# ArielleRosinski/pyGAT

Measured on AMD Instinct MI355X. Metric: GAT-layer fwd+bwd edges/sec, higher is better.
Workload: dtype f32

## Files before the change

include/pygat_amd.h:

```cpp
#ifndef PYGAT_AMD_H
#define PYGAT_AMD_H

#include <stdint.h>
#include <stddef.h>

#ifdef __cplusplus
extern "C" {
#endif

#define PYGAT_ABI_VERSION 14

enum {
  PYGAT_OK = 0,
  PYGAT_EINVAL = -1,
  PYGAT_EHIP = -2,
  PYGAT_ENODEV = -3
};

enum {
  PYGAT_F_ELU = 1,
  PYGAT_F_SKIP = 2,
  PYGAT_F_MAIN_ONLY = 4,
  PYGAT_F_FIXUP_ONLY = 8
};

int pygat_abi_version(void);
const char* pygat_last_error(void);
int pygat_padded_width(int f_out);
int pygat_device_count(void);
int pygat_device_name(char* host_buf, int len);
int pygat_kernel_footprint(const char* kernel, int* num_regs, int* scratch_bytes);

enum { PYGAT_GEMM_DEFAULT = -1, PYGAT_GEMM_SPLIT_BF16 = 0, PYGAT_GEMM_FP32_MFMA = 1 };
int pygat_default_gemm_mode(void);

int pygat_dense_row_counts(const float* adj, int n, int64_t ld, int mode,
                           int32_t* counts, void* stream);
size_t pygat_scan_workspace_bytes(int64_t n);
int pygat_exclusive_scan_i32(const int32_t* in, int64_t n, int32_t* out, void* ws, void* stream);
int pygat_dense_fill_cols(const float* adj, int n, int64_t ld, int mode,
                          const int32_t* rowptr, int32_t* col, void* stream);
int pygat_csr_symmetric_perm(int n, const int32_t* rowptr, const int32_t* col,
                             int32_t* perm, int32_t* flags, void* stream);

#define PYGAT_MAX_SEGMENTS 4
typedef struct {
  int nseg;
  int32_t col_start[PYGAT_MAX_SEGMENTS + 1];
  float* ptr[PYGAT_MAX_SEGMENTS];
  int64_t ld[PYGAT_MAX_SEGMENTS];
} pygat_out_segments;

size_t pygat_gemm_workspace_bytes(int M, int N, int split_k);
int pygat_gemm_f32(int transA, int transB, int M, int N, int64_t K,
                   const float* A, int64_t lda, const float* B, int64_t ldb,
                   const pygat_out_segments* out, int accumulate,
                   int split_k, void* ws, int gemm_mode, void* stream);

typedef struct {
  int w;
  int64_t stride;
} pygat_col_blocks;
int pygat_gemm_f32_blocked(int transA, int transB, int M, int N, int64_t K,
                           const float* A, int64_t lda, const pygat_col_blocks* a_blk, const float* B, int64_t ldb,
                           const pygat_out_segments* out, const pygat_col_blocks* c_blk, int accumulate,
                           int split_k, void* ws, int gemm_mode, void* stream);

int pygat_pack_params(int H, int Fin, int Fo, const float* W, const float* a,
                      const float* w_skip, float* Wcat, int64_t ldw, float* a_pad,
                      void* stream);
#define PYGAT_MAX_HEADS_TABLE 16
int pygat_pack_params_heads(int H, int Fin, int Fo, const float* const* W, const float* const* a,
                            const float* const* w_skip, float* Wcat, int64_t ldw, float* a_pad, void* stream);
int pygat_stack_heads(int H, int64_t nW, int nA, int64_t nS, const float* const* W, const float* const* a,
                      const float* const* w_skip, float* W_out, float* a_out, float* skip_out, void* stream);
int pygat_stack_heads_padded(int H, int64_t nW, int64_t nW_out, int nA, int64_t nS, int64_t nS_out, const float* const* W,
                             const float* const* a, const float* const* w_skip, float* W_out, float* a_out, float* skip_out,
                             void* stream);
int pygat_project(int n, int Fin, int H, int Fo, const float* X, int64_t ldx, const float* Wcat, int64_t ldw, const float* a_pad,
                  float* Wh, float* Sk, float* s, int split_k, void* ws, int gemm_mode, void* stream);
int pygat_project_blocked(int n, int Fin, int H, int Fo, const float* X, int64_t ldx, const pygat_col_blocks* x_blk,
                          const float* Wcat, int64_t ldw, const float* a_pad, float* Wh, float* Sk, float* s, int split_k,
                          void* ws, int gemm_mode, void* stream);
int pygat_attn_scores(int n, int H, int Fo, float* Wh, const float* wh_mask, const float* a_pad,
                      float* s, float* t, void* stream);
int pygat_unpack_wgrad(int H, int Fin, int Fo, const float* dWcat, int64_t ld,
                       int col_offset, float* dW, void* stream);

typedef struct {
  int n;
  int64_t nnz;
  const int32_t* rowptr;
  const int32_t* edge_rc;
  int slot_edges;
  const int32_t* slot_begin;
  const int32_t* cut_rows;
  int n_cut;
  int n_cut_wide;
  int64_t slot_first;
  int64_t slot_count;
  const int32_t* slot_meta;
  const int32_t* slot_order;
  const int32_t* user_row;
} pygat_graph;

int pygat_edge_pairs(int n, const int32_t* rowptr, const int32_t* col, int32_t* edge_rc, void* stream);

int pygat_slot_bounds(int n, int64_t nnz, const int32_t* rowptr, const int32_t* edge_rc, int slot_edges,
                      int32_t* slot_begin, void* stream);
int pygat_slot_meta(int n, int64_t nnz, const int32_t* rowptr, const int32_t* edge_rc, int slot_edges,
                    const int32_t* slot_begin, int32_t* slot_meta, void* stream);

size_t pygat_partials_bytes(int64_t nnz, int slot_edges, int H, int Fp);

int pygat_head_group(int n, int H, int Fo);

int pygat_gat_forward_phases_ok(int n, int H, int Fo);
int pygat_gat_forward(const pygat_graph* g, int H, int Fo, float alpha, int flags,
                      const float* Wh, const float* s, const float* a_pad, const float* sk,
                      const float* att_mask,
                      float* out, float* hattn, float* m, float* Z, float* aneg, float* qneg,
                      void* part, void* stream);

int pygat_head_mean(int n, int H, int Fo, const float* hattn, const float* sk,
                    float* out, void* stream);

int pygat_gat_backward_prepare(int n, int H, int Fo, int flags, int mean_mode,
                               const float* G, const float* y, const float* sk,
                               const float* s, const float* m, const float* Z,
                               float* GR, const float* aneg, const float* qneg, float alpha, float* ds,
                               int h_first, int h_count, int head_group, const int32_t* user_row, void* stream);
int pygat_gat_backward_row(const pygat_graph* g, int H, int Fo, float alpha,
                           const float* Wh, const float* a_pad, const float* GR,
                           const float* att_mask, float* ds, void* part, int h_first, int h_count, int head_group,
                           void* stream);
size_t pygat_gat_backward_col_da_bytes(const pygat_graph* gT, int H, int Fo, int head_group);
int pygat_gat_backward_col(const pygat_graph* gT, const int32_t* perm_t, int H, int Fo, float alpha,
                           const float* Wh, const float* a_pad, const float* GR,
                           const float* att_mask, const float* ds,
                           float* dWh, float* dt, float* dz_t, void* part, float* da_part, int h_first, int h_count,
                           int head_group, void* stream);
int pygat_a_grad_fold(const pygat_graph* gT, int H, int Fo, const float* Wh, const float* ds, const float* dt,
                      const float* da_part, float* da, void* ws, int head_group, void* stream);
int pygat_gat_backward_rowsum(const pygat_graph* g, const int32_t* perm_f, int H, int Fo, const float* dz_t,
                              float* ds, void* part, int h_first, int h_count, void* stream);
size_t pygat_agrad_workspace_bytes(int H, int Fo);
int pygat_a_grad(int n, int H, int Fo, const float* Wh, const float* ds, const float* dt,
                 float* da, void* ws, const float* a_pad, float* dWh, const float* dwh_mask, int h_first, int h_count,
                 void* stream);

size_t pygat_wgrad_workspace_bytes(int Fin, int H, int Fo, int split_k);
int pygat_wgrad(int n, int Fin, int H, int Fo, const float* X, int64_t ldx, const float* dWh, const float* ds,
                const float* a_pad, float* dW, int split_k, void* ws, int h_first, int h_count, int gemm_mode, void* stream);

int pygat_wgrad_blocked(int n, int Fin, int H, int Fo, const float* X, int64_t ldx, const pygat_col_blocks* x_blk,
                        const float* dWh, const float* ds, const float* a_pad, float* dW, int split_k, void* ws,
                        int h_first, int h_count, int gemm_mode, void* stream);

int pygat_gat_forward_tail(int row_first, int n_rows, int H, int Fo, int flags, const float* Wh, int64_t ldwh, const float* sk,
                           float* out, const int32_t* user_row, float* m, float* Z, float* qneg, void* stream);
int pygat_gat_backward_col_tail(int row_first, int n_rows, int H, int Fo, const float* GR, float* dWh, float* dt, void* stream);
int pygat_gat_backward_tail(int row_first, int n_rows, int H, int Fo, int flags, const float* G, const float* y,
                            const int32_t* user_row, float* dWh, int64_t ld_dwh, int zero_cols, float* ds, float* dt, void* stream);

int pygat_gatv2_forward(const pygat_graph* g, int H, int Fo, float alpha, int flags,
                        const float* WW, const float* a2, const float* sk, const float* att_mask,
                        float* out, float* hattn, float* m, float* Z, void* part, void* stream);
int pygat_gatv2_backward_prepare(int n, int H, int Fo, int flags, int mean_mode,
                                 const float* G, const float* y, const float* sk,
                                 const float* m, const float* Z, const float* WW, float* GRW, const int32_t* user_row,
                                 void* stream);
size_t pygat_gatv2_workspace_bytes(int64_t nnz, int slot_edges, int H, int Fo);
int pygat_gatv2_backward(const pygat_graph* g, const pygat_graph* gT, const int32_t* perm_t, const int32_t* perm_f,
                         int H, int Fo, float alpha, const float* WW, const float* a2, const float* GRW,
                         const float* att_mask, float* dWW, float* da, void* ws, void* stream);

int pygat_dropout_mask(int64_t count, float p, const void* seed, uint32_t stream_id, float* out, void* stream);
int pygat_dropout_mask2(float p, const void* seed, int64_t count1, uint32_t stream1, float* out1, int64_t count2,
                        uint32_t stream2, float* out2, void* stream);
int pygat_dropout_expand(int n, int Fin, int H, const float* x, int64_t ldx, const float* mask, float p,
                         const void* seed, uint32_t stream_id, float* out, int64_t ldo, void* stream);
int pygat_dropout_head_sum(int n, int Fin, int H, const float* dxe, int64_t lde, const float* mask, float p,
                           const void* seed, uint32_t stream_id, float* dx, int64_t ldx, int accumulate,
                           void* stream);
int pygat_pack_blockdiag(int H, int Fin, int Fo, const float* W, const float* w_skip, float* Bp, int64_t ldb,
                         void* stream);
int pygat_unpack_blockdiag(int H, int Fin, int Fo, const float* dBp, int64_t ldb, int col_offset, float* dW,
                           void* stream);

int pygat_headmask_supported(int H, int Fo, int skip);
int pygat_dropout_bits(int n, int Fin, int H, float p, const void* seed, int stream_id, unsigned char* bits, void* stream);
size_t pygat_project_dropout_workspace_bytes(int n, int H, int Fo, int skip, int split_k);
int pygat_project_dropout(int n, int Fin, int H, int Fo, const float* X, int64_t ldx, const unsigned char* bits, float p,
                          const float* Wcat, int64_t ldw, float* Wh, float* Sk, int split_k, void* ws, void* stream);
size_t pygat_wgrad_dropout_workspace_bytes(int Fin, int H, int Fo, int skip, int split_k);
int pygat_wgrad_dropout(int n, int Fin, int H, int Fo, const float* X, int64_t ldx, const unsigned char* bits, float p,
                        const float* dWh, const float* Gp, int64_t ldgp, float* dWc, int split_k, void* ws, void* stream);
int pygat_dropout_head_sum_bits(int n, int Fin, int H, const float* dxe, int64_t lde, const unsigned char* bits, float p,
                                float* dx, int64_t ldx, int accumulate, void* stream);
int pygat_dropout_narrow(int Fin, int H, int Fo, int skip);
int pygat_dx_dropout(int n, int Fin, int H, int Fo, const float* dWh, const float* Gp, int64_t ldgp, const unsigned char* bits,
                     float p, const float* Wcat, int64_t ldw, float* dx, int64_t lddx, int accumulate, void* stream);

size_t pygat_nll_workspace_bytes(int n);
int pygat_elu_logsoftmax_nll(int n, int C, const float* out, int64_t ldo, const int32_t* label, const float* weight,
                             void* ws, float* loss, void* stream);
int pygat_elu_logsoftmax_nll_backward(int n, int C, const float* out, int64_t ldo, const int32_t* label, const float* weight,
                                      const float* gscale, float* dout, int64_t ldd, void* stream);

int pygat_project_sparse(int n, int Fin, int H, int Fo, const int32_t* rowptr, const int32_t* col, const float* val,
                         const float* Wcat, int64_t ldw, float p, const void* seed, int stream_id, const unsigned char* bits,
                         float* Wh, float* Sk, float* s, void* stream);
size_t pygat_wgrad_sparse_workspace_bytes(int nseg, int H, int Fo, int skip);
int pygat_wgrad_sparse(int n, int Fin, int H, int Fo, int nseg, const int32_t* colseg, const int32_t* seg_col,
                       const int32_t* seg_begin, const int32_t* seg_end, const int32_t* row, const float* val, float p,
                       const void* seed, int stream_id, const unsigned char* bits, const float* dWh, const float* Gp, int64_t ldg,
                       void* ws, float* dW, float* dWskip, void* stream);

size_t pygat_bce_workspace_bytes(int64_t total);
int pygat_bce_with_logits(int64_t total, const float* logits, const float* targets, void* ws, float* loss, void* stream);
int pygat_bce_with_logits_backward(int64_t total, const float* logits, const float* targets, const float* gscale, float* dlogits,
                                   void* stream);

#define PYGAT_ADAM_MAX_TENSORS 48
#define PYGAT_ADAM_STATE_BYTES 24
int pygat_adam_step(int ntensors, float* const* params, const float* const* grads, float* const* exp_avg,
                    float* const* exp_avg_sq, const int64_t* numel, double lr, double beta1, double beta2, double eps,
                    double weight_decay, void* state, void* stream);

#ifdef __cplusplus
}
#endif
#endif
```

pygat_amd/_lib.py:

```python
from __future__ import annotations

import ctypes as C
import os

import torch

_HERE = os.path.dirname(os.path.abspath(__file__))
LIB_PATH = os.path.join(_HERE, "libpygat_amd.so")
from .config import config as _config
if _config.lib_path:
    LIB_PATH = os.path.abspath(_config.lib_path)

ABI_VERSION = 14
F_ELU = 1
F_SKIP = 2
F_MAIN_ONLY = 4
F_FIXUP_ONLY = 8

SYMBOLS = [
    "pygat_abi_version", "pygat_last_error", "pygat_padded_width", "pygat_device_count",
    "pygat_device_name", "pygat_kernel_footprint", "pygat_default_gemm_mode", "pygat_dense_row_counts", "pygat_scan_workspace_bytes",
    "pygat_exclusive_scan_i32", "pygat_dense_fill_cols", "pygat_csr_symmetric_perm",
    "pygat_gemm_workspace_bytes", "pygat_gemm_f32", "pygat_gemm_f32_blocked", "pygat_project_blocked", "pygat_wgrad_blocked", "pygat_pack_params", "pygat_pack_params_heads", "pygat_stack_heads", "pygat_stack_heads_padded", "pygat_project", "pygat_attn_scores",
    "pygat_unpack_wgrad",
    "pygat_edge_pairs", "pygat_slot_bounds", "pygat_slot_meta", "pygat_partials_bytes", "pygat_head_group", "pygat_gat_forward", "pygat_gat_forward_phases_ok", "pygat_gat_forward_tail", "pygat_gat_backward_col_tail", "pygat_gat_backward_tail", "pygat_head_mean",
    "pygat_gat_backward_prepare", "pygat_gat_backward_row", "pygat_gat_backward_col", "pygat_gat_backward_rowsum",
    "pygat_gat_backward_col_da_bytes", "pygat_a_grad_fold",
    "pygat_agrad_workspace_bytes", "pygat_a_grad", "pygat_wgrad_workspace_bytes", "pygat_wgrad",
    "pygat_gatv2_forward", "pygat_gatv2_backward_prepare", "pygat_gatv2_workspace_bytes", "pygat_gatv2_backward",
    "pygat_dropout_mask", "pygat_dropout_mask2", "pygat_dropout_expand", "pygat_dropout_head_sum", "pygat_pack_blockdiag",
    "pygat_unpack_blockdiag",
    "pygat_headmask_supported", "pygat_dropout_bits", "pygat_project_dropout_workspace_bytes", "pygat_project_dropout",
    "pygat_wgrad_dropout_workspace_bytes",
    "pygat_wgrad_dropout", "pygat_dropout_head_sum_bits",
    "pygat_nll_workspace_bytes", "pygat_elu_logsoftmax_nll", "pygat_elu_logsoftmax_nll_backward",
    "pygat_project_sparse", "pygat_wgrad_sparse", "pygat_wgrad_sparse_workspace_bytes", "pygat_dropout_narrow", "pygat_dx_dropout", "pygat_adam_step", "pygat_bce_workspace_bytes", "pygat_bce_with_logits", "pygat_bce_with_logits_backward",
]


MAX_ADAM_TENSORS = 48
MAX_SEGMENTS = 4


class OutSegments(C.Structure):
    _fields_ = [("nseg", C.c_int), ("col_start", C.c_int32 * (MAX_SEGMENTS + 1)), ("ptr", C.c_void_p * MAX_SEGMENTS),
                ("ld", C.c_int64 * MAX_SEGMENTS)]


class ColBlocks(C.Structure):
    _fields_ = [("w", C.c_int), ("stride", C.c_int64)]


class Graph(C.Structure):
    _fields_ = [("n", C.c_int), ("nnz", C.c_int64), ("rowptr", C.c_void_p), ("edge_rc", C.c_void_p),
                ("slot_edges", C.c_int), ("slot_begin", C.c_void_p), ("cut_rows", C.c_void_p),
                ("n_cut", C.c_int), ("n_cut_wide", C.c_int), ("slot_first", C.c_int64), ("slot_count", C.c_int64),
                ("slot_meta", C.c_void_p), ("slot_order", C.c_void_p), ("user_row", C.c_void_p)]


def _load():
    if not os.path.exists(LIB_PATH):
        raise ImportError(
            f"pygat_amd: {LIB_PATH} not found. Build it with `python -c 'import __graft_entry__ as g; "
            f"g.build()'` or `make -C pygat_amd/csrc`. There is no CPU/PyTorch fallback for the hot path.")
    lib = C.CDLL(LIB_PATH)
    missing = [s for s in SYMBOLS if not hasattr(lib, s)]
    if missing:
        raise ImportError(f"pygat_amd: {LIB_PATH} lacks symbols {missing}")
    p, i, i64, f, sz = C.c_void_p, C.c_int, C.c_int64, C.c_float, C.c_size_t
    lib.pygat_abi_version.restype = i
    lib.pygat_last_error.restype = C.c_char_p
    lib.pygat_padded_width.argtypes = [i]
    lib.pygat_device_name.argtypes = [C.c_char_p, i]
    lib.pygat_kernel_footprint.argtypes = [C.c_char_p, C.POINTER(C.c_int), C.POINTER(C.c_int)]
    lib.pygat_default_gemm_mode.argtypes = []
    lib.pygat_dense_row_counts.argtypes = [p, i, i64, i, p, p]
    lib.pygat_scan_workspace_bytes.argtypes = [i64]
    lib.pygat_scan_workspace_bytes.restype = sz
    lib.pygat_exclusive_scan_i32.argtypes = [p, i64, p, p, p]
    lib.pygat_dense_fill_cols.argtypes = [p, i, i64, i, p, p, p]
    lib.pygat_csr_symmetric_perm.argtypes = [i, p, p, p, p, p]
    lib.pygat_gemm_workspace_bytes.argtypes = [i, i, i]
    lib.pygat_gemm_workspace_bytes.restype = sz
    lib.pygat_gemm_f32.argtypes = [i, i, i, i, i64, p, i64, p, i64, C.POINTER(OutSegments), i, i, p, i, p]
    CB = C.POINTER(ColBlocks)
    lib.pygat_gemm_f32_blocked.argtypes = [i, i, i, i, i64, p, i64, CB, p, i64, C.POINTER(OutSegments), CB, i, i, p, i, p]
    lib.pygat_project_blocked.argtypes = [i, i, i, i, p, i64, CB, p, i64, p, p, p, p, i, p, i, p]
    lib.pygat_wgrad_blocked.argtypes = [i, i, i, i, p, i64, CB, p, p, p, p, i, p, i, i, i, p]
    lib.pygat_pack_params.argtypes = [i, i, i, p, p, p, p, i64, p, p]
    lib.pygat_pack_params_heads.argtypes = [i, i, i, p, p, p, p, i64, p, p]
    lib.pygat_stack_heads.argtypes = [i, i64, i, i64, p, p, p, p, p, p, p]
    lib.pygat_stack_heads_padded.argtypes = [i, i64, i64, i, i64, i64, p, p, p, p, p, p, p]
    lib.pygat_unpack_wgrad.argtypes = [i, i, i, p, i64, i, p, p]
    lib.pygat_attn_scores.argtypes = [i, i, i, p, p, p, p, p, p]
    lib.pygat_project.argtypes = [i, i, i, i, p, i64, p, i64, p, p, p, p, i, p, i, p]
    lib.pygat_edge_pairs.argtypes = [i, p, p, p, p]
    lib.pygat_slot_bounds.argtypes = [i, i64, p, p, i, p, p]
    lib.pygat_slot_meta.argtypes = [i, i64, p, p, i, p, p, p]
    lib.pygat_partials_bytes.argtypes = [i64, i, i, i]
    lib.pygat_partials_bytes.restype = sz
    lib.pygat_head_group.argtypes = [i, i, i]
    lib.pygat_head_group.restype = i
    lib.pygat_gat_forward.argtypes = [C.POINTER(Graph), i, i, f, i, p, p, p, p, p, p, p, p, p, p, p, p, p]
    lib.pygat_gat_forward_phases_ok.argtypes = [i, i, i]
    lib.pygat_gat_forward_tail.argtypes = [i, i, i, i, i, p, i64, p, p, p, p, p, p, p]
    lib.pygat_gat_backward_col_tail.argtypes = [i, i, i, i, p, p, p, p]
    lib.pygat_gat_backward_tail.argtypes = [i, i, i, i, i, p, p, p, p, i64, i, p, p, p]
    lib.pygat_head_mean.argtypes = [i, i, i, p, p, p, p]
    lib.pygat_gat_backward_prepare.argtypes = [i, i, i, i, i, p, p, p, p, p, p, p, p, p, f, p, i, i, i, p, p]
    lib.pygat_gat_backward_row.argtypes = [C.POINTER(Graph), i, i, f, p, p, p, p, p, p, i, i, i, p]
    lib.pygat_gat_backward_col.argtypes = [C.POINTER(Graph), p, i, i, f, p, p, p, p, p, p, p, p, p, p, i, i, i, p]
    lib.pygat_gat_backward_col_da_bytes.argtypes = [C.POINTER(Graph), i, i, i]
    lib.pygat_gat_backward_col_da_bytes.restype = sz
    lib.pygat_a_grad_fold.argtypes = [C.POINTER(Graph), i, i, p, p, p, p, p, p, i, p]
    lib.pygat_gat_backward_rowsum.argtypes = [C.POINTER(Graph), p, i, i, p, p, p, i, i, p]
    lib.pygat_agrad_workspace_bytes.argtypes = [i, i]
    lib.pygat_agrad_workspace_bytes.restype = sz
    lib.pygat_a_grad.argtypes = [i, i, i, p, p, p, p, p, p, p, p, i, i, p]
    lib.pygat_gatv2_forward.argtypes = [C.POINTER(Graph), i, i, f, i, p, p, p, p, p, p, p, p, p, p]
    lib.pygat_gatv2_backward_prepare.argtypes = [i, i, i, i, i, p, p, p, p, p, p, p, p, p]
    lib.pygat_gatv2_workspace_bytes.argtypes = [i64, i, i, i]
    lib.pygat_gatv2_workspace_bytes.restype = sz
    lib.pygat_gatv2_backward.argtypes = [C.POINTER(Graph), C.POINTER(Graph), p, p, i, i, f, p, p, p, p, p, p, p, p]
    u32 = C.c_uint32
    lib.pygat_wgrad_workspace_bytes.argtypes = [i, i, i, i]
    lib.pygat_wgrad_workspace_bytes.restype = sz
    lib.pygat_wgrad.argtypes = [i, i, i, i, p, i64, p, p, p, p, i, p, i, i, i, p]
    lib.pygat_dropout_mask.argtypes = [i64, f, p, u32, p, p]
    lib.pygat_dropout_mask2.argtypes = [f, p, i64, u32, p, i64, u32, p, p]
    lib.pygat_dropout_expand.argtypes = [i, i, i, p, i64, p, f, p, u32, p, i64, p]
    lib.pygat_dropout_head_sum.argtypes = [i, i, i, p, i64, p, f, p, u32, p, i64, i, p]
    lib.pygat_pack_blockdiag.argtypes = [i, i, i, p, p, p, i64, p]
    lib.pygat_unpack_blockdiag.argtypes = [i, i, i, p, i64, i, p, p]
    lib.pygat_headmask_supported.argtypes = [i, i, i]
    lib.pygat_dropout_bits.argtypes = [i, i, i, f, p, i, p, p]
    lib.pygat_project_dropout_workspace_bytes.argtypes = [i, i, i, i, i]
    lib.pygat_project_dropout_workspace_bytes.restype = sz
    lib.pygat_project_dropout.argtypes = [i, i, i, i, p, i64, p, f, p, i64, p, p, i, p, p]
    lib.pygat_wgrad_dropout_workspace_bytes.argtypes = [i, i, i, i, i]
    lib.pygat_wgrad_dropout_workspace_bytes.restype = sz
    lib.pygat_wgrad_dropout.argtypes = [i, i, i, i, p, i64, p, f, p, p, i64, p, i, p, p]
    lib.pygat_dropout_head_sum_bits.argtypes = [i, i, i, p, i64, p, f, p, i64, i, p]
    lib.pygat_project_sparse.argtypes = [i, i, i, i, p, p, p, p, i64, f, p, i, p, p, p, p, p]
    lib.pygat_wgrad_sparse.argtypes = [i, i, i, i, i, p, p, p, p, p, p, f, p, i, p, p, p, i64, p, p, p, p]
    lib.pygat_wgrad_sparse_workspace_bytes.argtypes = [i, i, i, i]
    lib.pygat_dropout_narrow.argtypes = [i, i, i, i]
    lib.pygat_bce_workspace_bytes.argtypes = [i64]
    lib.pygat_bce_workspace_bytes.restype = sz
    lib.pygat_bce_with_logits.argtypes = [i64, p, p, p, p, p]
    lib.pygat_bce_with_logits_backward.argtypes = [i64, p, p, p, p, p]
    lib.pygat_adam_step.argtypes = [i, p, p, p, p, p, C.c_double, C.c_double, C.c_double, C.c_double, C.c_double, p, p]
    lib.pygat_dx_dropout.argtypes = [i, i, i, i, p, p, i64, p, f, p, i64, p, i64, i, p]
    lib.pygat_wgrad_sparse_workspace_bytes.restype = sz
    lib.pygat_nll_workspace_bytes.argtypes = [i]
    lib.pygat_nll_workspace_bytes.restype = sz
    lib.pygat_elu_logsoftmax_nll.argtypes = [i, i, p, i64, p, p, p, p, p]
    lib.pygat_elu_logsoftmax_nll_backward.argtypes = [i, i, p, i64, p, p, p, p, i64, p]
    for s in SYMBOLS:
        fn = getattr(lib, s)
        if fn.restype is C.c_int or s in ("pygat_abi_version", "pygat_padded_width", "pygat_device_count", "pygat_default_gemm_mode"):
            fn.restype = i
    if lib.pygat_abi_version() != ABI_VERSION:
        raise ImportError(f"pygat_amd: ABI version {lib.pygat_abi_version()} != {ABI_VERSION}")
    return lib


lib = _load()


def check(rc: int, what: str = "") -> None:
    if rc == 0:
        return
    msg = lib.pygat_last_error().decode(errors="replace")
    if rc == -1:
        raise ValueError(f"pygat_amd {what}: {msg}")
    raise RuntimeError(f"pygat_amd {what}: {msg} (code {rc})")


def padded_width(f_out: int) -> int:
    fp = lib.pygat_padded_width(int(f_out))
    if fp == 0:
        raise ValueError(f"pygat_amd: head width {f_out} unsupported (1..256)")
    return fp
```

pygat_amd/config.py:

```python
from __future__ import annotations

import os
from dataclasses import dataclass, fields
from typing import Optional


def _flag(name: str, default: bool) -> bool:
    v = os.environ.get(name)
    return default if v is None else v not in ("0", "", "false", "False")


def _opt_flag(name: str) -> Optional[bool]:
    v = os.environ.get(name)
    return None if v is None else v == "1"


def _opt_int(name: str) -> Optional[int]:
    v = os.environ.get(name)
    return int(v) if v else None


@dataclass(frozen=True)
class Config:
    lib_path: Optional[str]
    dist_chunks: int
    dropout_wide: bool
    sparse_max_density: float
    sparse_x: bool
    slot_edges: Optional[int]
    slot_meta: bool
    two_gather_backward: Optional[bool]
    backward: Optional[str]
    da_in_k4: bool
    k1_split_min_k: int
    overlap_backward: bool
    pad_k: bool
    renumber: bool
    tail: bool

    @staticmethod
    def from_env() -> "Config":
        return Config(
            lib_path=os.environ.get("PYGAT_AMD_LIB") or None,
            dist_chunks=int(os.environ.get("PYGAT_DIST_CHUNKS", 4)),
            dropout_wide=_flag("PYGAT_DROPOUT_WIDE", False),
            sparse_max_density=float(os.environ.get("PYGAT_SPARSE_MAX_DENSITY", 0.15)),
            sparse_x=_flag("PYGAT_SPARSE_X", True),
            slot_edges=_opt_int("PYGAT_SLOT_EDGES"),
            slot_meta=not _flag("PYGAT_NO_SLOT_META", False),
            two_gather_backward=_opt_flag("PYGAT_TWO_GATHER_BACKWARD"),
            backward=os.environ.get("PYGAT_BACKWARD") or None,
            da_in_k4=_flag("PYGAT_DA_IN_K4", True),
            k1_split_min_k=int(os.environ.get("PYGAT_K1_SPLIT_MIN_K", 128)),
            overlap_backward=_flag("PYGAT_OVERLAP_BACKWARD", False),
            pad_k=_flag("PYGAT_PAD_K", True),
            renumber=_flag("PYGAT_RENUMBER", True),
            tail=_flag("PYGAT_TAIL", True),
        )

    def describe(self) -> dict:
        return {f.name: getattr(self, f.name) for f in fields(self)}


config = Config.from_env()
```

pygat_amd/csrc/core.hip:

```cpp
#include "common.h"
#include <string.h>

namespace pygat {
static thread_local char g_err[512] = "";

void set_error(const char* fmt, ...) {
  va_list ap;
  va_start(ap, fmt);
  vsnprintf(g_err, sizeof(g_err), fmt, ap);
  va_end(ap);
}

static const int g_default_split = [] { const char* e = getenv("PYGAT_GEMM_F32"); return (e && atoi(e) != 0) ? 0 : 1; }();
bool gemm_split(int mode) { return mode == PYGAT_GEMM_DEFAULT ? g_default_split != 0 : mode == PYGAT_GEMM_SPLIT_BF16; }
}

extern "C" int pygat_default_gemm_mode(void) { return pygat::g_default_split ? PYGAT_GEMM_SPLIT_BF16 : PYGAT_GEMM_FP32_MFMA; }

extern "C" int pygat_abi_version(void) { return PYGAT_ABI_VERSION; }
extern "C" const char* pygat_last_error(void) { return pygat::g_err; }
extern "C" int pygat_padded_width(int f_out) { return pygat::padded_width(f_out); }

namespace pygat {
int footprint_k2_headline(int* regs, int* scratch);
int footprint_k4_headline_da(int* regs, int* scratch);
int footprint_gemm_x3(int which, int* regs, int* scratch);
}

extern "C" int pygat_kernel_footprint(const char* kernel, int* num_regs, int* scratch_bytes) {
  PYGAT_REQUIRE(kernel && num_regs && scratch_bytes, "kernel_footprint: null argument");
  if (!strcmp(kernel, "k2_headline")) return pygat::footprint_k2_headline(num_regs, scratch_bytes);
  if (!strcmp(kernel, "k4_headline_da")) return pygat::footprint_k4_headline_da(num_regs, scratch_bytes);
  if (!strcmp(kernel, "tn_x3w")) return pygat::footprint_gemm_x3(0, num_regs, scratch_bytes);
  if (!strcmp(kernel, "x3gw")) return pygat::footprint_gemm_x3(1, num_regs, scratch_bytes);
  pygat::set_error("kernel_footprint: unknown kernel '%s' (k2_headline, k4_headline_da, tn_x3w, x3gw)", kernel);
  return PYGAT_EINVAL;
}

extern "C" int pygat_device_count(void) {
  int n = 0;
  if (hipGetDeviceCount(&n) != hipSuccess) {
    (void)hipGetLastError();
    return 0;
  }
  return n;
}

extern "C" int pygat_device_name(char* host_buf, int len) {
  if (!host_buf || len <= 0) return PYGAT_EINVAL;
  int dev = 0;
  hipDeviceProp_t p;
  if (hipGetDevice(&dev) != hipSuccess || hipGetDeviceProperties(&p, dev) != hipSuccess) {
    (void)hipGetLastError();
    pygat::set_error("no HIP device");
    return PYGAT_ENODEV;
  }
  snprintf(host_buf, (size_t)len, "%s (%s)", p.name, p.gcnArchName);
  return PYGAT_OK;
}
```

pygat_amd/csrc/gemm_fast.h:

```cpp
#pragma once
#include "common.h"

namespace pygat {

typedef float f32x16 __attribute__((ext_vector_type(16)));

struct SmallKArgs {
  int M, N, K;
  const float* A;
  int64_t lda;
  const float* B;
  int64_t ldb;
  pygat_out_segments out;
  int accumulate;
  int tiles_m;
  int transB;
  const float* sr_a;
  int sr_fp;
  const float* svec;
  int64_t sv_ld;
  int sv_n;
  float* s_out;
  int64_t s_ld;
  int vec_out, s_vec;
  int lds_rows;
};

struct TnArgs {
  int M, N;
  int64_t K;
  const float* A;
  int64_t lda;
  const float* B;
  int64_t ldb;
  int64_t k_per_split;
  float* ws;
  int N1;
  const float* B2;
  int64_t ldb2;
};

#ifdef __HIPCC__
__device__ __forceinline__ float* out_segment(const pygat_out_segments& out, int col, int64_t& ld) {
  ld = out.ld[0];
  float* p = out.ptr[0];
  int c0 = 0;
#pragma unroll
  for (int q = 1; q < PYGAT_MAX_SEGMENTS; ++q)
    if (q < out.nseg && col >= out.col_start[q]) { ld = out.ld[q]; p = out.ptr[q]; c0 = out.col_start[q]; }
  return p + (col - c0);
}
#endif

bool gemm_split(int mode);

int try_gemm_smallk_x3(const SmallKArgs& g, int NT, dim3 grid, hipStream_t st);
int try_project_x3(int n, int Fin, int H, int Fp, const float* X, int64_t ldx, const float* Wcat, int64_t ldw, float* Wh,
                   float* s, const float* a_pad, bool split, hipStream_t st);
int try_gemm_tn_x3(const TnArgs& g, int splits, hipStream_t st);
int try_gemm_x3g(int transA, int transB, int M, int N, int64_t K, const float* A, int64_t lda, const float* B, int64_t ldb,
                 const pygat_out_segments* out, int accumulate, int splits, int64_t k_per_split, float* ws, hipStream_t st,
                 ColBlocks ab, ColBlocks cb, int* splits_used);

}
```

pygat_amd/csrc/k1_gemm.hip:

```cpp
#include "common.h"
#include "narrow.h"
#include <type_traits>

namespace pygat {

typedef float f32x16 __attribute__((ext_vector_type(16)));

constexpr int BM = 128;
constexpr int BK = 16;
constexpr int PAD = 4;

struct GemmArgs {
  int M, N;
  int64_t K;
  const float* A;
  int64_t lda;
  const float* B;
  int64_t ldb;
  pygat_out_segments out;
  int accumulate;
  int64_t k_per_split;
  float* ws;
  int a_vec, b_vec;
  ColBlocks ab, cb;
// ... 216 lines not shown
        __syncthreads();
        if (kt + 1 < nkt) {
          gload2(kof(kt + 3));
          mma_tile(1);
          if (kt + 2 < nkt) sstore(0);
          __syncthreads();
        }
        if (((kt >> 1) % (FLUSH_TILES / 2)) == FLUSH_TILES / 2 - 1) flush();
      }
    } else {
      if (nkt > 0) {
        gload(kbeg);
        sstore(0);
      }
      __syncthreads();
      for (int64_t kt = 0; kt < nkt; ++kt) {
        const int buf = (int)(kt & 1);
        if (kt + 1 < nkt) gload(kbeg + (kt + 1) * BK);
        mma_tile(buf);
        if (kt + 1 < nkt) sstore(buf ^ 1);
        __syncthreads();
        if ((kt % FLUSH_TILES) == FLUSH_TILES - 1) flush();
      }
    }
  };
  if (interior) kloop(std::true_type{});
  else kloop(std::false_type{});
#pragma unroll
  for (int i = 0; i < NT; ++i)
#pragma unroll
    for (int r = 0; r < 16; ++r) acc[i][r] += acc2[i][r];

#pragma unroll
  for (int nt = 0; nt < NT; ++nt) {
    const int col = n0 + 32 * nt + fr;
    if (col >= g.N) continue;
    float* base;
    int64_t ld;
    if (g.ws) {
      base = g.ws + ((int64_t)blockIdx.z * g.M) * g.N + col;
      ld = g.N;
    } else if (g.cb.lw < 62) {
      base = g.out.ptr[0] + blk_off(col, g.cb);
      ld = g.out.ld[0];
    } else {
      int s = 0;
#pragma unroll
      for (int q = 1; q < PYGAT_MAX_SEGMENTS; ++q)
        if (q < g.out.nseg && col >= g.out.col_start[q]) s = q;
      base = g.out.ptr[s] + (col - g.out.col_start[s]);
      ld = g.out.ld[s];
    }
#pragma unroll
    for (int r = 0; r < 16; ++r) {
      const int row = m0 + 32 * w + (r & 3) + 8 * (r >> 2) + 4 * fk;
      if (row < g.M) {
        float* p = base + (int64_t)row * ld;
        if (!g.ws && g.accumulate) *p += acc[nt][r];
        else *p = acc[nt][r];
      }
    }
  }
}

__global__ __launch_bounds__(512) void gemm_splitk_reduce_kernel(int M, int N, int splits,
                                                                 const float* __restrict__ ws,
                                                                 pygat_out_segments out, int accumulate) {
  const int64_t tot = (int64_t)M * N;
  const int lane = threadIdx.x & 63, q = threadIdx.x >> 6;
  const int64_t i = (int64_t)blockIdx.x * 64 + lane;
  float v = 0.f;
  if (i < tot) {
    int z = q;
    for (; z + 24 < splits; z += 32) {
      const float x0 = ws[(int64_t)z * tot + i], x1 = ws[(int64_t)(z + 8) * tot + i];
      const float x2 = ws[(int64_t)(z + 16) * tot + i], x3 = ws[(int64_t)(z + 24) * tot + i];
      v += x0; v += x1; v += x2; v += x3;
    }
    for (; z < splits; z += 8) v += ws[(int64_t)z * tot + i];
  }
  __shared__ float sm[8][64];
  sm[q][lane] = v;
  __syncthreads();
  if (q == 0 && i < tot) {
    float acc = 0.f;
#pragma unroll
    for (int z = 0; z < 8; ++z) acc += sm[z][lane];
    const int row = (int)(i / N), col = (int)(i % N);
    int s = 0;
    for (int k = 1; k < out.nseg; ++k)
      if (col >= out.col_start[k]) s = k;
    float* p = out.ptr[s] + (int64_t)row * out.ld[s] + (col - out.col_start[s]);
    if (accumulate) *p += acc; else *p = acc;
  }
}

struct HeadMaskArgs {
  int M;
  int64_t K;
  const float* A;
  int64_t lda;
  const unsigned char* bits;
  const float* B1;
  int64_t ldb1;
  const float* B2;
  int64_t ldb2;
  float* C1;
  int64_t ldc1;
  float* C2;
  int64_t ldc2;
  int64_t c_split_stride;
  int H, Fp;
  float scale;
  int64_t k_per_split;
};

typedef float f32x4_u __attribute__((ext_vector_type(4), aligned(4)));
typedef uint32_t u32_u __attribute__((aligned(1)));

template <bool TA, int HB, int NTH>
__global__ __launch_bounds__(256) __attribute__((amdgpu_waves_per_eu(2))) void gemm_headmask_kernel(HeadMaskArgs g) {
  constexpr int NTOT = HB * NTH, BN = 32 * NTOT;
  constexpr int LDAS = BM + PAD, LDBS = BN + PAD;
  constexpr int NVA = 2;
  constexpr int NU = (BK * HB * 8 * NTH + 255) / 256;
  extern __shared__ __attribute__((aligned(16))) float hm_sm[];
  float* As = hm_sm;
  float* Bs = As + 2 * BK * LDAS;
  unsigned char* Ms = reinterpret_cast<unsigned char*>(Bs + 2 * BK * LDBS);
  const int m0 = blockIdx.x * BM, hb0 = blockIdx.y * HB;
  const int64_t kbeg = (int64_t)blockIdx.z * g.k_per_split;
  const int64_t kend = (kbeg + g.k_per_split < g.K) ? kbeg + g.k_per_split : g.K;
  const int lane = threadIdx.x & 63, w = threadIdx.x >> 6;
  const int cols_h = g.B2 ? 2 * g.Fp : g.Fp;
  const int q_h = cols_h >> 2;
  const int units = BK * HB * q_h;

  f32x16 acc[NTOT];
#pragma unroll
  for (int i = 0; i < NTOT; ++i)
#pragma unroll
    for (int r = 0; r < 16; ++r) acc[i][r] = 0.f;

  float4 ra[NVA];
  uint32_t rm[NVA];
  float4 rb[NU];
  auto gload = [&](int64_t k0) {
#pragma unroll
    for (int i = 0; i < NVA; ++i) {
      const int idx = threadIdx.x + 256 * i;
      float4 v = make_float4(0.f, 0.f, 0.f, 0.f);
      uint32_t mv = 0;
      int64_t off;
      int nval;
      if constexpr (TA) {
        const int64_t k = k0 + idx / (BM / 4);
        const int c = m0 + (idx % (BM / 4)) * 4;
        off = k * g.lda + c;
        nval = (k < kend) ? (g.M - c) : 0;
      } else {
        const int row = m0 + (idx >> 2);
        const int64_t k = k0 + (idx & 3) * 4;
        off = (int64_t)row * g.lda + k;
        nval = (row < g.M) ? (int)(kend - k) : 0;
      }
      if (nval >= 4) {
        const f32x4_u t = *reinterpret_cast<const f32x4_u*>(g.A + off);
        v = make_float4(t.x, t.y, t.z, t.w);
        mv = *reinterpret_cast<const u32_u*>(g.bits + off);
      } else if (nval > 0) {
        float t[4] = {0.f, 0.f, 0.f, 0.f};
        for (int q = 0; q < nval; ++q) { t[q] = g.A[off + q]; mv |= (uint32_t)g.bits[off + q] << (8 * q); }
        v = make_float4(t[0], t[1], t[2], t[3]);
      }
      ra[i] = v; rm[i] = mv;
    }
#pragma unroll
    for (int i = 0; i < NU; ++i) {
      const int u = threadIdx.x + 256 * i;
      float4 v = make_float4(0.f, 0.f, 0.f, 0.f);
      if (u < units) {
        const int kk = u / (HB * q_h), r2 = u - kk * (HB * q_h), hl = r2 / q_h, c = (r2 - hl * q_h) * 4;
        const int64_t k = k0 + kk;
        const int h = hb0 + hl;
        if (k < kend && h < g.H)
          v = c < g.Fp ? ld4(g.B1 + k * g.ldb1 + (int64_t)h * g.Fp + c) : ld4(g.B2 + k * g.ldb2 + (int64_t)h * g.Fp + (c - g.Fp));
      }
      rb[i] = v;
    }
  };
  auto sstore = [&](int buf) {
    float* as = As + buf * BK * LDAS;
    unsigned char* ms = Ms + buf * BK * LDAS;
    if constexpr (TA) store_kstrided<BM, NVA, LDAS>(as, ra);
    else store_kcontig<BM, NVA, LDAS>(as, ra);
#pragma unroll
    for (int i = 0; i < NVA; ++i) {
      const int idx = threadIdx.x + 256 * i;
      if constexpr (TA) {
        *reinterpret_cast<uint32_t*>(ms + (idx / (BM / 4)) * LDAS + (idx % (BM / 4)) * 4) = rm[i];
      } else {
        const int row = idx >> 2, kq = (idx & 3) * 4;
        ms[(kq + 0) * LDAS + row] = (unsigned char)rm[i]; ms[(kq + 1) * LDAS + row] = (unsigned char)(rm[i] >> 8);
        ms[(kq + 2) * LDAS + row] = (unsigned char)(rm[i] >> 16); ms[(kq + 3) * LDAS + row] = (unsigned char)(rm[i] >> 24);
      }
    }
    float* bs = Bs + buf * BK * LDBS;
#pragma unroll
    for (int i = 0; i < NU; ++i) {
      const int u = threadIdx.x + 256 * i;
      if (u < units) {
        const int kk = u / (HB * q_h), r2 = u - kk * (HB * q_h), hl = r2 / q_h, c = (r2 - hl * q_h) * 4;
        st4(bs + kk * LDBS + hl * 32 * NTH + c, rb[i]);
      }
    }
  };

  const int64_t nkt = (kend > kbeg) ? (kend - kbeg + BK - 1) / BK : 0;
  if (nkt > 0) { gload(kbeg); sstore(0); }
  __syncthreads();
  const int fr = lane & 31, fk = lane >> 5;
  for (int64_t kt = 0; kt < nkt; ++kt) {
    const int buf = (int)(kt & 1);
    if (kt + 1 < nkt) gload(kbeg + (kt + 1) * BK);
    const float* as = As + buf * BK * LDAS + fk * LDAS + 32 * w + fr;
    const unsigned char* ms = Ms + buf * BK * LDAS + fk * LDAS + 32 * w + fr;
    const float* bs = Bs + buf * BK * LDBS + fk * LDBS + fr;
#pragma unroll
    for (int kk = 0; kk < BK; kk += 2) {
      const float xs = as[kk * LDAS];
      const uint32_t mb = (uint32_t)ms[kk * LDAS] >> hb0;
#pragma unroll
      for (int hl = 0; hl < HB; ++hl) {
        const float a = ((mb >> hl) & 1u) ? xs : 0.f;
#pragma unroll
        for (int nt = 0; nt < NTH; ++nt)
          acc[hl * NTH + nt] = __builtin_amdgcn_mfma_f32_32x32x2f32(a, bs[kk * LDBS + 32 * (hl * NTH + nt)], acc[hl * NTH + nt], 0, 0, 0);
      }
    }
    if (kt + 1 < nkt) sstore(buf ^ 1);
    __syncthreads();
  }

  const int64_t zoff = (int64_t)blockIdx.z * g.c_split_stride;
#pragma unroll
  for (int hl = 0; hl < HB; ++hl) {
    const int h = hb0 + hl;
    if (h >= g.H) continue;
#pragma unroll
    for (int nt = 0; nt < NTH; ++nt) {
      const int c = 32 * nt + fr;
      if (c >= cols_h) continue;
      float* base = c < g.Fp ? g.C1 + zoff + (int64_t)h * g.Fp + c : g.C2 + zoff + (int64_t)h * g.Fp + (c - g.Fp);
      const int64_t ld = c < g.Fp ? g.ldc1 : g.ldc2;
#pragma unroll
      for (int r = 0; r < 16; ++r) {
        const int row = m0 + 32 * w + (r & 3) + 8 * (r >> 2) + 4 * fk;
        if (row < g.M) base[(int64_t)row * ld] = acc[hl * NTH + nt][r] * g.scale;
      }
    }
  }
}

template <bool TA>
static int launch_headmask(const HeadMaskArgs& g, int splits, hipStream_t st) {
  const int cols_h = g.B2 ? 2 * g.Fp : g.Fp;
  const int nth = cols_h <= 32 ? 1 : cols_h <= 64 ? 2 : cols_h <= 128 ? 4 : 8;
  const int hb = 8 / nth;
  if (cols_h > 256 || g.H > 8) return 0;
  dim3 grid((unsigned)cdiv(g.M, BM), (unsigned)cdiv(g.H, hb), (unsigned)splits);
  const size_t lds = (size_t)(2 * BK * (BM + PAD) + 2 * BK * (32 * 8 + PAD)) * sizeof(float) + 2 * BK * (BM + PAD);
  switch (nth) {
    case 1: hipLaunchKernelGGL((gemm_headmask_kernel<TA, 8, 1>), grid, dim3(256), lds, st, g); break;
    case 2: hipLaunchKernelGGL((gemm_headmask_kernel<TA, 4, 2>), grid, dim3(256), lds, st, g); break;
    case 4: hipLaunchKernelGGL((gemm_headmask_kernel<TA, 2, 4>), grid, dim3(256), lds, st, g); break;
    default: hipLaunchKernelGGL((gemm_headmask_kernel<TA, 1, 8>), grid, dim3(256), lds, st, g); break;
  }
  return 1;
}

template <bool TA, bool TB>
static int launch_gemm(const GemmArgs& g, int splits, hipStream_t st) {
  const int nt_needed = (int)cdiv(g.N, 32);
  int NT = nt_needed <= 1 ? 1 : nt_needed <= 2 ? 2 : nt_needed <= 3 ? 3 : nt_needed <= 4 ? 4 : nt_needed <= 5 ? 5 : 4;
  dim3 grid((unsigned)cdiv(g.M, BM), (unsigned)cdiv(g.N, 32 * NT), (unsigned)splits);
  auto lds = [](int nt, int bk) { return (size_t)2 * bk * ((BM + PAD) + (32 * nt + PAD)) * sizeof(float); };
  switch (NT) {
    case 1: hipLaunchKernelGGL((gemm_f32_kernel<TA, TB, 1, 16>), grid, dim3(256), lds(1, 16), st, g); break;
    case 2: hipLaunchKernelGGL((gemm_f32_kernel<TA, TB, 2, 16>), grid, dim3(256), lds(2, 16), st, g); break;
    case 3: hipLaunchKernelGGL((gemm_f32_kernel<TA, TB, 3, 16>), grid, dim3(256), lds(3, 16), st, g); break;
    case 4: hipLaunchKernelGGL((gemm_f32_kernel<TA, TB, 4, 16>), grid, dim3(256), lds(4, 16), st, g); break;
    default: hipLaunchKernelGGL((gemm_f32_kernel<TA, TB, 5, 16>), grid, dim3(256), lds(5, 16), st, g); break;
  }
  return 0;
}

int try_gemm_smallk(int transB, int M, int N, int64_t K, const float* A, int64_t lda, const float* B, int64_t ldb,
                    const pygat_out_segments* out, int accumulate, bool split, hipStream_t st, const float* svec = nullptr,
                    int64_t sv_ld = 0, int sv_n = 0, float* s_out = nullptr, int64_t s_ld = 0);
int try_gemm_tn_stream(int M, int N, int64_t K, const float* A, int64_t lda, const float* B, int64_t ldb,
                       int max_splits, float* ws, bool split, hipStream_t st, int N1, const float* B2, int64_t ldb2);
int try_project_x3(int n, int Fin, int H, int Fp, const float* X, int64_t ldx, const float* Wcat, int64_t ldw, float* Wh,
                   float* s, const float* a_pad, bool split, hipStream_t st);
int try_gemm_x3g(int transA, int transB, int M, int N, int64_t K, const float* A, int64_t lda, const float* B, int64_t ldb,
                 const pygat_out_segments* out, int accumulate, int splits, int64_t k_per_split, float* ws, hipStream_t st,
                 ColBlocks ab, ColBlocks cb, int* splits_used);
bool gemm_split(int mode);

}

using namespace pygat;

extern "C" size_t pygat_gemm_workspace_bytes(int M, int N, int split_k) {
  if (split_k <= 1) return 0;
  return (size_t)split_k * (size_t)M * (size_t)N * sizeof(float);
}

extern "C" int pygat_gemm_f32(int transA, int transB, int M, int N, int64_t K, const float* A, int64_t lda,
                              const float* B, int64_t ldb, const pygat_out_segments* out, int accumulate,
                              int split_k, void* ws, int gemm_mode, void* stream) {
  return pygat_gemm_f32_blocked(transA, transB, M, N, K, A, lda, nullptr, B, ldb, out, nullptr, accumulate, split_k, ws, gemm_mode,
                                stream);
}

extern "C" int pygat_gemm_f32_blocked(int transA, int transB, int M, int N, int64_t K, const float* A, int64_t lda,
                                      const pygat_col_blocks* a_blk, const float* B, int64_t ldb, const pygat_out_segments* out,
                                      const pygat_col_blocks* c_blk, int accumulate, int split_k, void* ws, int gemm_mode,
                                      void* stream) {
  PYGAT_REQUIRE(A && B && out, "gemm: null pointer");
  PYGAT_REQUIRE(gemm_mode >= PYGAT_GEMM_DEFAULT && gemm_mode <= PYGAT_GEMM_FP32_MFMA, "gemm: unknown product mode %d", gemm_mode);
  const bool split = gemm_split(gemm_mode);
  PYGAT_REQUIRE(M > 0 && N > 0 && K > 0, "gemm: bad sizes M=%d N=%d K=%lld", M, N, (long long)K);
  PYGAT_REQUIRE(out->nseg >= 1 && out->nseg <= PYGAT_MAX_SEGMENTS && out->col_start[0] == 0 && out->col_start[out->nseg] == N,
                "gemm: output segments must cover [0,N) (nseg=%d)", out->nseg);
  const bool a_blocked = col_blocks_on(a_blk), c_blocked = col_blocks_on(c_blk);
  for (int s = 0; s < out->nseg; ++s)
    PYGAT_REQUIRE(out->ptr[s] && out->col_start[s + 1] > out->col_start[s] &&
                      (c_blocked || out->ld[s] >= out->col_start[s + 1] - out->col_start[s]),
                  "gemm: bad output segment %d", s);
  PYGAT_REQUIRE((a_blocked ? lda >= a_blk->w : lda >= (transA ? M : K)) && ldb >= (transB ? K : N), "gemm: leading dimension too small");
  PYGAT_REQUIRE(col_blocks_ok(a_blk, transA ? M : K, lda) && (!a_blocked || aligned16(A)),
                "gemm: bad column blocks of A (w a power of two >= 16 dividing the blocked extent; 16-byte aligned base, rows, blocks)");
  PYGAT_REQUIRE(!c_blocked || (col_blocks_ok(c_blk, N, out->ld[0]) && out->nseg == 1 && aligned16(out->ptr[0])),
                "gemm: bad column blocks of C (one segment; w a power of two >= 16 dividing N)");
  if (split_k < 1) split_k = 1;
  PYGAT_REQUIRE(split_k == 1 || ws, "gemm: split_k > 1 needs a workspace");
  PYGAT_REQUIRE(!c_blocked || split_k == 1, "gemm: a column-blocked C takes no split-K");
  const ColBlocks ab = col_blocks_of(a_blk), cb = col_blocks_of(c_blk);
  hipStream_t st = (hipStream_t)stream;
  if (a_blocked || c_blocked) {
  } else if (!transA && split_k == 1) {
    int r = try_gemm_smallk(transB, M, N, K, A, lda, B, ldb, out, accumulate, split, st);
    if (r < 0) return r;
    if (r == 1) return PYGAT_OK;
  }
  if (!a_blocked && transA && !transB && split_k > 1) {
    int r = try_gemm_tn_stream(M, N, K, A, lda, B, ldb, split_k, (float*)ws, split, st, N, nullptr, 0);
    if (r < 0) return r;
    if (r >= 1) {
      int64_t tot = (int64_t)M * N;
      hipLaunchKernelGGL(gemm_splitk_reduce_kernel, dim3((unsigned)cdiv(tot, 64)), dim3(512), 0, st, M, N, r,
                         (const float*)ws, *out, accumulate);
      PYGAT_CHECK_LAUNCH("gemm_splitk_reduce");
      return PYGAT_OK;
    }
  }
  if (split) {
    const int64_t kps16 = cdiv(cdiv(K, split_k), 16) * 16;
    int sp = (int)cdiv(K, kps16);
    const int r = try_gemm_x3g(transA, transB, M, N, K, A, lda, B, ldb, out, accumulate, sp, kps16, (float*)ws, st, ab, cb, &sp);
    if (r < 0) return r;
    if (r == 1) {
      if (sp > 1) {
        hipLaunchKernelGGL(gemm_splitk_reduce_kernel, dim3((unsigned)cdiv((int64_t)M * N, 64)), dim3(512), 0, st, M, N, sp,
                           (const float*)ws, *out, accumulate);
        PYGAT_CHECK_LAUNCH("gemm_splitk_reduce");
      }
      return PYGAT_OK;
    }
  }
  GemmArgs g;
  g.M = M; g.N = N; g.K = K; g.A = A; g.lda = lda; g.B = B; g.ldb = ldb; g.out = *out;
  g.accumulate = accumulate;
  g.ab = ab; g.cb = cb;
  int64_t kps = cdiv(cdiv(K, split_k), BK) * BK;
  int splits = (int)cdiv(K, kps);
  g.k_per_split = kps;
  g.ws = (splits > 1) ? (float*)ws : nullptr;
  g.a_vec = aligned16(A) && (lda % 4 == 0);
  g.b_vec = aligned16(B) && (ldb % 4 == 0);
  if (!transA && !transB) launch_gemm<false, false>(g, splits, st);
  else if (transA && !transB) launch_gemm<true, false>(g, splits, st);
  else if (!transA && transB) launch_gemm<false, true>(g, splits, st);
  else { pygat::set_error("gemm: transA && transB is not built"); return PYGAT_EINVAL; }
  PYGAT_CHECK_LAUNCH("gemm_f32");
  if (splits > 1) {
    int64_t tot = (int64_t)M * N;
    hipLaunchKernelGGL(gemm_splitk_reduce_kernel, dim3((unsigned)cdiv(tot, 64)), dim3(512), 0, st, M, N, splits,
                       (const float*)ws, *out, accumulate);
    PYGAT_CHECK_LAUNCH("gemm_splitk_reduce");
  }
  return PYGAT_OK;
}

extern "C" int pygat_project(int n, int Fin, int H, int Fo, const float* X, int64_t ldx, const float* Wcat, int64_t ldw,
                             const float* a_pad, float* Wh, float* Sk, float* s, int split_k, void* ws, int gemm_mode,
                             void* stream) {
  return pygat_project_blocked(n, Fin, H, Fo, X, ldx, nullptr, Wcat, ldw, a_pad, Wh, Sk, s, split_k, ws, gemm_mode, stream);
}

extern "C" int pygat_project_blocked(int n, int Fin, int H, int Fo, const float* X, int64_t ldx, const pygat_col_blocks* x_blk,
                                     const float* Wcat, int64_t ldw, const float* a_pad, float* Wh, float* Sk, float* s,
                                     int split_k, void* ws, int gemm_mode, void* stream) {
  const bool blocked = col_blocks_on(x_blk);
  const int Fp = padded_width(Fo);
  PYGAT_REQUIRE(n > 0 && Fin > 0 && H > 0 && Fp > 0 && X && Wcat && Wh && s, "project: bad arguments");
  PYGAT_REQUIRE(gemm_mode >= PYGAT_GEMM_DEFAULT && gemm_mode <= PYGAT_GEMM_FP32_MFMA, "project: unknown product mode %d", gemm_mode);
  const bool split = gemm_split(gemm_mode);
  const int R = H * Fp, nw = R * (Sk ? 2 : 1), ncols = nw + H;
  PYGAT_REQUIRE(ldw >= nw + 2 * H && (blocked ? ldx >= x_blk->w : ldx >= Fin), "project: leading dimension too small");
  pygat_out_segments seg;
  int k = 0;
  if (!blocked && a_pad && split_k <= 1) {
    const int r = try_project_x3(n, Fin, H, Fp, X, ldx, Wcat, ldw, Wh, s, a_pad, split, (hipStream_t)stream);
    if (r < 0) return r;
    if (r == 1) {
      if (!Sk) return PYGAT_OK;
      seg.nseg = 1; seg.col_start[0] = 0; seg.col_start[1] = R; seg.ptr[0] = Sk; seg.ld[0] = R;
      return pygat_gemm_f32(0, 0, n, R, Fin, X, ldx, Wcat + R, ldw, &seg, 0, 1, nullptr, gemm_mode, stream);
    }
  }
  seg.col_start[0] = 0; seg.ptr[k] = Wh; seg.ld[k] = R; ++k;
  if (Sk) { seg.col_start[k] = R; seg.ptr[k] = Sk; seg.ld[k] = R; ++k; }
  if (!blocked && H <= 8 && split_k <= 1) {
    seg.col_start[k] = nw; seg.nseg = k;
    const int r = try_gemm_smallk(0, n, nw, Fin, X, ldx, Wcat, ldw, &seg, 0, split, (hipStream_t)stream, Wcat + nw, ldw, H, s, H);
    if (r < 0) return r;
    if (r == 1) return PYGAT_OK;
  }
  seg.col_start[k] = nw; seg.ptr[k] = s; seg.ld[k] = H; ++k;
  seg.col_start[k] = ncols;
  seg.nseg = k;
  return pygat_gemm_f32_blocked(0, 0, n, ncols, Fin, X, ldx, x_blk, Wcat, ldw, &seg, nullptr, 0, split_k, ws, gemm_mode, stream);
}

namespace pygat {
__global__ __launch_bounds__(256) void unpack_wgrad_rank1_kernel(int H, int Fin, int Fo, int Fp, const float* __restrict__ dWc,
                                                                 int64_t ld, int with_ds, const float* __restrict__ a_pad,
                                                                 float* __restrict__ dW) {
  const int64_t idx = (int64_t)blockIdx.x * 256 + threadIdx.x;
  if (idx >= (int64_t)H * Fin * Fo) return;
  const int f = (int)(idx % Fo);
  const int k = (int)((idx / Fo) % Fin);
  const int h = (int)(idx / ((int64_t)Fo * Fin));
  float v = dWc[(int64_t)k * ld + h * Fp + f];
  if (with_ds) v = fmaf(dWc[(int64_t)k * ld + H * Fp + h], a_pad[(int64_t)h * 2 * Fp + f], v);
  dW[idx] = v;
}
}

extern "C" size_t pygat_wgrad_workspace_bytes(int Fin, int H, int Fo, int split_k) {
  const int Fp = padded_width(Fo);
  if (Fin <= 0 || H <= 0 || Fp <= 0) return 0;
  if (split_k < 1) split_k = 1;
  const size_t ncols = (size_t)H * Fp + (size_t)((H + 3) / 4) * 4;
  return (size_t)(split_k + 1) * (size_t)Fin * ncols * sizeof(float);
}

extern "C" int pygat_wgrad(int n, int Fin, int H, int Fo, const float* X, int64_t ldx, const float* dWh, const float* ds,
                           const float* a_pad, float* dW, int split_k, void* ws, int h_first, int h_count, int gemm_mode,
                           void* stream) {
  return pygat_wgrad_blocked(n, Fin, H, Fo, X, ldx, nullptr, dWh, ds, a_pad, dW, split_k, ws, h_first, h_count, gemm_mode, stream);
}

extern "C" int pygat_wgrad_blocked(int n, int Fin, int H, int Fo, const float* X, int64_t ldx, const pygat_col_blocks* x_blk,
                                   const float* dWh, const float* ds, const float* a_pad, float* dW, int split_k, void* ws,
                                   int h_first, int h_count, int gemm_mode, void* stream) {
  const bool blocked = col_blocks_on(x_blk);
  const int Fp = padded_width(Fo);
  PYGAT_REQUIRE(gemm_mode >= PYGAT_GEMM_DEFAULT && gemm_mode <= PYGAT_GEMM_FP32_MFMA, "wgrad: unknown product mode %d", gemm_mode);
  const bool split = gemm_split(gemm_mode);
  PYGAT_REQUIRE(n > 0 && Fin > 0 && H > 0 && Fp > 0 && X && dWh && dW && ws && (blocked ? ldx >= x_blk->w : ldx >= Fin),
                "wgrad: bad arguments");
  PYGAT_REQUIRE(!ds || a_pad, "wgrad: ds needs a_pad");
  if (h_count == 0 && h_first == 0) h_count = H;
  PYGAT_REQUIRE(h_first >= 0 && h_count > 0 && h_first + h_count <= H, "wgrad: bad head range [%d, +%d) of %d", h_first, h_count, H);
  const int64_t ldd = (int64_t)H * Fp, lds = H;
  dWh += (int64_t)h_first * Fp;
  if (ds) ds += h_first;
  if (a_pad) a_pad += (int64_t)h_first * 2 * Fp;
  dW += (int64_t)h_first * Fin * Fo;
  H = h_count;
  if (split_k < 1) split_k = 1;
  hipStream_t st = (hipStream_t)stream;
  const int R = H * Fp;
  const int ldc = R + ((H + 3) / 4) * 4;
  float* dWc = (float*)ws;
  float* slabs = dWc + (size_t)Fin * ldc;
  pygat_out_segments seg;
  seg.nseg = 1; seg.col_start[0] = 0; seg.ptr[0] = dWc; seg.ld[0] = ldc;
  bool done = false;
  if (!blocked && ds && split_k > 1 && split && R > 64 && Fin > 64) {
    seg.col_start[1] = R;
    int r = try_gemm_tn_stream(Fin, R, n, X, ldx, dWh, ldd, split_k, slabs, split, st, R, nullptr, 0);
    if (r < 0) return r;
    if (r >= 1) {
      hipLaunchKernelGGL(gemm_splitk_reduce_kernel, dim3((unsigned)cdiv((int64_t)Fin * R, 64)), dim3(512), 0, st, Fin, R, r,
                         (const float*)slabs, seg, 0);
      PYGAT_CHECK_LAUNCH("wgrad(reduce)");
      pygat_out_segments seg2;
      seg2.nseg = 1; seg2.col_start[0] = 0; seg2.col_start[1] = H; seg2.ptr[0] = dWc + R; seg2.ld[0] = ldc;
      int64_t sk2 = (int64_t)split_k * (R + H) / H;
      if (sk2 > 256) sk2 = 256;
      const int r2 = try_gemm_tn_stream(Fin, H, n, X, ldx, ds, lds, (int)sk2, slabs, split, st, H, nullptr, 0);
      if (r2 < 0) return r2;
      if (r2 >= 1) {
        hipLaunchKernelGGL(gemm_splitk_reduce_kernel, dim3((unsigned)cdiv((int64_t)Fin * H, 64)), dim3(512), 0, st, Fin, H, r2,
                           (const float*)slabs, seg2, 0);
        PYGAT_CHECK_LAUNCH("wgrad(reduce ds)");
      } else {
        const int rc = pygat_gemm_f32(1, 0, Fin, H, n, X, ldx, ds, lds, &seg2, 0, split_k, slabs, gemm_mode, stream);
        if (rc) return rc;
      }
      done = true;
    }
  }
  if (!blocked && !done && ds && split_k > 1) {
    seg.col_start[1] = R + H;
    int r = try_gemm_tn_stream(Fin, R + H, n, X, ldx, dWh, ldd, split_k, slabs, split, st, R, ds, lds);
    if (r < 0) return r;
    if (r >= 1) {
      const int64_t tot = (int64_t)Fin * (R + H);
      hipLaunchKernelGGL(gemm_splitk_reduce_kernel, dim3((unsigned)cdiv(tot, 64)), dim3(512), 0, st, Fin, R + H, r,
                         (const float*)slabs, seg, 0);
      PYGAT_CHECK_LAUNCH("wgrad(reduce)");
      done = true;
    }
  }
  if (!done) {
    seg.col_start[1] = R;
    int rc = pygat_gemm_f32_blocked(1, 0, Fin, R, n, X, ldx, x_blk, dWh, ldd, &seg, nullptr, 0, split_k, slabs, gemm_mode, stream);
    if (rc) return rc;
    if (ds) {
      seg.col_start[1] = H; seg.ptr[0] = dWc + R;
      rc = pygat_gemm_f32_blocked(1, 0, Fin, H, n, X, ldx, x_blk, ds, lds, &seg, nullptr, 0, split_k, slabs, gemm_mode, stream);
      if (rc) return rc;
    }
  }
  hipLaunchKernelGGL(unpack_wgrad_rank1_kernel, dim3((unsigned)cdiv((int64_t)H * Fin * Fo, 256)), dim3(256), 0, st, H, Fin,
                     Fo, Fp, (const float*)dWc, (int64_t)ldc, ds ? 1 : 0, a_pad, dW);
  PYGAT_CHECK_LAUNCH("wgrad(unpack)");
  return PYGAT_OK;
}


extern "C" int pygat_headmask_supported(int H, int Fo, int skip) {
  const int Fp = padded_width(Fo);
  return (H >= 1 && H <= 8 && Fp > 0 && Fp * (skip ? 2 : 1) <= 256) ? 1 : 0;
}

extern "C" size_t pygat_project_dropout_workspace_bytes(int n, int H, int Fo, int skip, int split_k) {
  const int Fp = padded_width(Fo);
  if (n <= 0 || H <= 0 || Fp <= 0 || split_k <= 1) return 0;
  return (size_t)split_k * (size_t)n * (size_t)(H * Fp * (skip ? 2 : 1)) * sizeof(float);
}

extern "C" int pygat_project_dropout(int n, int Fin, int H, int Fo, const float* X, int64_t ldx, const unsigned char* bits,
                                     float p, const float* Wcat, int64_t ldw, float* Wh, float* Sk, int split_k, void* ws,
                                     void* stream) {
  const int Fp = padded_width(Fo);
  PYGAT_REQUIRE(n > 0 && Fin > 0 && X && bits && Wcat && Wh && ldx == Fin, "project_dropout: bad arguments (X must be dense: ldx == Fin)");
  PYGAT_REQUIRE(pygat_headmask_supported(H, Fo, Sk != nullptr), "project_dropout: unsupported H=%d F'=%d", H, Fo);
  PYGAT_REQUIRE(p >= 0.f && p <= 1.f, "project_dropout: p=%g outside [0,1]", (double)p);
  if (narrow_takes(Fin, H, Fo, Sk != nullptr))
    return narrow_project(n, Fin, H, Fo, X, ldx, bits, p, Wcat, ldw, Wh, Sk, (hipStream_t)stream);
  if (split_k < 1) split_k = 1;
  PYGAT_REQUIRE(split_k == 1 || ws, "project_dropout: split_k > 1 needs a workspace");
  const int R = H * Fp, ntot = R * (Sk ? 2 : 1);
  hipStream_t st = (hipStream_t)stream;
  const int64_t kps = cdiv(cdiv(Fin, split_k), BK) * BK;
  const int splits = (int)cdiv(Fin, kps);
  HeadMaskArgs g;
  g.M = n; g.K = Fin; g.A = X; g.lda = ldx; g.bits = bits;
  g.B1 = Wcat; g.ldb1 = ldw; g.B2 = Sk ? Wcat + R : nullptr; g.ldb2 = ldw;
  if (splits > 1) {
    g.C1 = (float*)ws; g.ldc1 = ntot; g.C2 = (float*)ws + R; g.ldc2 = ntot; g.c_split_stride = (int64_t)n * ntot;
  } else {
    g.C1 = Wh; g.ldc1 = R; g.C2 = Sk; g.ldc2 = R; g.c_split_stride = 0;
  }
  g.H = H; g.Fp = Fp; g.scale = p < 1.f ? 1.f / (1.f - p) : 0.f; g.k_per_split = kps;
  launch_headmask<false>(g, splits, st);
  PYGAT_CHECK_LAUNCH("project_dropout");
  if (splits > 1) {
    pygat_out_segments seg;
    seg.nseg = Sk ? 2 : 1; seg.col_start[0] = 0; seg.ptr[0] = Wh; seg.ld[0] = R; seg.col_start[1] = R;
    if (Sk) { seg.ptr[1] = Sk; seg.ld[1] = R; seg.col_start[2] = 2 * R; }
    hipLaunchKernelGGL(gemm_splitk_reduce_kernel, dim3((unsigned)cdiv((int64_t)n * ntot, 64)), dim3(512), 0, st, n, ntot,
                       splits, (const float*)ws, seg, 0);
    PYGAT_CHECK_LAUNCH("project_dropout(reduce)");
  }
  return PYGAT_OK;
}

extern "C" size_t pygat_wgrad_dropout_workspace_bytes(int Fin, int H, int Fo, int skip, int split_k) {
  const int Fp = padded_width(Fo);
  if (Fin <= 0 || H <= 0 || Fp <= 0) return 0;
  if (split_k < 1) split_k = 1;
  return (size_t)split_k * (size_t)Fin * (size_t)(H * Fp * (skip ? 2 : 1)) * sizeof(float);
}

extern "C" int pygat_wgrad_dropout(int n, int Fin, int H, int Fo, const float* X, int64_t ldx, const unsigned char* bits,
                                   float p, const float* dWh, const float* Gp, int64_t ldgp, float* dWc, int split_k,
                                   void* ws, void* stream) {
  const int Fp = padded_width(Fo);
  PYGAT_REQUIRE(n > 0 && Fin > 0 && X && bits && dWh && dWc && ldx == Fin, "wgrad_dropout: bad arguments");
  PYGAT_REQUIRE(pygat_headmask_supported(H, Fo, Gp != nullptr), "wgrad_dropout: unsupported H=%d F'=%d", H, Fo);
  if (split_k < 1) split_k = 1;
  PYGAT_REQUIRE(split_k == 1 || ws, "wgrad_dropout: split_k > 1 needs a workspace");
  if (narrow_takes(Fin, H, Fo, Gp != nullptr)) {
    PYGAT_REQUIRE(ws, "wgrad_dropout: the narrow kernels need the workspace (pygat_wgrad_dropout_workspace_bytes)");
    return narrow_wgrad(n, Fin, H, Fo, X, ldx, bits, p, dWh, Gp, ldgp, dWc, split_k, ws, (hipStream_t)stream);
  }
  const int R = H * Fp, ntot = R * (Gp ? 2 : 1);
  hipStream_t st = (hipStream_t)stream;
  int64_t kps = cdiv(cdiv(n, split_k), BK) * BK;
  const int splits = (int)cdiv(n, kps);
  float* out = splits > 1 ? (float*)ws : dWc;
  HeadMaskArgs g;
  g.M = Fin; g.K = n; g.A = X; g.lda = ldx; g.bits = bits;
  g.B1 = dWh; g.ldb1 = R; g.B2 = Gp; g.ldb2 = ldgp;
  g.C1 = out; g.ldc1 = ntot; g.C2 = out + R; g.ldc2 = ntot; g.c_split_stride = (int64_t)Fin * ntot;
  g.H = H; g.Fp = Fp; g.scale = p < 1.f ? 1.f / (1.f - p) : 0.f; g.k_per_split = kps;
  launch_headmask<true>(g, splits, st);
  PYGAT_CHECK_LAUNCH("wgrad_dropout");
  if (splits > 1) {
    pygat_out_segments seg;
    seg.nseg = 1; seg.col_start[0] = 0; seg.col_start[1] = ntot; seg.ptr[0] = dWc; seg.ld[0] = ntot;
    hipLaunchKernelGGL(gemm_splitk_reduce_kernel, dim3((unsigned)cdiv((int64_t)Fin * ntot, 64)), dim3(512), 0, st, Fin, ntot,
                       splits, (const float*)ws, seg, 0);
    PYGAT_CHECK_LAUNCH("wgrad_dropout(reduce)");
  }
  return PYGAT_OK;
}
```

pygat_amd/csrc/k1_gemm_x3.hip:

```cpp
#include "gemm_fast.h"
#include <stdlib.h>
#include <type_traits>

namespace pygat {

typedef __bf16 bf16x8 __attribute__((ext_vector_type(8)));

struct U4 { uint32_t v[4]; };
struct Frag3 { U4 h, m, l; };

__device__ __forceinline__ void split_pair(float x0, float x1, uint32_t& h, uint32_t& m, uint32_t& l) {
  const uint32_t u0 = __float_as_uint(x0), u1 = __float_as_uint(x1);
  h = __builtin_amdgcn_perm(u1, u0, 0x07060302u);
  const float r0 = x0 - __uint_as_float(u0 & 0xffff0000u), r1 = x1 - __uint_as_float(u1 & 0xffff0000u);
  const uint32_t v0 = __float_as_uint(r0), v1 = __float_as_uint(r1);
  m = __builtin_amdgcn_perm(v1, v0, 0x07060302u);
  const float q0 = r0 - __uint_as_float(v0 & 0xffff0000u), q1 = r1 - __uint_as_float(v1 & 0xffff0000u);
  l = __builtin_amdgcn_perm(__float_as_uint(q1), __float_as_uint(q0), 0x07060302u);
}
__device__ __forceinline__ Frag3 split8(float x0, float x1, float x2, float x3, float x4, float x5, float x6, float x7) {
  Frag3 f;
  split_pair(x0, x1, f.h.v[0], f.m.v[0], f.l.v[0]);
  split_pair(x2, x3, f.h.v[1], f.m.v[1], f.l.v[1]);
  split_pair(x4, x5, f.h.v[2], f.m.v[2], f.l.v[2]);
  split_pair(x6, x7, f.h.v[3], f.m.v[3], f.l.v[3]);
  return f;
}
__device__ __forceinline__ Frag3 split8v(const float4& a, const float4& b) { return split8(a.x, a.y, a.z, a.w, b.x, b.y, b.z, b.w); }
__device__ __forceinline__ void split_one(float x, uint16_t& h, uint16_t& m, uint16_t& l) {
  const uint32_t u = __float_as_uint(x);
  h = (uint16_t)(u >> 16);
  const float r = x - __uint_as_float(u & 0xffff0000u);
  const uint32_t v = __float_as_uint(r);
  m = (uint16_t)(v >> 16);
  const float q = r - __uint_as_float(v & 0xffff0000u);
  l = (uint16_t)(__float_as_uint(q) >> 16);
}

template <class TA_, class TB_>
__device__ __forceinline__ f32x16 mfma_bf16(const TA_& a, const TB_& b, f32x16 c) {
  return __builtin_amdgcn_mfma_f32_32x32x16_bf16(__builtin_bit_cast(bf16x8, a), __builtin_bit_cast(bf16x8, b), c, 0, 0, 0);
}
__device__ __forceinline__ void pair_of(const float4& a, const float4& b, int j, float& x0, float& x1) {
  if (j == 0) { x0 = a.x; x1 = a.y; } else if (j == 1) { x0 = a.z; x1 = a.w; } else if (j == 2) { x0 = b.x; x1 = b.y; } else { x0 = b.z; x1 = b.w; }
}
#ifndef PYGAT_DIAG_K1
#define PYGAT_DIAG_K1 0
#endif
#ifndef PYGAT_K1_LDS_ROWS
#define PYGAT_K1_LDS_ROWS 1
#endif
template <class TB_>
__device__ __forceinline__ f32x16 mma9(const Frag3& a, const TB_& bh, const TB_& bm, const TB_& bl, f32x16 c) {
#if (PYGAT_DIAG_K1 & 8)
  return mfma_bf16(a.h, bh, c);
#endif
  c = mfma_bf16(a.l, bl, c);
  c = mfma_bf16(a.l, bm, c);
  c = mfma_bf16(a.m, bl, c);
  c = mfma_bf16(a.l, bh, c);
  c = mfma_bf16(a.h, bl, c);
  c = mfma_bf16(a.m, bm, c);
  c = mfma_bf16(a.m, bh, c);
  c = mfma_bf16(a.h, bm, c);
  c = mfma_bf16(a.h, bh, c);
  return c;
}

template <class TB_>
__device__ __forceinline__ f32x16 mma9t(const Frag3& x, const TB_& wh, const TB_& wm, const TB_& wl, f32x16 c) {
#if (PYGAT_DIAG_K1 & 8)
  return mfma_bf16(wh, x.h, c);
#endif
  c = mfma_bf16(wl, x.l, c);
  c = mfma_bf16(wm, x.l, c);
  c = mfma_bf16(wl, x.m, c);
  c = mfma_bf16(wh, x.l, c);
  c = mfma_bf16(wl, x.h, c);
  c = mfma_bf16(wm, x.m, c);
  c = mfma_bf16(wh, x.m, c);
  c = mfma_bf16(wm, x.h, c);
  c = mfma_bf16(wh, x.h, c);
  return c;
}
__device__ __forceinline__ float half_wave_sum(float x) {
  const uint32_t u = __float_as_uint(x);
  const auto r = __builtin_amdgcn_permlane32_swap(u, u, false, false);
  return __uint_as_float(r[0]) + __uint_as_float(r[1]);
}

#if (PYGAT_DIAG_K1 & 16)
__device__ unsigned long long k1_stamps[2048 * 8 * 8];
#endif
template <bool TB, int NT, int SM, int SPC>
__global__ __launch_bounds__(512) void gemm_smallk_x3_kernel(SmallKArgs g) {
  constexpr bool SV = (SM == 1);
  constexpr int SRF = (SM >= 4) ? SM : 0;
  constexpr int BN = 32 * NT;
  extern __shared__ __attribute__((aligned(16))) unsigned char smem_x3[];
  const int KP = g.K + 8;
  uint16_t* Bimg = reinterpret_cast<uint16_t*>(smem_x3);
  const int IMG = BN * KP;
  float* Us = reinterpret_cast<float*>(Bimg + 3 * IMG);
  float* Asr = Us + (SV ? g.K * 8 : 0);
  float* Stg = Asr + (SRF > 0 ? BN : 0) + 4;
  const int n0 = blockIdx.y * BN;
  unsigned long long st_entry = 0; (void)st_entry;
  if ((PYGAT_DIAG_K1 & 16)) st_entry = __builtin_amdgcn_s_memrealtime();
  for (int item = threadIdx.x; item < (g.K >> 3) * BN; item += 512) {
    const int n = item % BN, k8 = item / BN;
    const bool ok = n0 + n < g.N;
    float v[8];
    if constexpr (!TB) {
      const float* bp = g.B + (int64_t)(8 * k8) * g.ldb + (ok ? n0 + n : 0);
#pragma unroll
      for (int j = 0; j < 8; ++j) v[j] = bp[(int64_t)j * g.ldb];
    } else {
      const float* bp = g.B + (int64_t)(ok ? n0 + n : 0) * g.ldb + 8 * k8;
#pragma unroll
      for (int j = 0; j < 8; ++j) v[j] = bp[j];
    }
    uint32_t ph[4], pm[4], pl[4];
#pragma unroll
    for (int j = 0; j < 4; ++j) {
      uint16_t h0, m0, l0, h1, m1, l1;
      split_one(ok ? v[2 * j] : 0.f, h0, m0, l0);
      split_one(ok ? v[2 * j + 1] : 0.f, h1, m1, l1);
      ph[j] = (uint32_t)h0 | ((uint32_t)h1 << 16); pm[j] = (uint32_t)m0 | ((uint32_t)m1 << 16); pl[j] = (uint32_t)l0 | ((uint32_t)l1 << 16);
    }
    uint16_t* d = Bimg + n * KP + 8 * k8;
    *reinterpret_cast<uint4*>(d) = make_uint4(ph[0], ph[1], ph[2], ph[3]);
    *reinterpret_cast<uint4*>(d + IMG) = make_uint4(pm[0], pm[1], pm[2], pm[3]);
    *reinterpret_cast<uint4*>(d + 2 * IMG) = make_uint4(pl[0], pl[1], pl[2], pl[3]);
  }
  if constexpr (SV) {
    for (int idx = threadIdx.x; idx < g.K * 8; idx += 512) {
      const int k = idx >> 3, h = idx & 7;
      Us[idx] = (h < g.sv_n) ? g.svec[(int64_t)k * g.sv_ld + h] : 0.f;
    }
  }
  if constexpr (SRF > 0) {
    for (int n = threadIdx.x; n < BN; n += 512) {
      const int col = n0 + n;
      Asr[n] = (col < g.N) ? g.sr_a[(col / SRF) * 2 * SRF + (col % SRF)] : 0.f;
    }
  }
  if (threadIdx.x < 4) reinterpret_cast<int*>(Asr + (SRF > 0 ? BN : 0))[threadIdx.x] = 0;
  __syncthreads();

  const int lane = threadIdx.x & 63, w = threadIdx.x >> 6;
  const int fr = lane & 31, fh = lane >> 5;
  const int nchunks = g.K / 32;
  if ((int)blockIdx.x >= g.tiles_m) return;
  const int my_tiles = (g.tiles_m - (int)blockIdx.x + (int)gridDim.x - 1) / (int)gridDim.x;
  const int total = my_tiles * nchunks;

  auto chunk_ptr = [&](int c) -> const float* {
    if (c > total - 1) c = total - 1;
    const int t = c / nchunks, kc = c - t * nchunks;
    int64_t row = ((int64_t)blockIdx.x + (int64_t)t * gridDim.x) * 256 + 32 * w + fr;
    if (row > g.M - 1) row = g.M - 1;
    return g.A + row * g.lda + kc * 32 + 8 * fh;
  };

  f32x16 acc[NT];
#pragma unroll
  for (int i = 0; i < NT; ++i)
#pragma unroll
    for (int r = 0; r < 16; ++r) acc[i][r] = 0.f;
  float sacc[8];
#pragma unroll
  for (int i = 0; i < 8; ++i) sacc[i] = 0.f;
  const bool sv_on = SV && blockIdx.y == 0;

  auto store_tile = [&](int64_t row0, auto fast_tag) {
    constexpr bool FAST = decltype(fast_tag)::value;
    const int64_t row = row0 + fr;
    const bool row_ok = FAST || row < g.M;
    const bool full = FAST || row0 + 32 <= g.M;
    if constexpr (SV) {
      if (sv_on) {
#pragma unroll
        for (int i = 0; i < 8; ++i) sacc[i] += __shfl_xor(sacc[i], 32);
        if (fh == 0 && row_ok) {
          float* so = g.s_out + row * g.s_ld;
          if (FAST && g.sv_n == 8) {
#pragma unroll
            for (int i = 0; i < 8; ++i) so[i] = sacc[i];
          } else {
#pragma unroll
            for (int i = 0; i < 8; ++i)
              if (i < g.sv_n) so[i] = sacc[i];
          }
        }
      }
#pragma unroll
      for (int i = 0; i < 8; ++i) sacc[i] = 0.f;
    }
    constexpr int SRD = SRF > 0 ? SRF : 32;
    constexpr int HPT = 32 / SRD, GPH = SRF > 0 ? SRF / 8 : 1;
    float hs[4] = {0.f, 0.f, 0.f, 0.f};
    float keep[4] = {0.f, 0.f, 0.f, 0.f};
    (void)keep;
    float* so = (SRF > 0) ? g.s_out + row * g.s_ld + n0 / SRD : nullptr;
#pragma unroll
    for (int nt = 0; nt < NT; ++nt) {
      if constexpr (SRF > 0 && !(PYGAT_DIAG_K1 & 2)) {
#pragma unroll
        for (int hh = 0; hh < HPT; ++hh) {
          float p = 0.f;
#pragma unroll
          for (int gg = 0; gg < GPH; ++gg) {
            const int gq = hh * GPH + gg;
            const float4 av = ld4(Asr + 32 * nt + 8 * gq + 4 * fh);
            p = fmaf(acc[nt][4 * gq], av.x, p); p = fmaf(acc[nt][4 * gq + 1], av.y, p);
            p = fmaf(acc[nt][4 * gq + 2], av.z, p); p = fmaf(acc[nt][4 * gq + 3], av.w, p);
          }
          const int hi = nt * HPT + hh;
          hs[hi & 3] = half_wave_sum(p);
          if constexpr (FAST) {
            if ((hi & 3) == 3) {
              const int grp = hi >> 2;
              if ((grp & 1) == 0) {
#pragma unroll
                for (int q = 0; q < 4; ++q) keep[q] = hs[q];
                if (hi == NT * HPT - 1) st4(so + 4 * grp, make_float4(keep[0], keep[1], keep[2], keep[3]));
              } else {
#pragma unroll
                for (int q = 0; q < 4; ++q) keep[q] = fh ? hs[q] : keep[q];
                st4(so + 4 * (grp - 1) + 4 * fh, make_float4(keep[0], keep[1], keep[2], keep[3]));
              }
            }
          } else if ((hi & 3) == 3) {
            if (g.s_vec) {
              if (row_ok && fh == ((hi >> 2) & 1)) st4(so + (hi - 3), make_float4(hs[0], hs[1], hs[2], hs[3]));
            } else if (row_ok && fh == 0) {
              so[hi - 3] = hs[0]; so[hi - 2] = hs[1]; so[hi - 1] = hs[2]; so[hi] = hs[3];
            }
          } else if (hi == NT * HPT - 1) {
            if (row_ok && fh == 0) {
#pragma unroll
              for (int q = 0; q <= (hi & 3); ++q) so[hi - (hi & 3) + q] = hs[q];
            }
          }
        }
      }
      const int colt = n0 + 32 * nt;
      if constexpr (FAST) {
        if (!(PYGAT_DIAG_K1 & 1)) {
          int64_t ld;
          float* base = out_segment(g.out, colt, ld);
          asm volatile("" : "+v"(ld));
          float* patch = Stg + w * (32 * 36);
#pragma unroll
          for (int gq = 0; gq < 4; ++gq)
            st4(patch + fr * 36 + 8 * gq + 4 * fh, make_float4(acc[nt][4 * gq], acc[nt][4 * gq + 1], acc[nt][4 * gq + 2], acc[nt][4 * gq + 3]));
          float* bq = base + (row0 + (lane >> 3)) * ld + 4 * (lane & 7);
#pragma unroll
          for (int q = 0; q < 4; ++q)
            st4(bq + (int64_t)8 * q * ld, ld4(patch + ((lane >> 3) + 8 * q) * 36 + 4 * (lane & 7)));
        }
      } else {
      const bool vec = full && !g.accumulate && g.vec_out && colt + 32 <= g.N;
      if ((PYGAT_DIAG_K1 & 1) ? (g.M == -12345) : vec) {
        int64_t ld;
        float* base = out_segment(g.out, colt, ld) + row * ld + 4 * fh;
#pragma unroll
        for (int gq = 0; gq < 4; ++gq)
          st4(base + 8 * gq, make_float4(acc[nt][4 * gq], acc[nt][4 * gq + 1], acc[nt][4 * gq + 2], acc[nt][4 * gq + 3]));
      } else if (!(PYGAT_DIAG_K1 & 1)) {
#pragma unroll
        for (int gq = 0; gq < 4; ++gq) {
          const int col4 = colt + 8 * gq + 4 * fh;
          int64_t ld;
          float* p = out_segment(g.out, col4, ld) + row * ld;
#pragma unroll
          for (int j = 0; j < 4; ++j)
            if (row_ok && col4 + j < g.N) {
              if (g.accumulate) p[j] += acc[nt][4 * gq + j]; else p[j] = acc[nt][4 * gq + j];
            }
        }
      }
      }
#pragma unroll
      for (int r = 0; r < 16; ++r) acc[nt][r] = 0.f;
    }
  };

#define PYGAT_X3_LOAD(R, P)                                                                   \
  {                                                                                           \
    const float* p__ = (P);                                                                   \
    R##0 = ld4(p__); R##1 = ld4(p__ + 4); R##2 = ld4(p__ + 16); R##3 = ld4(p__ + 20);         \
  }
#define PYGAT_X3_SACC(X, KK)                                                                  \
  {                                                                                           \
    const float4 ua = ld4(us + (KK) * 8), ub = ld4(us + (KK) * 8 + 4);                        \
    sacc[0] = fmaf((X), ua.x, sacc[0]); sacc[1] = fmaf((X), ua.y, sacc[1]);                   \
    sacc[2] = fmaf((X), ua.z, sacc[2]); sacc[3] = fmaf((X), ua.w, sacc[3]);                   \
    sacc[4] = fmaf((X), ub.x, sacc[4]); sacc[5] = fmaf((X), ub.y, sacc[5]);                   \
    sacc[6] = fmaf((X), ub.z, sacc[6]); sacc[7] = fmaf((X), ub.w, sacc[7]);                   \
  }
#define PYGAT_X3_SACC8(V0, V1, KK)                                                            \
  PYGAT_X3_SACC((V0).x, (KK) + 0) PYGAT_X3_SACC((V0).y, (KK) + 1) PYGAT_X3_SACC((V0).z, (KK) + 2) PYGAT_X3_SACC((V0).w, (KK) + 3) \
  PYGAT_X3_SACC((V1).x, (KK) + 4) PYGAT_X3_SACC((V1).y, (KK) + 5) PYGAT_X3_SACC((V1).z, (KK) + 6) PYGAT_X3_SACC((V1).w, (KK) + 7)
#define PYGAT_X3_BREAD(DST, S, NTI)                                                           \
  {                                                                                           \
    const uint16_t* q__ = bb + (NTI) * 32 * KP + (S) * 16;                                    \
    DST[0] = *reinterpret_cast<const uint4*>(q__);                                            \
    DST[1] = *reinterpret_cast<const uint4*>(q__ + IMG);                                      \
    DST[2] = *reinterpret_cast<const uint4*>(q__ + 2 * IMG);                                  \
  }
#define PYGAT_X3_BODY(R, KOFF, NSTEP)                                                         \
  {                                                                                           \
    const uint16_t* bb = Bimg + fr * KP + (KOFF) + 8 * fh;                                    \
    if constexpr (SV) if (sv_on) {                                                            \
      const float* us = Us + ((KOFF) + 8 * fh) * 8;                                           \
      PYGAT_X3_SACC8(R##0, R##1, 0)                                                           \
      if constexpr ((NSTEP) == 2) { PYGAT_X3_SACC8(R##2, R##3, 16) }                          \
    }                                                                                         \
    Frag3 af[2];                                                                              \
    af[0] = split8v((R##0), (R##1));                                                          \
    if constexpr ((NSTEP) == 2) af[1] = split8v((R##2), (R##3));                              \
    uint4 bf[2][3];                                                                           \
    PYGAT_X3_BREAD(bf[0], 0, 0)                                                               \
    _Pragma("unroll") for (int i__ = 0; i__ < (NSTEP) * NT; ++i__) {                          \
      const int s__ = i__ / NT, nt__ = i__ % NT;                                              \
      if (i__ + 1 < (NSTEP) * NT) PYGAT_X3_BREAD(bf[(i__ + 1) & 1], (i__ + 1) / NT, (i__ + 1) % NT) \
      __builtin_amdgcn_sched_barrier(0);                                                      \
      acc[nt__] = mma9t(af[s__], bf[i__ & 1][0], bf[i__ & 1][1], bf[i__ & 1][2], acc[nt__]);  \
      __builtin_amdgcn_sched_barrier(0);                                                      \
    }                                                                                         \
  }
#define PYGAT_X3_STEP(R, CIDX)                                                                \
  {                                                                                           \
    const int c__ = (CIDX);                                                                   \
    const int t__ = c__ / nchunks, kc__ = c__ - t__ * nchunks;                                \
    PYGAT_X3_BODY(R, kc__ * 32, 2)                                                            \
    if (kc__ == nchunks - 1) store_tile(((int64_t)blockIdx.x + (int64_t)t__ * gridDim.x) * 256 + 32 * w, std::false_type{}); \
  }

  float4 ra0, ra1, ra2, ra3, rb0, rb1, rb2, rb3, rc0, rc1, rc2, rc3, rd0, rd1, rd2, rd3;
  if constexpr (SPC == 0) {
    PYGAT_X3_LOAD(ra, chunk_ptr(0))
    __builtin_amdgcn_sched_barrier(0);
    PYGAT_X3_LOAD(rb, chunk_ptr(1))
    __builtin_amdgcn_sched_barrier(0);
    PYGAT_X3_LOAD(rc, chunk_ptr(2))
    __builtin_amdgcn_sched_barrier(0);
    for (int c = 0; c < total; c += 4) {
      PYGAT_X3_LOAD(rd, chunk_ptr(c + 3))
      PYGAT_X3_STEP(ra, c)
      PYGAT_X3_LOAD(ra, chunk_ptr(c + 4))
      if (c + 1 < total) PYGAT_X3_STEP(rb, c + 1)
      PYGAT_X3_LOAD(rb, chunk_ptr(c + 5))
      if (c + 2 < total) PYGAT_X3_STEP(rc, c + 2)
      PYGAT_X3_LOAD(rc, chunk_ptr(c + 6))
      if (c + 3 < total) PYGAT_X3_STEP(rd, c + 3)
    }
  } else {
    constexpr int CW = 16 * SPC;
    const int total_q = 8 * my_tiles;
    auto q_row0 = [&](int q) -> int64_t {
      return ((int64_t)blockIdx.x + (int64_t)(q >> 3) * gridDim.x) * 256 + 32 * (q & 7);
    };
    auto tile_ptr = [&](int q, int chunk) -> const float* {
      if (q > total_q - 1) q = total_q - 1;
      int64_t row = q_row0(q) + fr;
      if (row > g.M - 1) row = g.M - 1;
      if (PYGAT_DIAG_K1 & 4) row &= 255;
      return g.A + row * g.lda + chunk * CW + 8 * fh;
    };
    int* q_next = reinterpret_cast<int*>(Asr + (SRF > 0 ? BN : 0));
    const uint32_t q_addr = (uint32_t)(uintptr_t)(__attribute__((address_space(3))) int*)q_next;
    auto grab = [&]() -> int {
      int r;
      asm volatile("ds_add_rtn_u32 %0, %1, %2\n\ts_waitcnt lgkmcnt(0)" : "=v"(r) : "v"(q_addr), "v"(lane == 0 ? 1 : 0) : "memory");
      return r;
    };
#define PYGAT_X3_LOADC(R, P)                                                                  \
  {                                                                                           \
    const float* p__ = (P);                                                                   \
    R##0 = ld4(p__); R##1 = ld4(p__ + 4);                                                     \
    if constexpr (SPC == 2) { R##2 = ld4(p__ + 16); R##3 = ld4(p__ + 20); }                   \
  }
    constexpr int PPG = (4 + NT - 1) / NT;
    constexpr int VPM = ((11 + (SV ? 16 : 0)) * PPG + 8) / 9;
#define PYGAT_X3_PSTEP(SIDX, AC, AN, SRC0, SRC1, CUR0, CUR1, KOFF, KNEXT)                     \
  _Pragma("unroll") for (int i__ = 0; i__ < NT; ++i__) {                                      \
    constexpr int par__ = 0;                                                                  \
    (void)par__;                                                                              \
    const int cur__ = ((SIDX) * NT + i__) & 1;                                                \
    {                                                                                         \
      const int nk__ = (i__ + 1 < NT) ? (KOFF) : (KNEXT), nn__ = (i__ + 1 < NT) ? i__ + 1 : 0; \
      const uint16_t* q__ = Bimg + fr * KP + nk__ + 8 * fh + nn__ * 32 * KP;                  \
      bfP[cur__ ^ 1][0] = *reinterpret_cast<const uint4*>(q__);                               \
      bfP[cur__ ^ 1][1] = *reinterpret_cast<const uint4*>(q__ + IMG);                         \
      bfP[cur__ ^ 1][2] = *reinterpret_cast<const uint4*>(q__ + 2 * IMG);                     \
    }                                                                                         \
    _Pragma("unroll") for (int j__ = i__ * PPG; j__ < (i__ + 1) * PPG && j__ < 4; ++j__) {    \
      float x0__, x1__;                                                                       \
      pair_of((SRC0), (SRC1), j__, x0__, x1__);                                               \
      split_pair(x0__, x1__, AN.h.v[j__], AN.m.v[j__], AN.l.v[j__]);                          \
      if constexpr (SV) if (sv_on) {                                                          \
        pair_of((CUR0), (CUR1), j__, x0__, x1__);                                             \
        const float* us = Us + ((KOFF) + 8 * fh + 2 * j__) * 8;                               \
        PYGAT_X3_SACC(x0__, 0) PYGAT_X3_SACC(x1__, 1)                                         \
      }                                                                                       \
    }                                                                                         \
    acc[i__] = mma9t(AC, bfP[cur__][0], bfP[cur__][1], bfP[cur__][2], acc[i__]);              \
    _Pragma("unroll") for (int m__ = 0; m__ < 9; ++m__) {                                     \
      __builtin_amdgcn_sched_group_barrier(0x008, 1, 0);                                      \
      __builtin_amdgcn_sched_group_barrier(0x002, VPM, 0);                                    \
      if (m__ < (SV ? 7 : 3)) __builtin_amdgcn_sched_group_barrier(0x100, 1, 0);              \
    }                                                                                         \
    __builtin_amdgcn_sched_barrier(0);                                                        \
  }
#if (PYGAT_DIAG_K1 & 16)
#define PYGAT_X3_STAMP(V) { __builtin_amdgcn_sched_barrier(0); V = __builtin_amdgcn_s_memtime(); __builtin_amdgcn_sched_barrier(0); }
#else
#define PYGAT_X3_STAMP(V)
#endif
    unsigned long long st_a = 0, st_b = 0, st_c = 0, st_mfma = 0, st_epi = 0, st_first = 0, st_real = 0, st_n = 0;
    (void)st_n; (void)st_a; (void)st_b; (void)st_c; (void)st_mfma; (void)st_epi; (void)st_first; (void)st_real;
    if ((PYGAT_DIAG_K1 & 16)) st_real = __builtin_amdgcn_s_memrealtime();
#define PYGAT_X3_TILE(FAST)                                                                   \
  {                                                                                           \
    PYGAT_X3_STAMP(st_a)                                                                      \
    PYGAT_X3_LOADC(rd, tile_ptr(qc, 3))                                                       \
    const int qn = __builtin_amdgcn_readfirstlane(qn_v);                                      \
    if constexpr (SPC == 2) {                                                                 \
      PYGAT_X3_PSTEP(0, afA, afB, ra2, ra3, ra0, ra1, 0, 16)                                  \
      PYGAT_X3_PSTEP(1, afB, afA, rb0, rb1, ra2, ra3, 16, 32)                                 \
      PYGAT_X3_LOADC(ra, tile_ptr(qn, 0))                                                     \
      PYGAT_X3_PSTEP(2, afA, afB, rb2, rb3, rb0, rb1, 32, 48)                                 \
      PYGAT_X3_PSTEP(3, afB, afA, rc0, rc1, rb2, rb3, 48, 64)                                 \
      PYGAT_X3_LOADC(rb, tile_ptr(qn, 1))                                                     \
      PYGAT_X3_PSTEP(4, afA, afB, rc2, rc3, rc0, rc1, 64, 80)                                 \
      PYGAT_X3_PSTEP(5, afB, afA, rd0, rd1, rc2, rc3, 80, 96)                                 \
      PYGAT_X3_LOADC(rc, tile_ptr(qn, 2))                                                     \
      PYGAT_X3_PSTEP(6, afA, afB, rd2, rd3, rd0, rd1, 96, 112)                                \
      PYGAT_X3_PSTEP(7, afB, afA, ra0, ra1, rd2, rd3, 112, 0)                                 \
    } else {                                                                                  \
      PYGAT_X3_PSTEP(0, afA, afB, rb0, rb1, ra0, ra1, 0, 16)                                  \
      PYGAT_X3_LOADC(ra, tile_ptr(qn, 0))                                                     \
      PYGAT_X3_PSTEP(1, afB, afA, rc0, rc1, rb0, rb1, 16, 32)                                 \
      PYGAT_X3_LOADC(rb, tile_ptr(qn, 1))                                                     \
      PYGAT_X3_PSTEP(2, afA, afB, rd0, rd1, rc0, rc1, 32, 48)                                 \
      PYGAT_X3_LOADC(rc, tile_ptr(qn, 2))                                                     \
      PYGAT_X3_PSTEP(3, afB, afA, ra0, ra1, rd0, rd1, 48, 0)                                  \
    }                                                                                         \
    PYGAT_X3_STAMP(st_b)                                                                      \
    store_tile(q_row0(qc), FAST);                                                             \
    qc = qn;                                                                                  \
    qn_v = grab();                                                                            \
    PYGAT_X3_STAMP(st_c)                                                                      \
    if ((PYGAT_DIAG_K1 & 16)) { if (!st_first) st_first = st_a; st_mfma += st_b - st_a; st_epi += st_c - st_b; ++st_n; }   \
  }
    int qc = __builtin_amdgcn_readfirstlane(grab());
    int qn_v = grab();
    PYGAT_X3_LOADC(ra, tile_ptr(qc, 0))
    __builtin_amdgcn_sched_barrier(0);
    PYGAT_X3_LOADC(rb, tile_ptr(qc, 1))
    __builtin_amdgcn_sched_barrier(0);
    PYGAT_X3_LOADC(rc, tile_ptr(qc, 2))
    __builtin_amdgcn_sched_barrier(0);
    Frag3 afA = split8v(ra0, ra1), afB;
    uint4 bfP[2][3];
    {
      const uint16_t* q__ = Bimg + fr * KP + 8 * fh;
      bfP[0][0] = *reinterpret_cast<const uint4*>(q__);
      bfP[0][1] = *reinterpret_cast<const uint4*>(q__ + IMG);
      bfP[0][2] = *reinterpret_cast<const uint4*>(q__ + 2 * IMG);
    }
    const int64_t last_base = ((int64_t)blockIdx.x + (int64_t)(my_tiles - 1) * gridDim.x) * 256;
    int full_last = (int)((g.M - last_base) / 32);
    full_last = full_last < 0 ? 0 : (full_last > 8 ? 8 : full_last);
    constexpr bool FASTABLE = SRF == 0 || ((NT * 32 / (SRF > 0 ? SRF : 32)) % 4) == 0;
    const int fast_q = (!FASTABLE || (g.N % 32) != 0 || !g.vec_out || !g.lds_rows || (SRF > 0 && !g.s_vec)) ? 0 : 8 * (my_tiles - 1) + full_last;
    if (qc < fast_q) {
      PYGAT_X3_TILE(std::true_type{})
      while (qc < fast_q) PYGAT_X3_TILE(std::true_type{})
    }
    while (qc < total_q) PYGAT_X3_TILE(std::false_type{})
#if (PYGAT_DIAG_K1 & 16)
    if (lane == 0 && blockIdx.x < 2048) {
      unsigned long long* o = k1_stamps + ((int64_t)blockIdx.x * 8 + w) * 8;
      o[0] = st_c - st_first; o[1] = st_mfma; o[2] = st_epi; o[3] = st_n;
      o[4] = st_entry; o[5] = st_real; o[6] = __builtin_amdgcn_s_memrealtime(); o[7] = 0;
    }
#endif
#undef PYGAT_X3_STAMP
#undef PYGAT_X3_LOADC
#undef PYGAT_X3_TILE
#undef PYGAT_X3_PSTEP
  }
#undef PYGAT_X3_LOAD
#undef PYGAT_X3_SACC
#undef PYGAT_X3_SACC8
#undef PYGAT_X3_BREAD
#undef PYGAT_X3_STEP
#undef PYGAT_X3_BODY
}

template <bool TB, int SM, int SPC>
static hipError_t launch_smallk_x3(const SmallKArgs& g, int NT, dim3 grid, size_t lds, hipStream_t st) {
  int dev = -1;
  (void)hipGetDevice(&dev);
#define PYGAT_X3_LAUNCH(n)                                                                                \
  case n: {                                                                                               \
    static bool attr_set[64] = {};    \
    if (dev < 0 || dev >= 64 || !attr_set[dev]) {                                                         \
      (void)hipFuncSetAttribute(reinterpret_cast<const void*>(&gemm_smallk_x3_kernel<TB, n, SM, SPC>),    \
                                hipFuncAttributeMaxDynamicSharedMemorySize, 160 * 1024);                  \
      if (dev >= 0 && dev < 64) attr_set[dev] = true;                                                     \
    }                                                                                                     \
    hipLaunchKernelGGL((gemm_smallk_x3_kernel<TB, n, SM, SPC>), grid, dim3(512), lds, st, g);             \
  } break;
  switch (NT) {
    PYGAT_X3_LAUNCH(1)
    PYGAT_X3_LAUNCH(2)
    PYGAT_X3_LAUNCH(3)
    PYGAT_X3_LAUNCH(4)
    default:
    PYGAT_X3_LAUNCH(5)
  }
#undef PYGAT_X3_LAUNCH
  return hipGetLastError();
}

template <int SPC>
static hipError_t launch_smallk_x3_sv(const SmallKArgs& g, int NT, dim3 grid, size_t lds, hipStream_t st) {
  int dev = -1;
  (void)hipGetDevice(&dev);
#define PYGAT_X3_LAUNCH(n)                                                                                \
  {                                                                                                       \
    static bool attr_set[64] = {};                                                                        \
    if (dev < 0 || dev >= 64 || !attr_set[dev]) {                                                         \
      (void)hipFuncSetAttribute(reinterpret_cast<const void*>(&gemm_smallk_x3_kernel<false, n, 1, SPC>),  \
                                hipFuncAttributeMaxDynamicSharedMemorySize, 160 * 1024);                  \
      if (dev >= 0 && dev < 64) attr_set[dev] = true;                                                     \
    }                                                                                                     \
    hipLaunchKernelGGL((gemm_smallk_x3_kernel<false, n, 1, SPC>), grid, dim3(512), lds, st, g);           \
  }
  if (NT == 1) PYGAT_X3_LAUNCH(1) else PYGAT_X3_LAUNCH(2)
#undef PYGAT_X3_LAUNCH
  return hipGetLastError();
}

int try_gemm_smallk_x3(const SmallKArgs& g_in, int NT, dim3 grid, hipStream_t st) {
  SmallKArgs g = g_in;
  const size_t lds = (size_t)3 * (32 * NT) * (g.K + 8) * sizeof(uint16_t) + (g.svec ? (size_t)g.K * 8 * sizeof(float) : 0) +
                     (g.sr_a ? (size_t)32 * NT * sizeof(float) : 0) + 16;
  const size_t lds_patches = (size_t)8 * 32 * 36 * sizeof(float);
  g.vec_out = 1;
  for (int q = 0; q < g.out.nseg; ++q) {
    if ((g.out.col_start[q] % 4) != 0) return 0;
    if ((g.out.col_start[q] % 32) != 0 || (g.out.ld[q] % 4) != 0 || !aligned16(g.out.ptr[q])) g.vec_out = 0;
  }
  g.lds_rows = (PYGAT_K1_LDS_ROWS && g.vec_out && lds + lds_patches <= 150 * 1024) ? 1 : 0;
  g.s_vec = (g.s_out && aligned16(g.s_out) && (g.s_ld % 4) == 0 && g.sr_fp > 0 && ((32 * NT / g.sr_fp) % 4) == 0) ? 1 : 0;
  if (lds > 150 * 1024 || (g.svec && NT == 5)) return 0;
  const size_t ldsz = lds + (g.lds_rows ? lds_patches : 0);
  constexpr bool generic = false;
  const int spc = (generic || g.accumulate || g.svec || (NT == 5 && g.K == 128)) ? 0 : (g.K == 128 ? 2 : (g.K == 64 ? 1 : 0));
  hipError_t e;
  if (g.sr_a) {
    if (spc == 0 || g.transB || g.svec || (g.sr_fp != 8 && g.sr_fp != 16) || (g.N % (32 * NT)) != 0) return 0;
    if (spc == 2) e = g.sr_fp == 16 ? launch_smallk_x3<false, 16, 2>(g, NT, grid, ldsz, st) : launch_smallk_x3<false, 8, 2>(g, NT, grid, ldsz, st);
    else e = g.sr_fp == 16 ? launch_smallk_x3<false, 16, 1>(g, NT, grid, ldsz, st) : launch_smallk_x3<false, 8, 1>(g, NT, grid, ldsz, st);
  } else if (g.svec) {
    const int spc_sv = (NT <= 2 && !g.accumulate) ? (g.K == 128 ? 2 : (g.K == 64 ? 1 : 0)) : 0;
    e = spc_sv == 2 ? launch_smallk_x3_sv<2>(g, NT, grid, ldsz, st)
                    : (spc_sv == 1 ? launch_smallk_x3_sv<1>(g, NT, grid, ldsz, st) : launch_smallk_x3<false, 1, 0>(g, NT, grid, ldsz, st));
  } else if (g.transB) {
    e = spc == 2 ? launch_smallk_x3<true, 0, 2>(g, NT, grid, ldsz, st)
                 : (spc == 1 ? launch_smallk_x3<true, 0, 1>(g, NT, grid, ldsz, st) : launch_smallk_x3<true, 0, 0>(g, NT, grid, ldsz, st));
  } else {
    e = spc == 2 ? launch_smallk_x3<false, 0, 2>(g, NT, grid, ldsz, st)
                 : (spc == 1 ? launch_smallk_x3<false, 0, 1>(g, NT, grid, ldsz, st) : launch_smallk_x3<false, 0, 0>(g, NT, grid, ldsz, st));
  }
  if (e != hipSuccess) {
    set_error("gemm_smallk_x3: %s", hipGetErrorString(e));
    return PYGAT_EHIP;
  }
  return 1;
}

int try_project_x3(int n, int Fin, int H, int Fp, const float* X, int64_t ldx, const float* Wcat, int64_t ldw, float* Wh,
                   float* s, const float* a_pad, bool split, hipStream_t st) {
  const int R = H * Fp;
  if (!split || !a_pad || (Fp != 8 && Fp != 16) || (R % 32) != 0 || (Fin != 64 && Fin != 128) || n < 8192) return 0;
  if (!aligned16(X) || (ldx % 4) != 0) return 0;
  const int nt_r = R / 32;
  if (nt_r > 4 && (nt_r % 4) != 0) return 0;
  const int NT = nt_r <= 4 ? nt_r : 4;
  SmallKArgs g;
  g.M = n; g.N = R; g.K = Fin; g.A = X; g.lda = ldx; g.B = Wcat; g.ldb = ldw; g.accumulate = 0;
  g.out.nseg = 1; g.out.col_start[0] = 0; g.out.col_start[1] = R; g.out.ptr[0] = Wh; g.out.ld[0] = R;
  g.svec = nullptr; g.sv_ld = 0; g.sv_n = 0; g.s_out = s; g.s_ld = H;
  g.tiles_m = (int)cdiv(n, 256); g.transB = 0; g.sr_a = a_pad; g.sr_fp = Fp;
  const int tiles_n = R / (32 * NT);
  int gx = 256 / tiles_n;
  if (gx < 1) gx = 1;
  if (gx > g.tiles_m) gx = g.tiles_m;
  return try_gemm_smallk_x3(g, NT, dim3((unsigned)gx, (unsigned)tiles_n, 1), st);
}


constexpr int TNX_RS = 10;
constexpr int TNX_IMG = 128 * TNX_RS;
constexpr int TNX_STAGE = 6 * TNX_IMG;
__device__ __forceinline__ uint4 ld_frag(const uint32_t* p) {
  const uint2 a = *reinterpret_cast<const uint2*>(p), b = *reinterpret_cast<const uint2*>(p + 2);
  return make_uint4(a.x, a.y, b.x, b.y);
}

__global__ __launch_bounds__(256) void gemm_tn_x3_kernel(TnArgs g) {
  extern __shared__ __attribute__((aligned(16))) uint32_t lds_tn[];
  const int tid = threadIdx.x, lane = tid & 63, w = tid >> 6;
  const int fr = lane & 31, fh = lane >> 5;
  const int m0 = blockIdx.y * 128, n0 = blockIdx.z * 128;
  const int64_t kbeg = (int64_t)blockIdx.x * g.k_per_split;
  const int64_t kend = (kbeg + g.k_per_split < g.K) ? kbeg + g.k_per_split : g.K;
  const int nsteps = (int)((kend - kbeg + 15) / 16);
  const int kp = tid & 7, c4 = tid >> 3;
  const float* la = g.A + ((m0 + 4 * c4 + 3 < g.M) ? m0 + 4 * c4 : 0);
  const float* lb = g.B + ((n0 + 4 * c4 + 3 < g.N) ? n0 + 4 * c4 : 0);
#define PYGAT_TNL_LOAD(R, STEP)                                                               \
  {                                                                                           \
    const int64_t k__ = kbeg + 16 * (int64_t)(STEP) + 2 * kp;    \
    int64_t k0__ = k__ < kend ? k__ : kend - 1, k1__ = k__ + 1 < kend ? k__ + 1 : kend - 1;   \
    if (PYGAT_DIAG_K1 & 4) { k0__ &= 255; k1__ &= 255; }    \
    R##a0 = ld4(la + k0__ * g.lda); R##a1 = ld4(la + k1__ * g.lda);                           \
    R##b0 = ld4(lb + k0__ * g.ldb); R##b1 = ld4(lb + k1__ * g.ldb);                           \
    R##z0 = k__ < kend ? 1.f : 0.f; R##z1 = k__ + 1 < kend ? 1.f : 0.f;                       \
  }
#define PYGAT_TNL_PUT(IMGBASE, X0, X1, COL)                                                   \
  {                                                                                           \
    uint32_t h__, m__, l__;                                                                   \
    split_pair((X0), (X1), h__, m__, l__);                                                    \
    uint32_t* q__ = (IMGBASE) + (4 * c4 + (COL)) * TNX_RS + kp;                               \
    q__[0] = h__; q__[TNX_IMG] = m__; q__[2 * TNX_IMG] = l__;                                 \
  }
#define PYGAT_TNL_PUTA(R, STAGE, C, CMP)                                                       \
  PYGAT_TNL_PUT(lds_tn + (STAGE) * TNX_STAGE, R##a0.CMP * R##z0, R##a1.CMP * R##z1, C)
#define PYGAT_TNL_PUTB(R, STAGE, C, CMP)                                                       \
  PYGAT_TNL_PUT(lds_tn + (STAGE) * TNX_STAGE + 3 * TNX_IMG, R##b0.CMP, R##b1.CMP, C)
#define PYGAT_TNL_SPLIT(R, STAGE)                                                             \
  PYGAT_TNL_PUTA(R, STAGE, 0, x) PYGAT_TNL_PUTA(R, STAGE, 1, y) PYGAT_TNL_PUTA(R, STAGE, 2, z) PYGAT_TNL_PUTA(R, STAGE, 3, w) \
  PYGAT_TNL_PUTB(R, STAGE, 0, x) PYGAT_TNL_PUTB(R, STAGE, 1, y) PYGAT_TNL_PUTB(R, STAGE, 2, z) PYGAT_TNL_PUTB(R, STAGE, 3, w)
  f32x16 acc[2][2];
#pragma unroll
  for (int i = 0; i < 2; ++i)
#pragma unroll
    for (int j = 0; j < 2; ++j)
#pragma unroll
      for (int r = 0; r < 16; ++r) acc[i][j][r] = 0.f;
  const uint32_t* fa = lds_tn + (64 * (w >> 1) + fr) * TNX_RS + 4 * fh;
  const uint32_t* fb = lds_tn + 3 * TNX_IMG + (64 * (w & 1) + fr) * TNX_RS + 4 * fh;
#define PYGAT_TNL_READ(STAGE)                                                                 \
  uint4 fq[4][3];                                                                             \
  {                                                                                           \
    const uint32_t* a__ = fa + (STAGE) * TNX_STAGE;                                           \
    const uint32_t* b__ = fb + (STAGE) * TNX_STAGE;                                           \
    _Pragma("unroll") for (int p = 0; p < 3; ++p) {                                           \
      fq[0][p] = ld_frag(a__ + p * TNX_IMG);                                                  \
      fq[1][p] = ld_frag(a__ + p * TNX_IMG + 32 * TNX_RS);                                    \
      fq[2][p] = ld_frag(b__ + p * TNX_IMG);                                                  \
      fq[3][p] = ld_frag(b__ + p * TNX_IMG + 32 * TNX_RS);                                    \
    }                                                                                         \
  }
#define PYGAT_TNL_QUARTER(TM, TN, PUT0, PUT1)                                                 \
  {                                                                                           \
    PUT0 PUT1                                                                                 \
    Frag3 af__;                                                                               \
    af__.h = __builtin_bit_cast(U4, fq[TM][0]); af__.m = __builtin_bit_cast(U4, fq[TM][1]);   \
    af__.l = __builtin_bit_cast(U4, fq[TM][2]);                                               \
    acc[TM][TN] = mma9(af__, fq[2 + TN][0], fq[2 + TN][1], fq[2 + TN][2], acc[TM][TN]);       \
    _Pragma("unroll") for (int m__ = 0; m__ < 9; ++m__) {                                     \
      __builtin_amdgcn_sched_group_barrier(0x008, 1, 0);                                      \
      __builtin_amdgcn_sched_group_barrier(0x002, 3, 0);                                      \
      if (m__ < 6) __builtin_amdgcn_sched_group_barrier(0x200, 1, 0);                         \
    }                                                                                         \
    __builtin_amdgcn_sched_barrier(0);                                                        \
  }
#define PYGAT_TNL_STEP(RSPLIT, RLOAD, I)                                                      \
  {                                                                                           \
    PYGAT_TNL_LOAD(RLOAD, (I) + 3)                                                            \
    PYGAT_TNL_READ((I) & 1)                                                                   \
    __builtin_amdgcn_sched_barrier(0);                                                        \
    const int sn__ = ((I) + 1) & 1;    \
    PYGAT_TNL_QUARTER(0, 0, PYGAT_TNL_PUTA(RSPLIT, sn__, 0, x), PYGAT_TNL_PUTA(RSPLIT, sn__, 1, y)) \
    PYGAT_TNL_QUARTER(0, 1, PYGAT_TNL_PUTA(RSPLIT, sn__, 2, z), PYGAT_TNL_PUTA(RSPLIT, sn__, 3, w)) \
    PYGAT_TNL_QUARTER(1, 0, PYGAT_TNL_PUTB(RSPLIT, sn__, 0, x), PYGAT_TNL_PUTB(RSPLIT, sn__, 1, y)) \
    PYGAT_TNL_QUARTER(1, 1, PYGAT_TNL_PUTB(RSPLIT, sn__, 2, z), PYGAT_TNL_PUTB(RSPLIT, sn__, 3, w)) \
    __syncthreads();                                                                          \
  }
  float4 r0a0, r0a1, r0b0, r0b1, r1a0, r1a1, r1b0, r1b1, r2a0, r2a1, r2b0, r2b1;
  float r0z0, r0z1, r1z0, r1z1, r2z0, r2z1;
  PYGAT_TNL_LOAD(r0, 0)
  __builtin_amdgcn_sched_barrier(0);
  PYGAT_TNL_LOAD(r1, 1)
  __builtin_amdgcn_sched_barrier(0);
  PYGAT_TNL_LOAD(r2, 2)
  __builtin_amdgcn_sched_barrier(0);
  PYGAT_TNL_SPLIT(r0, 0)
  __syncthreads();
  for (int i = 0; i < nsteps; i += 3) {
    PYGAT_TNL_STEP(r1, r0, i)
    PYGAT_TNL_STEP(r2, r1, i + 1)
    PYGAT_TNL_STEP(r0, r2, i + 2)
  }
#undef PYGAT_TNL_LOAD
#undef PYGAT_TNL_PUT
#undef PYGAT_TNL_SPLIT
#undef PYGAT_TNL_QUARTER
#undef PYGAT_TNL_PUTA
#undef PYGAT_TNL_PUTB
#undef PYGAT_TNL_READ
#undef PYGAT_TNL_STEP
  float* base = g.ws + (int64_t)blockIdx.x * g.M * g.N;
  const int wm0 = m0 + 64 * (w >> 1), wn0 = n0 + 64 * (w & 1);
#pragma unroll
  for (int tm = 0; tm < 2; ++tm)
#pragma unroll
    for (int tn = 0; tn < 2; ++tn) {
      const int col = wn0 + 32 * tn + fr;
      if (col >= g.N) continue;
#pragma unroll
      for (int r = 0; r < 16; ++r) {
        const int row = wm0 + 32 * tm + (r & 3) + 8 * (r >> 2) + 4 * fh;
        if (row < g.M) base[(int64_t)row * g.N + col] = acc[tm][tn][r];
      }
    }
}

#ifndef PYGAT_TN_WIDE
#define PYGAT_TN_WIDE 1
#endif
typedef float f32x4 __attribute__((ext_vector_type(4)));
constexpr int TNW_RS = 16;
constexpr int TNW_IMG = 128 * TNW_RS;
constexpr int TNW_STAGE = 6 * TNW_IMG;
template <class TA_, class TB_>
__device__ __forceinline__ f32x4 mfma16_bf16(const TA_& a, const TB_& b, f32x4 c) {
  return __builtin_amdgcn_mfma_f32_16x16x32_bf16(__builtin_bit_cast(bf16x8, a), __builtin_bit_cast(bf16x8, b), c, 0, 0, 0);
}

__global__ __launch_bounds__(512) void gemm_tn_x3w_kernel(TnArgs g) {
  extern __shared__ __attribute__((aligned(16))) uint32_t lds_tw[];
  const int tid = threadIdx.x, lane = tid & 63, w = tid >> 6;
  const int fi = lane & 15, fq = lane >> 4;
  const int m0 = blockIdx.y * 128, n0 = blockIdx.z * 128;
  const int64_t kbeg = (int64_t)blockIdx.x * g.k_per_split;
  const int64_t kend = (kbeg + g.k_per_split < g.K) ? kbeg + g.k_per_split : g.K;
  const int nsteps = (int)((kend - kbeg + 31) / 32);
  const int kp = tid & 7, c4 = (tid >> 3) & 31, pr = kp + 8 * (tid >> 8);
  const float* la = g.A + ((m0 + 4 * c4 + 3 < g.M) ? m0 + 4 * c4 : 0);
  const float* lb = g.B + ((n0 + 4 * c4 + 3 < g.N) ? n0 + 4 * c4 : 0);
  uint32_t* const wbase = lds_tw + (4 * c4) * TNW_RS + (pr & 3);
  const int wq = pr >> 2, wrot = 2 * (c4 & 1);
#define PYGAT_TWL_LOAD(R, STEP)                                                               \
  {                                                                                           \
    const int64_t k__ = kbeg + 32 * (int64_t)(STEP) + 2 * pr;    \
    const int64_t k0__ = k__ < kend ? k__ : kend - 1, k1__ = k__ + 1 < kend ? k__ + 1 : kend - 1;   \
    R##a0 = ld4(la + k0__ * g.lda); R##a1 = ld4(la + k1__ * g.lda);                           \
    R##b0 = ld4(lb + k0__ * g.ldb); R##b1 = ld4(lb + k1__ * g.ldb);                           \
    R##z0 = k__ < kend ? 1.f : 0.f; R##z1 = k__ + 1 < kend ? 1.f : 0.f;                       \
  }
#define PYGAT_TWL_PUT(IMGBASE, X0, X1, COL)                                                   \
  {                                                                                           \
    uint32_t h__, m__, l__;                                                                   \
    split_pair((X0), (X1), h__, m__, l__);                                                    \
    uint32_t* q__ = (IMGBASE) + (wbase - lds_tw) + (COL) * TNW_RS + 4 * ((wq + wrot + ((COL) >> 1)) & 3);   \
    q__[0] = h__; q__[TNW_IMG] = m__; q__[2 * TNW_IMG] = l__;                                 \
  }
#define PYGAT_TWL_PUTA(R, STAGE, C, CMP)                                                       \
  PYGAT_TWL_PUT(lds_tw + (STAGE) * TNW_STAGE, R##a0.CMP * R##z0, R##a1.CMP * R##z1, C)
#define PYGAT_TWL_PUTB(R, STAGE, C, CMP)                                                       \
  PYGAT_TWL_PUT(lds_tw + (STAGE) * TNW_STAGE + 3 * TNW_IMG, R##b0.CMP, R##b1.CMP, C)
#define PYGAT_TWL_SPLIT(R, STAGE)                                                             \
  PYGAT_TWL_PUTA(R, STAGE, 0, x) PYGAT_TWL_PUTA(R, STAGE, 1, y) PYGAT_TWL_PUTA(R, STAGE, 2, z) PYGAT_TWL_PUTA(R, STAGE, 3, w) \
  PYGAT_TWL_PUTB(R, STAGE, 0, x) PYGAT_TWL_PUTB(R, STAGE, 1, y) PYGAT_TWL_PUTB(R, STAGE, 2, z) PYGAT_TWL_PUTB(R, STAGE, 3, w)
  f32x4 acc[2][4];
#pragma unroll
  for (int i = 0; i < 2; ++i)
#pragma unroll
    for (int j = 0; j < 4; ++j)
#pragma unroll
      for (int r = 0; r < 4; ++r) acc[i][j][r] = 0.f;
  const int fso = 4 * ((fq + (fi >> 1)) & 3);
  const uint32_t* fa = lds_tw + (32 * (w >> 1) + fi) * TNW_RS + fso;
  const uint32_t* fb = lds_tw + 3 * TNW_IMG + (64 * (w & 1) + fi) * TNW_RS + fso;
#define PYGAT_TWL_READ(STAGE)                                                                 \
  uint4 fqa[2][3], fqb[4][3];                                                                 \
  {                                                                                           \
    const uint32_t* a__ = fa + (STAGE) * TNW_STAGE;                                           \
    const uint32_t* b__ = fb + (STAGE) * TNW_STAGE;                                           \
    _Pragma("unroll") for (int p = 0; p < 3; ++p) {                                           \
      fqa[0][p] = *reinterpret_cast<const uint4*>(a__ + p * TNW_IMG);                         \
      fqa[1][p] = *reinterpret_cast<const uint4*>(a__ + p * TNW_IMG + 16 * TNW_RS);           \
      _Pragma("unroll") for (int t = 0; t < 4; ++t)                                           \
        fqb[t][p] = *reinterpret_cast<const uint4*>(b__ + p * TNW_IMG + 16 * t * TNW_RS);     \
    }                                                                                         \
  }
#define PYGAT_TWL_GROUP(TM, TN, PUT0)                                                         \
  {                                                                                           \
    PUT0                                                                                      \
    f32x4 c__ = acc[TM][TN];                                                                  \
    c__ = mfma16_bf16(fqa[TM][2], fqb[TN][2], c__); c__ = mfma16_bf16(fqa[TM][2], fqb[TN][1], c__);   \
    c__ = mfma16_bf16(fqa[TM][1], fqb[TN][2], c__); c__ = mfma16_bf16(fqa[TM][2], fqb[TN][0], c__);   \
    c__ = mfma16_bf16(fqa[TM][0], fqb[TN][2], c__); c__ = mfma16_bf16(fqa[TM][1], fqb[TN][1], c__);   \
    c__ = mfma16_bf16(fqa[TM][1], fqb[TN][0], c__); c__ = mfma16_bf16(fqa[TM][0], fqb[TN][1], c__);   \
    c__ = mfma16_bf16(fqa[TM][0], fqb[TN][0], c__);                                           \
    acc[TM][TN] = c__;                                                                        \
    _Pragma("unroll") for (int m__ = 0; m__ < 9; ++m__) {                                     \
      __builtin_amdgcn_sched_group_barrier(0x008, 1, 0);                                      \
      __builtin_amdgcn_sched_group_barrier(0x002, 2, 0);                                      \
      if (m__ >= 3 && m__ < 6) __builtin_amdgcn_sched_group_barrier(0x200, 1, 0);             \
    }                                                                                         \
    __builtin_amdgcn_sched_barrier(0);                                                        \
  }
#define PYGAT_TWL_STEP(RSPLIT, RLOAD, I)                                                      \
  {                                                                                           \
    PYGAT_TWL_LOAD(RLOAD, (I) + 3)                                                            \
    PYGAT_TWL_READ((I) & 1)                                                                   \
    __builtin_amdgcn_sched_barrier(0);                                                        \
    const int sn__ = ((I) + 1) & 1;    \
    PYGAT_TWL_GROUP(0, 0, PYGAT_TWL_PUTA(RSPLIT, sn__, 0, x)) PYGAT_TWL_GROUP(0, 1, PYGAT_TWL_PUTA(RSPLIT, sn__, 1, y)) \
    PYGAT_TWL_GROUP(0, 2, PYGAT_TWL_PUTA(RSPLIT, sn__, 2, z)) PYGAT_TWL_GROUP(0, 3, PYGAT_TWL_PUTA(RSPLIT, sn__, 3, w)) \
    PYGAT_TWL_GROUP(1, 0, PYGAT_TWL_PUTB(RSPLIT, sn__, 0, x)) PYGAT_TWL_GROUP(1, 1, PYGAT_TWL_PUTB(RSPLIT, sn__, 1, y)) \
    PYGAT_TWL_GROUP(1, 2, PYGAT_TWL_PUTB(RSPLIT, sn__, 2, z)) PYGAT_TWL_GROUP(1, 3, PYGAT_TWL_PUTB(RSPLIT, sn__, 3, w)) \
    __syncthreads();                                                                          \
  }
  float4 r0a0, r0a1, r0b0, r0b1, r1a0, r1a1, r1b0, r1b1, r2a0, r2a1, r2b0, r2b1;
  float r0z0, r0z1, r1z0, r1z1, r2z0, r2z1;
  PYGAT_TWL_LOAD(r0, 0)
  __builtin_amdgcn_sched_barrier(0);
  PYGAT_TWL_LOAD(r1, 1)
  __builtin_amdgcn_sched_barrier(0);
  PYGAT_TWL_LOAD(r2, 2)
  __builtin_amdgcn_sched_barrier(0);
  PYGAT_TWL_SPLIT(r0, 0)
  __syncthreads();
  for (int i = 0; i < nsteps; i += 3) {
    PYGAT_TWL_STEP(r1, r0, i)
    PYGAT_TWL_STEP(r2, r1, i + 1)
    PYGAT_TWL_STEP(r0, r2, i + 2)
  }
#undef PYGAT_TWL_LOAD
#undef PYGAT_TWL_PUT
#undef PYGAT_TWL_SPLIT
#undef PYGAT_TWL_GROUP
#undef PYGAT_TWL_PUTA
#undef PYGAT_TWL_PUTB
#undef PYGAT_TWL_READ
#undef PYGAT_TWL_STEP
  float* base = g.ws + (int64_t)blockIdx.x * g.M * g.N;
  const int wm0 = m0 + 32 * (w >> 1), wn0 = n0 + 64 * (w & 1);
#pragma unroll
  for (int tm = 0; tm < 2; ++tm)
#pragma unroll
    for (int tn = 0; tn < 4; ++tn) {
      const int col = wn0 + 16 * tn + fi;
      if (col >= g.N) continue;
#pragma unroll
      for (int r = 0; r < 4; ++r) {
        const int row = wm0 + 16 * tm + 4 * fq + r;
        if (row < g.M) base[(int64_t)row * g.N + col] = acc[tm][tn][r];
      }
    }
}

int try_gemm_tn_x3(const TnArgs& g, int splits, hipStream_t st) {
  if (g.B2 || g.M <= 64 || g.N <= 64 || (g.k_per_split % 16) != 0) return 0;
  if (!aligned16(g.A) || !aligned16(g.B) || (g.lda % 4) != 0 || (g.ldb % 4) != 0 || (g.M % 4) != 0 || (g.N % 4) != 0) return 0;
  int dev = -1;
  (void)hipGetDevice(&dev);
#if PYGAT_TN_WIDE
  {
    const int tiles = (int)(cdiv(g.M, 128) * cdiv(g.N, 128));
    int sw = splits;
    if (sw * tiles > 256) sw = 256 / tiles > 0 ? 256 / tiles : 1;
    TnArgs gw = g;
    gw.k_per_split = cdiv(cdiv(g.K, sw), 96) * 96;
    sw = (int)cdiv(g.K, gw.k_per_split);
    constexpr size_t ldsw = 2 * TNW_STAGE * sizeof(uint32_t);
    static bool attr_w[64] = {};
    if (dev < 0 || dev >= 64 || !attr_w[dev]) {
      (void)hipFuncSetAttribute(reinterpret_cast<const void*>(&gemm_tn_x3w_kernel), hipFuncAttributeMaxDynamicSharedMemorySize, (int)ldsw);
      if (dev >= 0 && dev < 64) attr_w[dev] = true;
    }
    hipLaunchKernelGGL(gemm_tn_x3w_kernel, dim3((unsigned)sw, (unsigned)cdiv(g.M, 128), (unsigned)cdiv(g.N, 128)), dim3(512), ldsw, st, gw);
    hipError_t ew = hipGetLastError();
    if (ew != hipSuccess) {
      set_error("gemm_tn_x3w: %s", hipGetErrorString(ew));
      return PYGAT_EHIP;
    }
    return sw;
  }
#endif
  dim3 grid((unsigned)splits, (unsigned)cdiv(g.M, 128), (unsigned)cdiv(g.N, 128));
  constexpr size_t lds = 2 * TNX_STAGE * sizeof(uint32_t);
  static bool attr_set[64] = {};
  if (dev < 0 || dev >= 64 || !attr_set[dev]) {
    (void)hipFuncSetAttribute(reinterpret_cast<const void*>(&gemm_tn_x3_kernel), hipFuncAttributeMaxDynamicSharedMemorySize, (int)lds);
    if (dev >= 0 && dev < 64) attr_set[dev] = true;
  }
// ... 163 lines not shown
#pragma unroll
        for (int b = 0; b < 2; ++b)
#pragma unroll
          for (int r = 0; r < 16; ++r) { acc2[a][b][r] += acc[a][b][r]; acc[a][b][r] = 0.f; }
    }
  }
  const int wm0 = m0 + 64 * (w >> 1), wn0 = n0 + 64 * (w & 1);
#pragma unroll
  for (int tm = 0; tm < 2; ++tm)
#pragma unroll
    for (int tn = 0; tn < 2; ++tn) {
      const int col = wn0 + 32 * tn + fr;
      if (col >= g.N) continue;
      float* base;
      int64_t ld;
      if (g.ws) { base = g.ws + (int64_t)blockIdx.x * g.M * g.N + col; ld = g.N; }
      else if (g.cb.lw < 62) { base = g.out.ptr[0] + blk_off(col, g.cb); ld = g.out.ld[0]; }
      else base = out_segment(g.out, col, ld);
      const bool add = !g.ws && g.accumulate;
#pragma unroll
      for (int r = 0; r < 16; ++r) {
        const int row = wm0 + 32 * tm + (r & 3) + 8 * (r >> 2) + 4 * fh;
        if (row < g.M) {
          float* p = base + (int64_t)row * ld;
          const float v = acc[tm][tn][r] + acc2[tm][tn][r];
          *p = add ? *p + v : v;
        }
      }
    }
}

#ifndef PYGAT_X3G_WIDE
#define PYGAT_X3G_WIDE 1
#endif
struct X3gwSlot {
  float4 a0, a1, b0, b1;
};

template <bool KCA, bool KCB>
__global__ __launch_bounds__(512) void gemm_x3gw_kernel(X3gArgs g) {
  extern __shared__ __attribute__((aligned(16))) uint32_t lds_xw[];
  const int tid = threadIdx.x, lane = tid & 63, w = tid >> 6;
  const int fi = lane & 15, fq = lane >> 4;
  const int m0 = blockIdx.y * 128, n0 = blockIdx.z * 128;
  const int64_t kbeg = (int64_t)blockIdx.x * g.k_per_split;
  const int64_t kend = (kbeg + g.k_per_split < g.K) ? kbeg + g.k_per_split : g.K;
  const int nsteps = (int)((kend - kbeg + 31) / 32);
  const int kp = tid & 7, c4 = (tid >> 3) & 31, pr = kp + 8 * (tid >> 8);
  const int lq = (tid >> 4) & 3, lrow = (tid & 15) + 16 * (tid >> 6);
  const float* la;
  const float* lb;
  if constexpr (KCA) la = g.A + (int64_t)((m0 + lrow < g.M) ? m0 + lrow : g.M - 1) * g.lda;
  else la = g.A + blk_off((m0 + 4 * c4 < g.M) ? m0 + 4 * c4 : 0, g.ab);
  if constexpr (KCB) lb = g.B + (int64_t)((n0 + lrow < g.N) ? n0 + lrow : g.N - 1) * g.ldb;
  else lb = g.B + ((n0 + 4 * c4 < g.N) ? n0 + 4 * c4 : 0);

  auto load = [&](X3gwSlot& r, int step) {
    const int st = step < nsteps ? step : nsteps - 1;
    const int64_t ks = kbeg + 32 * (int64_t)st;
    {
      const int64_t k = ks + 2 * pr;
      const int64_t k0 = k < kend ? k : kend - 1, k1 = k + 1 < kend ? k + 1 : kend - 1;
      if constexpr (!KCA) { r.a0 = ld4(la + k0 * g.lda); r.a1 = ld4(la + k1 * g.lda); }
      if constexpr (!KCB) { r.b0 = ld4(lb + k0 * g.ldb); r.b1 = ld4(lb + k1 * g.ldb); }
    }
    {
      const int64_t k = ks + 8 * lq;
      const int64_t k0 = k < kend ? k : kend - 4, k1 = k + 4 < kend ? k + 4 : kend - 4;
      if constexpr (KCA) { r.a0 = ld4(la + blk_off(k0, g.ab)); r.a1 = ld4(la + blk_off(k1, g.ab)); }
      if constexpr (KCB) { r.b0 = ld4(lb + k0); r.b1 = ld4(lb + k1); }
    }
  };
  auto put_strided = [&](uint32_t* img, const float4& x0, const float4& x1, float z0, float z1, auto q_tag) {
    constexpr int Q = decltype(q_tag)::value;
    const float p0 = Q == 0 ? x0.x : Q == 1 ? x0.y : Q == 2 ? x0.z : x0.w;
    const float p1 = Q == 0 ? x1.x : Q == 1 ? x1.y : Q == 2 ? x1.z : x1.w;
    uint32_t h, m, l;
    split_pair(p0 * z0, p1 * z1, h, m, l);
    uint32_t* d = img + (4 * c4 + Q) * TNW_RS + 4 * (((pr >> 2) + 2 * (c4 & 1) + (Q >> 1)) & 3) + (pr & 3);
    d[0] = h; d[TNW_IMG] = m; d[2 * TNW_IMG] = l;
  };
  auto put_contig = [&](uint32_t* img, const float4& x0, const float4& x1, float z0, float z1, uint32_t (&ph)[4], uint32_t (&pm)[4],
                        uint32_t (&pl)[4], auto q_tag) {
    constexpr int Q = decltype(q_tag)::value;
    const float p0 = Q == 0 ? x0.x * z0 : Q == 1 ? x0.z * z0 : Q == 2 ? x1.x * z1 : x1.z * z1;
    const float p1 = Q == 0 ? x0.y * z0 : Q == 1 ? x0.w * z0 : Q == 2 ? x1.y * z1 : x1.w * z1;
    split_pair(p0, p1, ph[Q], pm[Q], pl[Q]);
    if constexpr (Q == 3) {
      uint32_t* d = img + lrow * TNW_RS + 4 * ((lq + (lrow >> 1)) & 3);
      *reinterpret_cast<uint4*>(d) = make_uint4(ph[0], ph[1], ph[2], ph[3]);
      *reinterpret_cast<uint4*>(d + TNW_IMG) = make_uint4(pm[0], pm[1], pm[2], pm[3]);
      *reinterpret_cast<uint4*>(d + 2 * TNW_IMG) = make_uint4(pl[0], pl[1], pl[2], pl[3]);
    }
  };
  uint32_t pah[4], pam[4], pal[4], pbh[4], pbm[4], pbl[4];
  auto put_a = [&](const X3gwSlot& r, int stage, int step_of_r, auto q_tag) {
    uint32_t* img = lds_xw + stage * TNW_STAGE;
    const int64_t ks = kbeg + 32 * (int64_t)step_of_r;
    if constexpr (KCA) {
      const int64_t k = ks + 8 * lq;
      put_contig(img, r.a0, r.a1, k < kend ? 1.f : 0.f, k + 4 < kend ? 1.f : 0.f, pah, pam, pal, q_tag);
    } else {
      const int64_t k = ks + 2 * pr;
      put_strided(img, r.a0, r.a1, k < kend ? 1.f : 0.f, k + 1 < kend ? 1.f : 0.f, q_tag);
    }
  };
  auto put_b = [&](const X3gwSlot& r, int stage, auto q_tag) {
    uint32_t* img = lds_xw + stage * TNW_STAGE + 3 * TNW_IMG;
    if constexpr (KCB) put_contig(img, r.b0, r.b1, 1.f, 1.f, pbh, pbm, pbl, q_tag);
    else put_strided(img, r.b0, r.b1, 1.f, 1.f, q_tag);
  };

  f32x4 acc[2][4], acc2[2][4];
#pragma unroll
  for (int i = 0; i < 2; ++i)
#pragma unroll
    for (int j = 0; j < 4; ++j)
#pragma unroll
      for (int r = 0; r < 4; ++r) { acc[i][j][r] = 0.f; acc2[i][j][r] = 0.f; }
  const int fso = 4 * ((fq + (fi >> 1)) & 3);
  const uint32_t* fa = lds_xw + (32 * (w >> 1) + fi) * TNW_RS + fso;
  const uint32_t* fb = lds_xw + 3 * TNW_IMG + (64 * (w & 1) + fi) * TNW_RS + fso;

  using Q0 = std::integral_constant<int, 0>;
  using Q1 = std::integral_constant<int, 1>;
  using Q2 = std::integral_constant<int, 2>;
  using Q3 = std::integral_constant<int, 3>;
  auto step = [&](const X3gwSlot& rs, X3gwSlot& rl, int i) {
    load(rl, i + 2);
    uint4 fqa[2][3], fqb[4][3];
    {
      const uint32_t* a_ = fa + (i & 1) * TNW_STAGE;
      const uint32_t* b_ = fb + (i & 1) * TNW_STAGE;
#pragma unroll
      for (int p = 0; p < 3; ++p) {
        fqa[0][p] = *reinterpret_cast<const uint4*>(a_ + p * TNW_IMG);
        fqa[1][p] = *reinterpret_cast<const uint4*>(a_ + p * TNW_IMG + 16 * TNW_RS);
#pragma unroll
        for (int t = 0; t < 4; ++t) fqb[t][p] = *reinterpret_cast<const uint4*>(b_ + p * TNW_IMG + 16 * t * TNW_RS);
      }
    }
    __builtin_amdgcn_sched_barrier(0);
    const int sn = (i + 1) & 1;
    auto group = [&](auto tm_tag, auto tn_tag) {
      constexpr int TM = decltype(tm_tag)::value, TN = decltype(tn_tag)::value;
      f32x4 c = acc[TM][TN];
      c = mfma16_bf16(fqa[TM][2], fqb[TN][2], c); c = mfma16_bf16(fqa[TM][2], fqb[TN][1], c);
      c = mfma16_bf16(fqa[TM][1], fqb[TN][2], c); c = mfma16_bf16(fqa[TM][2], fqb[TN][0], c);
      c = mfma16_bf16(fqa[TM][0], fqb[TN][2], c); c = mfma16_bf16(fqa[TM][1], fqb[TN][1], c);
      c = mfma16_bf16(fqa[TM][1], fqb[TN][0], c); c = mfma16_bf16(fqa[TM][0], fqb[TN][1], c);
      c = mfma16_bf16(fqa[TM][0], fqb[TN][0], c);
      acc[TM][TN] = c;
#pragma unroll
      for (int m = 0; m < 9; ++m) {
        __builtin_amdgcn_sched_group_barrier(0x008, 1, 0);
        __builtin_amdgcn_sched_group_barrier(0x002, 2, 0);
        if (m >= 3 && m < 6) __builtin_amdgcn_sched_group_barrier(0x200, 1, 0);
      }
      __builtin_amdgcn_sched_barrier(0);
    };
    put_a(rs, sn, i + 1, Q0{}); group(Q0{}, Q0{});
    put_a(rs, sn, i + 1, Q1{}); group(Q0{}, Q1{});
    put_a(rs, sn, i + 1, Q2{}); group(Q0{}, Q2{});
    put_a(rs, sn, i + 1, Q3{}); group(Q0{}, Q3{});
    put_b(rs, sn, Q0{}); group(Q1{}, Q0{});
    put_b(rs, sn, Q1{}); group(Q1{}, Q1{});
    put_b(rs, sn, Q2{}); group(Q1{}, Q2{});
    put_b(rs, sn, Q3{}); group(Q1{}, Q3{});
    __syncthreads();
  };

  X3gwSlot r0, r1;
  load(r0, 0);
  __builtin_amdgcn_sched_barrier(0);
  load(r1, 1);
  __builtin_amdgcn_sched_barrier(0);
  put_a(r0, 0, 0, Q0{}); put_a(r0, 0, 0, Q1{}); put_a(r0, 0, 0, Q2{}); put_a(r0, 0, 0, Q3{});
  put_b(r0, 0, Q0{}); put_b(r0, 0, Q1{}); put_b(r0, 0, Q2{}); put_b(r0, 0, Q3{});
  __syncthreads();
  for (int i = 0; i < nsteps; i += 2) {
    step(r1, r0, i);
    if (i + 1 < nsteps) step(r0, r1, i + 1);
    if (((i >> 1) & 1) == 1) {
#pragma unroll
      for (int a = 0; a < 2; ++a)
#pragma unroll
        for (int b = 0; b < 4; ++b)
#pragma unroll
          for (int r = 0; r < 4; ++r) { acc2[a][b][r] += acc[a][b][r]; acc[a][b][r] = 0.f; }
    }
  }
  const int wm0 = m0 + 32 * (w >> 1), wn0 = n0 + 64 * (w & 1);
#pragma unroll
  for (int tm = 0; tm < 2; ++tm)
#pragma unroll
    for (int tn = 0; tn < 4; ++tn) {
      const int col = wn0 + 16 * tn + fi;
      if (col >= g.N) continue;
      float* base;
      int64_t ld;
      if (g.ws) { base = g.ws + (int64_t)blockIdx.x * g.M * g.N + col; ld = g.N; }
      else if (g.cb.lw < 62) { base = g.out.ptr[0] + blk_off(col, g.cb); ld = g.out.ld[0]; }
      else base = out_segment(g.out, col, ld);
      const bool add = !g.ws && g.accumulate;
#pragma unroll
      for (int r = 0; r < 4; ++r) {
        const int row = wm0 + 16 * tm + 4 * fq + r;
        if (row < g.M) {
          float* p = base + (int64_t)row * ld;
          const float v = acc[tm][tn][r] + acc2[tm][tn][r];
          *p = add ? *p + v : v;
        }
      }
    }
}

int try_gemm_x3g(int transA, int transB, int M, int N, int64_t K, const float* A, int64_t lda, const float* B, int64_t ldb,
                 const pygat_out_segments* out, int accumulate, int splits, int64_t k_per_split, float* ws, hipStream_t st,
                 ColBlocks ab, ColBlocks cb, int* splits_used) {
  if (splits_used) *splits_used = splits;
  if (M < 64 || N <= 64 || K < 32) return 0;
  if (!aligned16(A) || !aligned16(B) || (lda % 4) != 0 || (ldb % 4) != 0) return 0;
  const bool kca = !transA, kcb = transB != 0;
  if ((kca || kcb) && ((K % 4) != 0 || (k_per_split % 4) != 0)) return 0;
  if ((!kca && (M % 4) != 0 && lda < (M + 3) / 4 * 4) || (!kcb && (N % 4) != 0 && ldb < (N + 3) / 4 * 4)) return 0;
  if (splits > 1 && (!ws || (k_per_split % 16) != 0)) return 0;
  X3gArgs g;
  g.M = M; g.N = N; g.K = K; g.A = A; g.lda = lda; g.B = B; g.ldb = ldb;
  g.k_per_split = splits > 1 ? k_per_split : K;
  g.ws = splits > 1 ? ws : nullptr;
  g.out = *out; g.accumulate = accumulate;
  g.ab = ab; g.cb = cb;
  if (cb.lw < 62 && splits > 1) return 0;
#if PYGAT_X3G_WIDE
  {
    const int tiles = (int)(cdiv(M, 128) * cdiv(N, 128));
    int sw = splits;
    if (sw > 1) {
      if (sw * tiles > 256) sw = 256 / tiles > 1 ? 256 / tiles : 1;
      if (sw > 1) {
        g.k_per_split = cdiv(cdiv(K, sw), 32) * 32;
        sw = (int)cdiv(K, g.k_per_split);
      }
      if (sw <= 1) { sw = 1; g.k_per_split = K; g.ws = nullptr; }
    }
    if (splits_used) *splits_used = sw;
    constexpr size_t ldsw = 2 * TNW_STAGE * sizeof(uint32_t);
    dim3 gridw((unsigned)sw, (unsigned)cdiv(M, 128), (unsigned)cdiv(N, 128));
#define PYGAT_X3GW_LAUNCH(KA, KB)                                                                                         \
  do {                                                                                                                    \
    int dev = -1;                                                                                                         \
    (void)hipGetDevice(&dev);                                                                                             \
    static bool attr_set[64] = {};                                                                                        \
    if (dev < 0 || dev >= 64 || !attr_set[dev]) {                                                                         \
      (void)hipFuncSetAttribute(reinterpret_cast<const void*>(&gemm_x3gw_kernel<KA, KB>),                                 \
                                hipFuncAttributeMaxDynamicSharedMemorySize, (int)ldsw);                                   \
      if (dev >= 0 && dev < 64) attr_set[dev] = true;                                                                     \
    }                                                                                                                     \
    hipLaunchKernelGGL((gemm_x3gw_kernel<KA, KB>), gridw, dim3(512), ldsw, st, g);                                        \
  } while (0)
    if (kca && kcb) PYGAT_X3GW_LAUNCH(true, true);
    else if (kca) PYGAT_X3GW_LAUNCH(true, false);
    else if (kcb) PYGAT_X3GW_LAUNCH(false, true);
    else PYGAT_X3GW_LAUNCH(false, false);
#undef PYGAT_X3GW_LAUNCH
    hipError_t ew = hipGetLastError();
    if (ew != hipSuccess) {
      set_error("gemm_x3gw: %s", hipGetErrorString(ew));
      return PYGAT_EHIP;
    }
    return 1;
  }
#endif
  dim3 grid((unsigned)splits, (unsigned)cdiv(M, 128), (unsigned)cdiv(N, 128));
  constexpr size_t lds = 2 * TNX_STAGE * sizeof(uint32_t);
#define PYGAT_X3G_LAUNCH(KA, KB)                                                                                          \
  do {                                                                                                                    \
    int dev = -1;                                                                                                         \
    (void)hipGetDevice(&dev);                                                                                             \
    static bool attr_set[64] = {};                                                                                        \
    if (dev < 0 || dev >= 64 || !attr_set[dev]) {                                                                         \
      (void)hipFuncSetAttribute(reinterpret_cast<const void*>(&gemm_x3g_kernel<KA, KB>),                                  \
                                hipFuncAttributeMaxDynamicSharedMemorySize, (int)lds);                                    \
      if (dev >= 0 && dev < 64) attr_set[dev] = true;                                                                     \
    }                                                                                                                     \
    hipLaunchKernelGGL((gemm_x3g_kernel<KA, KB>), grid, dim3(256), lds, st, g);                                           \
  } while (0)
  if (kca && kcb) PYGAT_X3G_LAUNCH(true, true);
  else if (kca) PYGAT_X3G_LAUNCH(true, false);
  else if (kcb) PYGAT_X3G_LAUNCH(false, true);
  else PYGAT_X3G_LAUNCH(false, false);
#undef PYGAT_X3G_LAUNCH
  hipError_t e = hipGetLastError();
  if (e != hipSuccess) {
    set_error("gemm_x3g: %s", hipGetErrorString(e));
    return PYGAT_EHIP;
  }
  return 1;
}

int footprint_gemm_x3(int which, int* regs, int* scratch) {
  hipFuncAttributes at;
  const void* fn = which == 0 ? reinterpret_cast<const void*>(&gemm_tn_x3w_kernel)
                              : reinterpret_cast<const void*>(&gemm_x3gw_kernel<true, false>);
  const hipError_t e = hipFuncGetAttributes(&at, fn);
  if (e != hipSuccess) {
    (void)hipGetLastError();
    set_error("kernel_footprint: %s", hipGetErrorString(e));
    return PYGAT_EHIP;
  }
  *regs = at.numRegs; *scratch = (int)at.localSizeBytes;
  return PYGAT_OK;
}

}

#if (PYGAT_DIAG_K1 & 16)
extern "C" __attribute__((visibility("default"))) int pygat_diag_k1_stamps(unsigned long long* host, int words) {
  const int all = 2048 * 8 * 8;
  if (!host || words < all) return -1;
  if (hipDeviceSynchronize() != hipSuccess) return -2;
  return hipMemcpyFromSymbol(host, HIP_SYMBOL(pygat::k1_stamps), sizeof(unsigned long long) * all) == hipSuccess ? all : -3;
}
#endif
```

pygat_amd/ops.py:

```python
from __future__ import annotations

import ctypes as C
import threading
from typing import Optional, Sequence

import torch

from . import _lib
from ._lib import lib, check, padded_width
from .config import config as _config
from .graph import CSRGraph, slot_edges_for


def _stream() -> int:
    return torch.cuda.current_stream().cuda_stream


class KernelTimer:

    def __init__(self):
        self.spans = []

    def times_ms(self):
        out = {}
        for name, a, b in self.spans:
            out.setdefault(name, []).append(a.elapsed_time(b))
        return out


TIMER: Optional[KernelTimer] = None

TWO_GATHER_BACKWARD: Optional[bool] = _config.two_gather_backward

BACKWARD_FLAVOUR: Optional[str] = _config.backward


def two_gather_backward(row_floats: int) -> bool:
    return TWO_GATHER_BACKWARD if TWO_GATHER_BACKWARD is not None else row_floats < 64


def backward_flavour(row_floats: int) -> str:
    if BACKWARD_FLAVOUR:
        if BACKWARD_FLAVOUR not in ("rowlocal", "rowsum", "two-gather"):
            raise ValueError(f"PYGAT_BACKWARD={BACKWARD_FLAVOUR!r}: expected rowlocal, rowsum or two-gather")
        return BACKWARD_FLAVOUR
    if TWO_GATHER_BACKWARD is not None:
        return "two-gather" if TWO_GATHER_BACKWARD else "rowsum"
    return "rowlocal" if row_floats <= 256 else "rowsum"


BWD_WINDOW_FLOATS: Optional[int] = None

DA_IN_K4 = _config.da_in_k4
DA_MIN_BYTES = 32 << 20


RENUMBER = _config.renumber
RENUMBER_MIN_BYTES = 160 << 20
RENUMBER_MIN_BYTES_TAIL = 48 << 20
TAIL = _config.tail
TAIL_MIN_SHARE = 0.05


def head_group(N: int, H: int, Fo: int) -> int:
    if BWD_WINDOW_FLOATS is None:
        return lib.pygat_head_group(N, H, Fo)
    Fp = padded_width(Fo)
    return H if H * Fp <= BWD_WINDOW_FLOATS else max(1, min(H, BWD_WINDOW_FLOATS // Fp))


class _span:
    def __init__(self, name):
        self.name = name

    def __enter__(self):
        if TIMER is not None:
            self.a = torch.cuda.Event(enable_timing=True)
            self.a.record()

    def __exit__(self, *exc):
        if TIMER is not None:
            b = torch.cuda.Event(enable_timing=True)
            b.record()
            TIMER.spans.append((self.name, self.a, b))
        return False


def _ptr(t):
    return None if t is None else t.data_ptr()


_side = {}


def _side_stream(dev) -> "torch.cuda.Stream":
    key = torch.device(dev).index
    if key not in _side:
        _side[key] = torch.cuda.Stream(device=dev)
    return _side[key]


_K1_SLAB = _config.k1_split_min_k
OVERLAP_BACKWARD = _config.overlap_backward


def _segments(cols_ptr_ld) -> _lib.OutSegments:
    seg = _lib.OutSegments()
    seg.nseg = len(cols_ptr_ld)
    c = 0
    for k, (ncol, t, ld) in enumerate(cols_ptr_ld):
        seg.col_start[k] = c
        seg.ptr[k] = t.data_ptr()
        seg.ld[k] = ld
        c += ncol
    seg.col_start[len(cols_ptr_ld)] = c
    return seg


def _x3g_takes(transA: bool, transB: bool, M: int, N: int, K: int) -> bool:
    kca, kcb = not transA, transB
    return M >= 64 and N > 64 and K >= 32 and ((K % 4) == 0 or not (kca or kcb))


def _split_k(M: int, N: int, K: int, streamed_k: bool = False, mode: Optional[str] = None, transB: bool = False) -> int:
    nt = -(-N // 32)
    if streamed_k and K >= 4096 and M * N <= 512 * 512 and (mode or get_gemm_mode()) == "split-bf16" and M > 64 and N > 64 \
            and M % 4 == 0 and N % 4 == 0:
        tiles = -(-M // 128) * -(-N // 128)
        return max(1, min(512 // tiles, K // 256)) if tiles < 512 else 1
    if streamed_k and K >= 4096 and M * N <= 512 * 512:
        tiles = -(-M // 128) * -(-N // (32 * min(nt, 5 if nt == 5 else 4)))
        return max(1, min(256 // tiles, K // 256)) if tiles < 256 else 1
    if (mode or get_gemm_mode()) == "split-bf16" and _x3g_takes(streamed_k, transB, M, N, K) and not (not streamed_k and K <= 256 and M >= 8192):
        tiles = -(-M // 128) * -(-N // 128)
        return 1 if tiles >= 96 else max(1, min(K // 256, 512 // tiles))
    bn = 32 * (nt if nt <= 5 else 4)
    tiles = -(-M // 128) * -(-N // bn)
    by_traffic = int(0.125 * K * (M + N) / (M * N))
    want = (512 if streamed_k else 256) // tiles
    return max(1, min(256, 1024 // tiles, K // 256, max(by_traffic, want))) if tiles < 1024 else 1


GEMM_MODES = {"split-bf16": 0, "fp32-mfma": 1}
_mode_tls = threading.local()


def _mode_code(mode: Optional[str] = None) -> int:
    mode = mode or getattr(_mode_tls, "mode", None)
    return -1 if mode is None else GEMM_MODES[mode]


def set_gemm_mode(mode: Optional[str]) -> None:
    if mode is not None and mode not in GEMM_MODES:
        raise ValueError(f"gemm mode {mode!r}: expected one of {sorted(GEMM_MODES)}")
    _mode_tls.mode = mode


def get_gemm_mode() -> str:
    code = _mode_code()
    if code < 0:
        code = lib.pygat_default_gemm_mode()
    return next(k for k, v in GEMM_MODES.items() if v == code)


class gemm_mode:

    def __init__(self, mode: Optional[str]):
        self.mode = mode

    def __enter__(self):
        self.prev = getattr(_mode_tls, "mode", None)
        set_gemm_mode(self.mode)

    def __exit__(self, *exc):
        _mode_tls.mode = self.prev
        return False


def gemm(transA: bool, transB: bool, M: int, N: int, K: int, A: torch.Tensor, lda: int, B: torch.Tensor,
         ldb: int, segments, accumulate: bool = False, split_k: Optional[int] = None, mode: Optional[str] = None,
         a_blocks=None, c_blocks=None) -> None:
    if c_blocks is not None:
        split_k = 1
    if split_k is None:
        split_k = _split_k(M, N, K, streamed_k=transA and not transB, mode=mode, transB=transB)
    ws = None
    if split_k > 1:
        ws = torch.empty(lib.pygat_gemm_workspace_bytes(M, N, split_k) // 4, dtype=torch.float32, device=A.device)
    seg = _segments(segments)
    if a_blocks is None and c_blocks is None:
        check(lib.pygat_gemm_f32(int(transA), int(transB), M, N, K, A.data_ptr(), lda, B.data_ptr(), ldb,
                                 C.byref(seg), int(accumulate), split_k, _ptr(ws), _mode_code(mode), _stream()), "gemm_f32")
    else:
        check(lib.pygat_gemm_f32_blocked(int(transA), int(transB), M, N, K, A.data_ptr(), lda,
                                         None if a_blocks is None else C.byref(a_blocks), B.data_ptr(), ldb, C.byref(seg),
                                         None if c_blocks is None else C.byref(c_blocks), int(accumulate), split_k, _ptr(ws),
                                         _mode_code(mode), _stream()), "gemm_f32_blocked")


class _Level:

    def __init__(self, x, H, Fo, skip):
        self.blocks = None if x.dim() == 2 else _lib.ColBlocks(int(x.shape[2]), int(x.shape[1]) * int(x.shape[2]))
        self.N, self.Fin = (x.shape[0], x.shape[1]) if x.dim() == 2 else (x.shape[1], x.shape[0] * x.shape[2])
        self.ldx = self.Fin if x.dim() == 2 else int(x.shape[2])
        self.H, self.Fo, self.skip = H, Fo, skip
        self.Fp = padded_width(Fo)
        self.R = H * self.Fp
        self.hg = head_group(self.N, H, Fo)
        self.ldw = -(-(self.R * (2 if skip else 1) + 2 * H) // 4) * 4
        self.ts = 0

    def xb(self):
        return None if self.blocks is None else C.byref(self.blocks)

    def gp_windows(self):
        for h0 in range(0, self.H, self.hg):
            hc = min(self.hg, self.H - h0)
            yield h0 * self.Fp, hc * self.Fp, h0 * (self.Fp + 4)

    def gp_col(self, h):
        h0 = (h // self.hg) * self.hg
        return h0 * (self.Fp + 4) + (h - h0) * self.Fp


def _in_features(x) -> int:
    return x.shape[1] if x.dim() == 2 else x.shape[0] * x.shape[2]


def blocked_input_ok(x3: torch.Tensor) -> bool:
    w = int(x3.shape[2])
    return x3.dim() == 3 and x3.is_cuda and x3.dtype == torch.float32 and w >= 16 and (w & (w - 1)) == 0


class GATLevelFn(torch.autograd.Function):

    @staticmethod
    def forward(ctx, x, W, a, Wskip, graph: CSRGraph, alpha: float, concat: bool, bwd_heads=None, pipeline=None):
        if not x.is_cuda:
            raise RuntimeError("pygat_amd: inputs must be on the GPU; the hot path has no CPU fallback")
        ctx.in_dtypes = (x.dtype, W.dtype, a.dtype, None if Wskip is None else Wskip.dtype)
        x = x.contiguous().float()
        W = W.contiguous().float(); a = a.contiguous().float()
        H, Fin, Fo = W.shape
        if _in_features(x) != Fin or a.shape != (H, 2 * Fo):
            raise ValueError(f"shape mismatch: x {tuple(x.shape)}, W {tuple(W.shape)}, a {tuple(a.shape)}")
        skip = Wskip is not None
        if skip:
            Wskip = Wskip.contiguous().float()

        def pack(Wcat, ldw, a_pad, st):
            check(lib.pygat_pack_params(H, Fin, Fo, W.data_ptr(), a.data_ptr(), _ptr(Wskip), Wcat.data_ptr(), ldw,
                                        a_pad.data_ptr(), st), "pack_params")
        return _level_forward(ctx, tuple(ctx.needs_input_grad[:4]), x, H, Fo, skip, pack, graph, alpha, concat, bwd_heads, pipeline)

    @staticmethod
    def backward(ctx, G):
        dx, dW, da, dWs = _level_backward(ctx, G)
        cast = lambda g_, k: g_ if g_ is None or g_.dtype == ctx.in_dtypes[k] else g_.to(ctx.in_dtypes[k])
        return (cast(dx, 0), cast(dW, 1), cast(da, 2), cast(dWs, 3), None, None, None, None, None)


PAD_K = _config.pad_k
MAX_HEAD_TABLE = 16


class GATLevelHeadsFn(torch.autograd.Function):

    @staticmethod
    def forward(ctx, x, graph: CSRGraph, alpha: float, concat: bool, pipeline, H: int, skip: bool, xs, *params):
        if not x.is_cuda:
            raise RuntimeError("pygat_amd: inputs must be on the GPU; the hot path has no CPU fallback")
        Ws, As = params[:H], params[H:2 * H]
        Ss = params[2 * H:3 * H] if skip else ()
        Fin, Fo = Ws[0].shape
        ctx.in_dtype_x = x.dtype
        ctx.param_shapes = [tuple(p.shape) for p in params]
        ctx.param_dtypes = [p.dtype for p in params]
        x = x.contiguous().float()
        Ws = [w.contiguous().float() for w in Ws]; As = [v.contiguous().float() for v in As]; Ss = [w.contiguous().float() for w in Ss]
        if _in_features(x) != Fin or any(w.shape != (Fin, Fo) for w in Ws) or any(v.numel() != 2 * Fo for v in As):
            raise ValueError(f"shape mismatch: x {tuple(x.shape)}, W {tuple(Ws[0].shape)}, a {tuple(As[0].shape)}")
        PT = C.c_void_p * H
        wp, ap = PT(*[w.data_ptr() for w in Ws]), PT(*[v.data_ptr() for v in As])
        sp = PT(*[w.data_ptr() for w in Ss]) if skip else None

        def pack(Wcat, ldw, a_pad, st):
            check(lib.pygat_pack_params_heads(H, Fin, Fo, wp, ap, sp, Wcat.data_ptr(), ldw, a_pad.data_ptr(), st), "pack_params_heads")
        n = ctx.needs_input_grad
        need = (n[0], any(n[8:8 + H]), any(n[8 + H:8 + 2 * H]), skip and any(n[8 + 2 * H:8 + 3 * H]))
        ctx.H, ctx.skip = H, skip
        return _level_forward(ctx, need, x, H, Fo, skip, pack, graph, alpha, concat, None, pipeline, xs=xs)

    @staticmethod
    def backward(ctx, G):
        dx, dW, da, dWs = _level_backward(ctx, G)
        H = ctx.H
        if dx is not None and dx.dtype != ctx.in_dtype_x:
            dx = dx.to(ctx.in_dtype_x)
        outs = []
        for k in range(H):
            outs.append(None if dW is None else dW[k])
        for k in range(H):
            outs.append(None if da is None else da[k].reshape(ctx.param_shapes[H + k]))
        if ctx.skip:
            for k in range(H):
                outs.append(None if dWs is None else dWs[k])
        outs = [g_ if g_ is None or g_.dtype == dt else g_.to(dt) for g_, dt in zip(outs, ctx.param_dtypes)]
        return (dx, None, None, None, None, None, None, None) + tuple(outs)


def _level_forward(ctx, need, x, H, Fo, skip, pack, graph: CSRGraph, alpha: float, concat: bool, bwd_heads, pipeline, xs=None):
    if x.dim() == 3 and not blocked_input_ok(x):
        raise ValueError(f"column-blocked input {tuple(x.shape)}: blocks must be a power of two >= 16 floats wide (float32, GPU)")
    L = _Level(x, H, Fo, skip)
    Fin = L.Fin
    if L.N != graph.n:
        raise ValueError(f"x has {L.N} rows but the graph has {graph.n} nodes")
    if L.blocks is not None:
        xs = None
    user_row = None
    tail = None
    single_out = (not concat) and H == 1
    if (RENUMBER and not need[0] and xs is None and pipeline is None and x.dim() == 2 and (concat or single_out)
            and graph.user_row is None and not graph.degree_sorted and L.N * L.R * 4 >= min(RENUMBER_MIN_BYTES, RENUMBER_MIN_BYTES_TAIL)
            and not torch.cuda.is_current_stream_capturing()):
        from .features import permuted_rows
        g_int, to_user, _ = graph.degree_ordered()
        worth = L.N * L.R * 4 >= RENUMBER_MIN_BYTES
        if not worth and TAIL and concat and graph.symmetric:
            t = g_int.fwd.self_loop_tail(slot_edges_for(L.R, g_int.slot_edges))
            worth = t is not None and L.N - t[0] >= TAIL_MIN_SHARE * L.N
        xp = permuted_rows(x, to_user) if worth else None
        if xp is not None:
            x, graph, user_row = xp, g_int, to_user
    L.ts = slot_edges_for(L.R, graph.slot_edges)
    L.mode = get_gemm_mode()
    dev, f32 = x.device, torch.float32
    need_grad = any(need)
    ctx.need = need
    with torch.cuda.device(dev):
        st = _stream()
        Wcat = torch.empty(Fin, L.ldw, dtype=f32, device=dev)
        a_pad = torch.empty(H, 2, L.Fp, dtype=f32, device=dev)
        pack(Wcat, L.ldw, a_pad, st)
        Wh = torch.empty(L.N, L.R, dtype=f32, device=dev)
        Sk = torch.empty(L.N, L.R, dtype=f32, device=dev) if skip else None
        s = torch.empty(L.N, H, dtype=f32, device=dev)
        ncols = L.R * (2 if skip else 1) + H
        tiles = -(-L.N // 128) * -(-ncols // 128)
        split_k = max(1, min(-(-384 // tiles), Fin // _K1_SLAB)) if tiles < 256 else 1
        ws = torch.empty(lib.pygat_gemm_workspace_bytes(L.N, ncols, split_k) // 4, dtype=f32, device=dev) \
            if split_k > 1 else None
        if xs is not None and need[0]:
            xs = None
        with _span("k1_project"):
            if xs is not None:
                check(lib.pygat_project_sparse(L.N, Fin, H, Fo, xs.rowptr.data_ptr(), xs.col.data_ptr(), xs.val.data_ptr(),
                                               Wcat.data_ptr(), L.ldw, 0.0, None, 0, None, Wh.data_ptr(), _ptr(Sk), s.data_ptr(),
                                               st), "project_sparse")
            else:
                check(lib.pygat_project_blocked(L.N, Fin, H, Fo, x.data_ptr(), L.ldx, L.xb(), Wcat.data_ptr(), L.ldw, a_pad.data_ptr(),
                                                Wh.data_ptr(), _ptr(Sk), s.data_ptr(), split_k, _ptr(ws), GEMM_MODES[L.mode], st),
                      "project")
        flags = (_lib.F_ELU if concat else 0) | (_lib.F_SKIP if skip else 0)
        single = (not concat) and H == 1
        hattn = torch.empty(L.N, L.R, dtype=f32, device=dev) if (not concat and (need_grad or not single)) else None
        m = torch.empty(L.N, H, dtype=f32, device=dev) if need_grad else None
        Z = torch.empty(L.N, H, dtype=f32, device=dev) if need_grad else None
        flavour = backward_flavour(L.R) if need_grad else None
        aneg = torch.empty(L.N, L.R, dtype=f32, device=dev) if flavour == "rowlocal" else None
        qneg = torch.empty(L.N, H, dtype=f32, device=dev) if flavour == "rowlocal" else None
        out = pipeline[2] if (pipeline is not None and len(pipeline) > 2 and concat) else None
        if out is not None:
            if tuple(out.shape) != (L.N, H * Fo) or out.dtype != f32 or not out.is_contiguous() or out.device != dev:
                raise ValueError(f"pipeline output buffer {tuple(out.shape)}: expected a contiguous float32 [{L.N}, {H * Fo}] on {dev}")
            out = torch.empty(0, dtype=f32, device=dev).set_(out.untyped_storage(), out.storage_offset(), out.shape, out.stride())
        else:
            out = torch.empty(L.N, H * Fo if concat else Fo, dtype=f32, device=dev)
        part = torch.empty(lib.pygat_partials_bytes(graph.nnz, L.ts, H, L.Fp) // 4, dtype=f32,
                           device=dev)
        if (TAIL and graph.degree_sorted and concat and graph.symmetric
                and (not need_grad or (flavour == "rowlocal" and L.hg >= H and bwd_heads is None))):
            t = graph.fwd.self_loop_tail(L.ts)
            if t is not None and L.N - t[0] >= TAIL_MIN_SHARE * L.N:
                tail = (t[0], t[2], t[1])
        chunks = [(graph.fwd.ref(L.ts) if tail is None else tail[1], 0, L.N if tail is None else tail[0])]
        if pipeline is not None and concat and pipeline[0] > 1:
            chunks = (graph.fwd.row_chunks(int(pipeline[0]), L.ts) if tail is None
                      else graph.fwd.row_chunks(int(pipeline[0]), L.ts, nslots=tail[2], row_end=tail[0]))
        phases = len(chunks) > 1 and TIMER is None and bool(lib.pygat_gat_forward_phases_ok(L.N, H, Fo))
        if phases:
            main_s, side_s = torch.cuda.current_stream(dev), _side_stream(dev)

        def k2(gref, fl, stream):
            check(lib.pygat_gat_forward(gref, H, Fo, float(alpha), fl, Wh.data_ptr(), s.data_ptr(),
                                        a_pad.data_ptr(), _ptr(Sk), None, out.data_ptr() if (concat or single) else None,
                                        _ptr(hattn), _ptr(m), _ptr(Z), _ptr(aneg), _ptr(qneg), part.data_ptr(), stream),
                  "gat_forward")
        for c, (gref, r0, r1) in enumerate(chunks):
            if phases:
                k2(gref, flags | _lib.F_MAIN_ONLY, st)
                side_s.wait_stream(main_s)
                with torch.cuda.stream(side_s):
                    k2(gref, flags | _lib.F_FIXUP_ONLY, side_s.cuda_stream)
                    pipeline[1](c, r0, r1, out)
                continue
            with _span("k2_forward"):
                k2(gref, flags, st)
                if tail is not None and c == len(chunks) - 1:
                    check(lib.pygat_gat_forward_tail(tail[0], L.N - tail[0], H, Fo, flags, Wh.data_ptr(), 0, _ptr(Sk), out.data_ptr(),
                                                     _ptr(user_row), _ptr(m), _ptr(Z), _ptr(qneg), st), "gat_forward_tail")
            if pipeline is not None and concat:
                pipeline[1](c, r0, r1 if not (tail is not None and c == len(chunks) - 1) else L.N, out)
        if phases:
            main_s.wait_stream(side_s)
            if tail is not None:
                check(lib.pygat_gat_forward_tail(tail[0], L.N - tail[0], H, Fo, flags, Wh.data_ptr(), 0, _ptr(Sk), out.data_ptr(),
                                                 _ptr(user_row), _ptr(m), _ptr(Z), _ptr(qneg), st), "gat_forward_tail")
                pipeline[1](len(chunks), tail[0], L.N, out)
        if not concat and not single:
            check(lib.pygat_head_mean(L.N, H, Fo, hattn.data_ptr(), _ptr(Sk), out.data_ptr(), st), "head_mean")
    if need_grad:
        ctx.save_for_backward(x, Wcat, a_pad, Wh, s, Sk, out if concat else hattn, m, Z, aneg, qneg)
        ctx.graph, ctx.L, ctx.alpha, ctx.concat, ctx.flags = graph, L, float(alpha), concat, flags
        ctx.user_row = user_row
        ctx.tail = tail
        ctx.xs = xs
        ctx.flavour = flavour
        ctx.bwd_heads = None
        if bwd_heads is not None:
            hb, hr = int(bwd_heads[0]), int(bwd_heads[1])
            if not (0 <= hb and 0 < hr and hb + hr <= H):
                raise ValueError(f"bwd_heads {bwd_heads} outside the {H} heads of the level")
            if skip or need[0]:
                raise ValueError("pygat_amd: bwd_heads supports neither a skip projection nor a gradient into x")
            ctx.bwd_heads = (hb, hr)
    return out

def _level_backward(ctx, G):
    x, Wcat, a_pad, Wh, s, Sk, y, m, Z, aneg, qneg = ctx.saved_tensors
    graph, L, H, Fo = ctx.graph, ctx.L, ctx.L.H, ctx.L.Fo
    dev, f32 = x.device, torch.float32
    G = G.contiguous().float()
    ranged = ctx.bwd_heads is not None
    hb, hr = ctx.bwd_heads if ranged else (0, 0)
    Hb = hr if ranged else H
    with torch.cuda.device(dev):
        st = _stream()
        RW = Hb * (L.Fp + 4)
        GR = torch.empty(L.N, RW, dtype=f32, device=dev)
        ds = torch.empty(L.N, H, dtype=f32, device=dev)
        dt = torch.empty(L.N, H, dtype=f32, device=dev)
        dWh = torch.empty(L.N, L.R, dtype=f32, device=dev)
        part = torch.empty(lib.pygat_partials_bytes(graph.nnz, L.ts, H, L.Fp) // 4, dtype=f32,
                           device=dev)
        rowlocal = ctx.flavour == "rowlocal"
        hgw = lib.pygat_head_group(L.N, Hb, Fo) if (ranged and BWD_WINDOW_FLOATS is None) else (min(L.hg, Hb) if not ranged else head_group(L.N, Hb, Fo))
        tail = getattr(ctx, "tail", None)
        gT = graph.bwd.ref(L.ts) if tail is None else tail[1]
        da_part = None
        if DA_IN_K4 and not ranged and ctx.flavour != "rowsum" and ctx.need[2] and L.N * L.R * 4 >= DA_MIN_BYTES:
            nb = lib.pygat_gat_backward_col_da_bytes(gT, H, Fo, hgw)
            if nb:
                da_part = torch.empty(nb // 4, dtype=f32, device=dev)
        fused_tail = tail is not None and not L.skip
        with _span("k3a_prepare"):
            check(lib.pygat_gat_backward_prepare(tail[0] if fused_tail else L.N, H, Fo, ctx.flags, 0 if ctx.concat else 1, G.data_ptr(),
                                                 y.data_ptr(), _ptr(Sk), s.data_ptr(), m.data_ptr(), Z.data_ptr(),
                                                 GR.data_ptr(), _ptr(aneg), _ptr(qneg), ctx.alpha,
                                                 ds.data_ptr() if rowlocal else None, hb, hr, hgw, _ptr(getattr(ctx, "user_row", None)), st),
                      "gat_backward_prepare")
        two_gather = ctx.flavour == "two-gather"
        if rowlocal:
            with _span("k4_backward_col"):
                check(lib.pygat_gat_backward_col(gT, None, H, Fo, ctx.alpha, Wh.data_ptr(),
                                                 a_pad.data_ptr(), GR.data_ptr(), None, ds.data_ptr(),
                                                 dWh.data_ptr(), dt.data_ptr(), None, part.data_ptr(), _ptr(da_part), hb, hr, hgw, st),
                      "gat_backward_col")
                if fused_tail:
                    check(lib.pygat_gat_backward_tail(tail[0], L.N - tail[0], H, Fo, ctx.flags, G.data_ptr(), y.data_ptr(),
                                                      _ptr(getattr(ctx, "user_row", None)), dWh.data_ptr(), 0, 0, ds.data_ptr(), dt.data_ptr(), st),
                          "gat_backward_tail")
                elif tail is not None:
                    check(lib.pygat_gat_backward_col_tail(tail[0], L.N - tail[0], H, Fo, GR.data_ptr(), dWh.data_ptr(), dt.data_ptr(), st),
                          "gat_backward_col_tail")
        elif two_gather:
            with _span("k3b_row"):
                check(lib.pygat_gat_backward_row(graph.fwd.ref(L.ts), H, Fo, ctx.alpha, Wh.data_ptr(),
                                                 a_pad.data_ptr(), GR.data_ptr(), None, ds.data_ptr(),
                                                 part.data_ptr(), hb, hr, hgw, st), "gat_backward_row")
            with _span("k4_backward_col"):
                check(lib.pygat_gat_backward_col(graph.bwd.ref(L.ts), None, H, Fo, ctx.alpha, Wh.data_ptr(),
                                                 a_pad.data_ptr(), GR.data_ptr(), None, ds.data_ptr(),
                                                 dWh.data_ptr(), dt.data_ptr(), None, part.data_ptr(), _ptr(da_part), hb, hr, hgw, st),
                      "gat_backward_col")
        else:
            dz_t = torch.empty(graph.nnz, H, dtype=f32, device=dev)
            with _span("k4_backward_col"):
                check(lib.pygat_gat_backward_col(graph.bwd.ref(L.ts), None, H, Fo, ctx.alpha, Wh.data_ptr(),
                                                 a_pad.data_ptr(), GR.data_ptr(), None, None,
                                                 dWh.data_ptr(), dt.data_ptr(), dz_t.data_ptr(), part.data_ptr(), None, hb, hr, hgw, st),
                      "gat_backward_col")
            with _span("k3c_rowsum"):
                check(lib.pygat_gat_backward_rowsum(graph.fwd.ref(L.ts), graph.perm_f.data_ptr(), H, Fo,
                                                    dz_t.data_ptr(), ds.data_ptr(), part.data_ptr(), hb, hr, st),
                      "gat_backward_rowsum")
        da = (torch.zeros if ranged else torch.empty)(H, 2 * Fo, dtype=f32, device=dev)
        ws = torch.empty(lib.pygat_agrad_workspace_bytes(H, Fo) // 4, dtype=f32, device=dev)
        rowsum = ctx.flavour == "rowsum"
        xs = getattr(ctx, "xs", None)
        sparse_w = xs is not None and not ranged and (not L.skip or L.hg >= H)
        fold_ds = (rowsum and ctx.need[1] and not ctx.need[0] and not sparse_w
                   and (Hb * L.Fp) % 32 == 0 and L.N >= 4096)
        finish = rowsum and not fold_ds
        fork = OVERLAP_BACKWARD and not finish and TIMER is None and ctx.need[1]
        if fork:
            main, side = torch.cuda.current_stream(), _side_stream(dev)
            side.wait_stream(main)
        if da_part is not None:
            with _span("k5_afold"):
                check(lib.pygat_a_grad_fold(gT, H, Fo, Wh.data_ptr(), ds.data_ptr(), dt.data_ptr(),
                                            da_part.data_ptr(), da.data_ptr(), ws.data_ptr(), hgw,
                                            side.cuda_stream if fork else st), "a_grad_fold")
        else:
            with _span("k5_agrad"):
                check(lib.pygat_a_grad(L.N, H, Fo, Wh.data_ptr(), ds.data_ptr(), dt.data_ptr(), da.data_ptr(),
                                       ws.data_ptr(), a_pad.data_ptr() if finish else None,
                                       dWh.data_ptr() if finish else None, None, hb, hr,
                                       side.cuda_stream if fork else st), "a_grad")
        dW = dWs = dx = None
        if sparse_w and (ctx.need[1] or (L.skip and ctx.need[3])):
            dW = torch.empty(H, L.Fin, Fo, dtype=f32, device=dev)
            want_s = L.skip and ctx.need[3]
            dWs = torch.empty(H, L.Fin, Fo, dtype=f32, device=dev) if want_s else None
            wss = torch.empty(lib.pygat_wgrad_sparse_workspace_bytes(xs.nseg, H, Fo, int(want_s)) // 4 + 4, dtype=f32, device=dev)
            with _span("k5_wgrad"):
                check(lib.pygat_wgrad_sparse(L.N, L.Fin, H, Fo, xs.nseg, xs.colseg.data_ptr(), xs.seg_col.data_ptr(),
                                             xs.seg_begin.data_ptr(), xs.seg_end.data_ptr(), xs.trow.data_ptr(), xs.tval.data_ptr(),
                                             0.0, None, 0, None, dWh.data_ptr(), GR.data_ptr() if want_s else None, RW,
                                             wss.data_ptr(), dW.data_ptr(), _ptr(dWs), st), "wgrad_sparse")
        elif ctx.need[1]:
            split_k = _split_k(L.Fin, Hb * L.Fp + (Hb if fold_ds else 0), L.N, streamed_k=True, mode=L.mode)
            wsw = torch.empty(lib.pygat_wgrad_workspace_bytes(L.Fin, H, Fo, split_k) // 4, dtype=f32, device=dev)
            dW = (torch.zeros if ranged else torch.empty)(H, L.Fin, Fo, dtype=f32, device=dev)
            with _span("k5_wgrad"):
                check(lib.pygat_wgrad_blocked(L.N, L.Fin, H, Fo, x.data_ptr(), L.ldx, L.xb(), dWh.data_ptr(),
                                              ds.data_ptr() if fold_ds else None, a_pad.data_ptr(), dW.data_ptr(), split_k,
                                              wsw.data_ptr(), hb, hr, GEMM_MODES[L.mode], st), "wgrad")
        if L.skip and ctx.need[3] and not sparse_w:
            dSc = torch.empty(L.Fin, L.R, dtype=f32, device=dev)
            for c0, w, g0 in L.gp_windows():
                gemm(True, False, L.Fin, w, L.N, x, L.ldx, GR[:, g0:], RW, [(w, dSc[:, c0:], L.R)], mode=L.mode, a_blocks=L.blocks)
            dWs = torch.empty(H, L.Fin, Fo, dtype=f32, device=dev)
            check(lib.pygat_unpack_wgrad(H, L.Fin, Fo, dSc.data_ptr(), L.R, 0, dWs.data_ptr(), st), "unpack")
        if ctx.need[0]:
            dx = torch.empty(x.shape, dtype=f32, device=dev)
            with _span("k5_xgrad"):
                gemm(False, True, L.N, L.Fin, L.R, dWh, L.R, Wcat, L.ldw, [(L.Fin, dx, L.ldx)], mode=L.mode, c_blocks=L.blocks)
                if L.skip:
                    for c0, w, g0 in L.gp_windows():
                        gemm(False, True, L.N, L.Fin, w, GR[:, g0:], RW, Wcat[:, L.R + c0:], L.ldw,
                             [(L.Fin, dx, L.ldx)], accumulate=True, split_k=1, mode=L.mode, c_blocks=L.blocks)
        if fork:
            main.wait_stream(side)
    return dx, dW, (da if ctx.need[2] else None), dWs


class StackHeads(torch.autograd.Function):

    @staticmethod
    def forward(ctx, H: int, skip: bool, rows: int, *params):
        Ws, As = params[:H], params[H:2 * H]
        Ss = params[2 * H:3 * H] if skip else ()
        dev, f32 = Ws[0].device, torch.float32
        ctx.shapes = [tuple(p.shape) for p in params]
        ctx.H, ctx.skip = H, skip
        ok = Ws[0].is_cuda and H <= MAX_HEAD_TABLE and all(p.dtype == f32 and p.is_contiguous() for p in params)
        pad = rows > 0 and rows != Ws[0].shape[0]
        if not ok:
            grow = (lambda t: torch.nn.functional.pad(t, (0, 0, 0, rows - t.shape[0]))) if pad else (lambda t: t)
            return (torch.stack([grow(w) for w in Ws], 0), torch.stack([q.reshape(-1) for q in As], 0),
                    torch.stack([grow(w) for w in Ss], 0) if skip else None)
        wshape = (rows, *Ws[0].shape[1:]) if pad else tuple(Ws[0].shape)
        W = torch.empty(H, *wshape, dtype=f32, device=dev)
        a = torch.empty(H, As[0].numel(), dtype=f32, device=dev)
        S = None
        if skip:
            S = torch.empty(H, *((rows, *Ss[0].shape[1:]) if pad else Ss[0].shape), dtype=f32, device=dev)
        PT = C.c_void_p * H
        with torch.cuda.device(dev):
            check(lib.pygat_stack_heads_padded(H, Ws[0].numel(), W[0].numel(), As[0].numel(), Ss[0].numel() if skip else 0,
                                               S[0].numel() if skip else 0, PT(*[w.data_ptr() for w in Ws]),
                                               PT(*[v.data_ptr() for v in As]), PT(*[w.data_ptr() for w in Ss]) if skip else None,
                                               W.data_ptr(), a.data_ptr(), _ptr(S), _stream()), "stack_heads")
        return W, a, S

    @staticmethod
    def backward(ctx, dW, da, dS):
        H = ctx.H
        rows_w = ctx.shapes[0][0]
        outs = [None if dW is None else dW[k][:rows_w] for k in range(H)]
        outs += [None if da is None else da[k].reshape(ctx.shapes[H + k]) for k in range(H)]
        if ctx.skip:
            rows_s = ctx.shapes[2 * H][0]
            outs += [None if dS is None else dS[k][:rows_s] for k in range(H)]
        return (None, None, None) + tuple(outs)


def stack_heads(Ws, As, Wskips):
    return StackHeads.apply(len(Ws), Wskips is not None, 0, *Ws, *As, *(Wskips if Wskips is not None else ()))


def gat_level(x: torch.Tensor, graph: CSRGraph, Ws: Sequence[torch.Tensor], As: Sequence[torch.Tensor],
              Wskips: Optional[Sequence[torch.Tensor]], alpha: float, concat: bool, pipeline=None, xs=None) -> torch.Tensor:
    H = len(Ws)
    Fin = x.shape[1]
    if (xs is None and PAD_K and Fin % 16 and 16 < Fin <= 1024 and x.is_cuda and not x.requires_grad and x.dim() == 2
            and H <= MAX_HEAD_TABLE and Ws[0].dim() == 2 and Ws[0].is_cuda):
        from .features import padded_columns
        xp = padded_columns(x, 16)
        W, a, Wskip = StackHeads.apply(H, Wskips is not None, xp.shape[1], *Ws, *As, *(Wskips if Wskips is not None else ()))
        return GATLevelFn.apply(xp, W, a, Wskip, graph, alpha, concat, None, pipeline)
    if H <= MAX_HEAD_TABLE:
        return GATLevelHeadsFn.apply(x, graph, alpha, concat, pipeline, H, Wskips is not None, xs, *Ws, *As,
                                     *(Wskips if Wskips is not None else ()))
    W = torch.stack(list(Ws), 0)
    a = torch.stack([p.reshape(-1) for p in As], 0)
    Wskip = torch.stack(list(Wskips), 0) if Wskips is not None else None
    return GATLevelFn.apply(x, W, a, Wskip, graph, alpha, concat, None, pipeline)
```

Before: 3.911 billion.

## Fuse self-loop tail forward output into projection GEMM epilogue

Adds a tail-aware variant of the small-K projection GEMM. For rows past the self-loop tail start, its epilogue writes Wh (with optional ELU) straight into the layer output through the user-row permutation. This removes the separate gat_forward_tail kernel and its re-read of Wh for those rows. The tail softmax stats (m, Z, qneg) are instead set with tensor fills. This adds a per-row branch, index loads and extra template instantiations to the GEMM epilogue, and falls back to the unfused path when its conditions are not met.

Result: faster. 4.044 billion, median of 6 (+3.4%).

```diff
diff --git a/include/pygat_amd.h b/include/pygat_amd.h
--- a/include/pygat_amd.h
+++ b/include/pygat_amd.h
@@ -8,7 +8,7 @@
 extern "C" {
 #endif
 
-#define PYGAT_ABI_VERSION 14
+#define PYGAT_ABI_VERSION 15
 
 enum {
   PYGAT_OK = 0,
@@ -163,6 +163,10 @@
 int pygat_gat_backward_tail(int row_first, int n_rows, int H, int Fo, int flags, const float* G, const float* y,
                             const int32_t* user_row, float* dWh, int64_t ld_dwh, int zero_cols, float* ds, float* dt, void* stream);
 
+int pygat_project_tail_blocked(int n, int Fin, int H, int Fo, const float* X, int64_t ldx, const pygat_col_blocks* x_blk,
+                               const float* Wcat, int64_t ldw, const float* a_pad, float* Wh, float* s, int split_k, void* ws,
+                               int gemm_mode, int row_first, const int32_t* user_row, float* out, int flags, void* stream);
+
 int pygat_gatv2_forward(const pygat_graph* g, int H, int Fo, float alpha, int flags,
                         const float* WW, const float* a2, const float* sk, const float* att_mask,
                         float* out, float* hattn, float* m, float* Z, void* part, void* stream);
diff --git a/pygat_amd/_lib.py b/pygat_amd/_lib.py
--- a/pygat_amd/_lib.py
+++ b/pygat_amd/_lib.py
@@ -11,7 +11,7 @@
 if _config.lib_path:
     LIB_PATH = os.path.abspath(_config.lib_path)
 
-ABI_VERSION = 14
+ABI_VERSION = 15
 F_ELU = 1
 F_SKIP = 2
 F_MAIN_ONLY = 4
@@ -23,7 +23,7 @@
     "pygat_exclusive_scan_i32", "pygat_dense_fill_cols", "pygat_csr_symmetric_perm",
     "pygat_gemm_workspace_bytes", "pygat_gemm_f32", "pygat_gemm_f32_blocked", "pygat_project_blocked", "pygat_wgrad_blocked", "pygat_pack_params", "pygat_pack_params_heads", "pygat_stack_heads", "pygat_stack_heads_padded", "pygat_project", "pygat_attn_scores",
     "pygat_unpack_wgrad",
-    "pygat_edge_pairs", "pygat_slot_bounds", "pygat_slot_meta", "pygat_partials_bytes", "pygat_head_group", "pygat_gat_forward", "pygat_gat_forward_phases_ok", "pygat_gat_forward_tail", "pygat_gat_backward_col_tail", "pygat_gat_backward_tail", "pygat_head_mean",
+    "pygat_edge_pairs", "pygat_slot_bounds", "pygat_slot_meta", "pygat_partials_bytes", "pygat_head_group", "pygat_gat_forward", "pygat_gat_forward_phases_ok", "pygat_gat_forward_tail", "pygat_gat_backward_col_tail", "pygat_gat_backward_tail", "pygat_project_tail_blocked", "pygat_head_mean",
     "pygat_gat_backward_prepare", "pygat_gat_backward_row", "pygat_gat_backward_col", "pygat_gat_backward_rowsum",
     "pygat_gat_backward_col_da_bytes", "pygat_a_grad_fold",
     "pygat_agrad_workspace_bytes", "pygat_a_grad", "pygat_wgrad_workspace_bytes", "pygat_wgrad",
@@ -106,6 +106,7 @@
     lib.pygat_gat_forward_tail.argtypes = [i, i, i, i, i, p, i64, p, p, p, p, p, p, p]
     lib.pygat_gat_backward_col_tail.argtypes = [i, i, i, i, p, p, p, p]
     lib.pygat_gat_backward_tail.argtypes = [i, i, i, i, i, p, p, p, p, i64, i, p, p, p]
+    lib.pygat_project_tail_blocked.argtypes = [i, i, i, i, p, i64, CB, p, i64, p, p, p, i, p, i, i, p, p, i, p]
     lib.pygat_head_mean.argtypes = [i, i, i, p, p, p, p]
     lib.pygat_gat_backward_prepare.argtypes = [i, i, i, i, i, p, p, p, p, p, p, p, p, p, f, p, i, i, i, p, p]
     lib.pygat_gat_backward_row.argtypes = [C.POINTER(Graph), i, i, f, p, p, p, p, p, p, i, i, i, p]
diff --git a/pygat_amd/config.py b/pygat_amd/config.py
--- a/pygat_amd/config.py
+++ b/pygat_amd/config.py
@@ -37,6 +37,7 @@
     pad_k: bool
     renumber: bool
     tail: bool
+    tail_fused: bool
 
     @staticmethod
     def from_env() -> "Config":
@@ -56,6 +57,7 @@
             pad_k=_flag("PYGAT_PAD_K", True),
             renumber=_flag("PYGAT_RENUMBER", True),
             tail=_flag("PYGAT_TAIL", True),
+            tail_fused=_flag("PYGAT_TAIL_FUSED", True),
         )
 
     def describe(self) -> dict:
diff --git a/pygat_amd/csrc/core.hip b/pygat_amd/csrc/core.hip
--- a/pygat_amd/csrc/core.hip
+++ b/pygat_amd/csrc/core.hip
@@ -33,7 +33,8 @@
   if (!strcmp(kernel, "k4_headline_da")) return pygat::footprint_k4_headline_da(num_regs, scratch_bytes);
   if (!strcmp(kernel, "tn_x3w")) return pygat::footprint_gemm_x3(0, num_regs, scratch_bytes);
   if (!strcmp(kernel, "x3gw")) return pygat::footprint_gemm_x3(1, num_regs, scratch_bytes);
-  pygat::set_error("kernel_footprint: unknown kernel '%s' (k2_headline, k4_headline_da, tn_x3w, x3gw)", kernel);
+  if (!strcmp(kernel, "k1_x3_tail")) return pygat::footprint_gemm_x3(2, num_regs, scratch_bytes);
+  pygat::set_error("kernel_footprint: unknown kernel '%s' (k2_headline, k4_headline_da, tn_x3w, x3gw, k1_x3_tail)", kernel);
   return PYGAT_EINVAL;
 }
 
diff --git a/pygat_amd/csrc/gemm_fast.h b/pygat_amd/csrc/gemm_fast.h
--- a/pygat_amd/csrc/gemm_fast.h
+++ b/pygat_amd/csrc/gemm_fast.h
@@ -24,6 +24,11 @@
   int64_t s_ld;
   int vec_out, s_vec;
   int lds_rows;
+  int64_t row_first;
+  const int32_t* urow;
+  float* tail_out;
+  int64_t ld_out;
+  int tail_elu;
 };
 
 struct TnArgs {
@@ -54,9 +59,12 @@
 
 bool gemm_split(int mode);
 
-int try_gemm_smallk_x3(const SmallKArgs& g, int NT, dim3 grid, hipStream_t st);
+int try_gemm_smallk_x3(const SmallKArgs& g, int NT, dim3 grid, hipStream_t st, int tl = 0);
 int try_project_x3(int n, int Fin, int H, int Fp, const float* X, int64_t ldx, const float* Wcat, int64_t ldw, float* Wh,
                    float* s, const float* a_pad, bool split, hipStream_t st);
+int try_project_x3_tail(int n, int Fin, int H, int Fp, const float* X, int64_t ldx, const float* Wcat, int64_t ldw, float* Wh,
+                        float* s, const float* a_pad, bool split, hipStream_t st, int64_t row_first, const int32_t* urow,
+                        float* out, int elu);
 int try_gemm_tn_x3(const TnArgs& g, int splits, hipStream_t st);
 int try_gemm_x3g(int transA, int transB, int M, int N, int64_t K, const float* A, int64_t lda, const float* B, int64_t ldb,
                  const pygat_out_segments* out, int accumulate, int splits, int64_t k_per_split, float* ws, hipStream_t st,
diff --git a/pygat_amd/csrc/k1_gemm.hip b/pygat_amd/csrc/k1_gemm.hip
--- a/pygat_amd/csrc/k1_gemm.hip
+++ b/pygat_amd/csrc/k1_gemm.hip
@@ -542,6 +542,9 @@
                        int max_splits, float* ws, bool split, hipStream_t st, int N1, const float* B2, int64_t ldb2);
 int try_project_x3(int n, int Fin, int H, int Fp, const float* X, int64_t ldx, const float* Wcat, int64_t ldw, float* Wh,
                    float* s, const float* a_pad, bool split, hipStream_t st);
+int try_project_x3_tail(int n, int Fin, int H, int Fp, const float* X, int64_t ldx, const float* Wcat, int64_t ldw, float* Wh,
+                        float* s, const float* a_pad, bool split, hipStream_t st, int64_t row_first, const int32_t* urow,
+                        float* out, int elu);
 int try_gemm_x3g(int transA, int transB, int M, int N, int64_t K, const float* A, int64_t lda, const float* B, int64_t ldb,
                  const pygat_out_segments* out, int accumulate, int splits, int64_t k_per_split, float* ws, hipStream_t st,
                  ColBlocks ab, ColBlocks cb, int* splits_used);
@@ -682,6 +685,26 @@
   seg.col_start[k] = ncols;
   seg.nseg = k;
   return pygat_gemm_f32_blocked(0, 0, n, ncols, Fin, X, ldx, x_blk, Wcat, ldw, &seg, nullptr, 0, split_k, ws, gemm_mode, stream);
+}
+
+extern "C" int pygat_project_tail_blocked(int n, int Fin, int H, int Fo, const float* X, int64_t ldx, const pygat_col_blocks* x_blk,
+                                          const float* Wcat, int64_t ldw, const float* a_pad, float* Wh, float* s, int split_k,
+                                          void* ws, int gemm_mode, int row_first, const int32_t* user_row, float* out, int flags,
+                                          void* stream) {
+  const int Fp = padded_width(Fo);
+  PYGAT_REQUIRE(n > 0 && Fin > 0 && H > 0 && Fp > 0 && X && Wcat && Wh && s && out, "project_tail: bad arguments");
+  PYGAT_REQUIRE(row_first >= 0 && row_first < n, "project_tail: tail rows [%d, %d) empty", row_first, n);
+  PYGAT_REQUIRE((flags & ~PYGAT_F_ELU) == 0, "project_tail: flags other than PYGAT_F_ELU (a skip projection takes the tail stream)");
+  PYGAT_REQUIRE(gemm_mode >= PYGAT_GEMM_DEFAULT && gemm_mode <= PYGAT_GEMM_FP32_MFMA, "project_tail: unknown product mode %d", gemm_mode);
+  if (!col_blocks_on(x_blk) && a_pad && split_k <= 1 && Fo == Fp) {
+    const int r = try_project_x3_tail(n, Fin, H, Fp, X, ldx, Wcat, ldw, Wh, s, a_pad, gemm_split(gemm_mode), (hipStream_t)stream,
+                                      row_first, user_row, out, (flags & PYGAT_F_ELU) ? 1 : 0);
+    if (r < 0) return r;
+    if (r == 1) return PYGAT_OK;
+  }
+  const int rc = pygat_project_blocked(n, Fin, H, Fo, X, ldx, x_blk, Wcat, ldw, a_pad, Wh, nullptr, s, split_k, ws, gemm_mode, stream);
+  if (rc) return rc;
+  return pygat_gat_forward_tail(row_first, n - row_first, H, Fo, flags, Wh, 0, nullptr, out, user_row, nullptr, nullptr, nullptr, stream);
 }
 
 namespace pygat {
diff --git a/pygat_amd/csrc/k1_gemm_x3.hip b/pygat_amd/csrc/k1_gemm_x3.hip
--- a/pygat_amd/csrc/k1_gemm_x3.hip
+++ b/pygat_amd/csrc/k1_gemm_x3.hip
@@ -1,4 +1,5 @@
 #include "gemm_fast.h"
+#include "attn_common.h"
 #include <stdlib.h>
 #include <type_traits>
 
@@ -92,7 +93,7 @@
 #if (PYGAT_DIAG_K1 & 16)
 __device__ unsigned long long k1_stamps[2048 * 8 * 8];
 #endif
-template <bool TB, int NT, int SM, int SPC>
+template <bool TB, int NT, int SM, int SPC, int TL = 0>
 __global__ __launch_bounds__(512) void gemm_smallk_x3_kernel(SmallKArgs g) {
   constexpr bool SV = (SM == 1);
   constexpr int SRF = (SM >= 4) ? SM : 0;
@@ -178,6 +179,23 @@
     const int64_t row = row0 + fr;
     const bool row_ok = FAST || row < g.M;
     const bool full = FAST || row0 + 32 <= g.M;
+    int32_t tu[FAST ? 4 : 1];
+    if constexpr (TL > 0) {
+#pragma unroll
+      for (int q = 0; q < (FAST ? 4 : 1); ++q) {
+        const int64_t r = FAST ? row0 + (lane >> 3) + 8 * q : (row < g.M ? row : g.M - 1);
+        tu[q] = TL == 2 ? g.urow[r] : (int32_t)r;
+      }
+    }
+    (void)tu;
+    auto tail_route = [&](int64_t r, int64_t u, int col, float4& v, float*& dst) {
+      const bool tl = r >= g.row_first;
+      const bool el = tl && g.tail_elu;
+      const float4 e = make_float4(elu1(v.x), elu1(v.y), elu1(v.z), elu1(v.w));
+      v.x = el ? e.x : v.x; v.y = el ? e.y : v.y; v.z = el ? e.z : v.z; v.w = el ? e.w : v.w;
+      dst = tl ? g.tail_out + u * g.ld_out + col : dst;
+    };
+    (void)tail_route;
     if constexpr (SV) {
       if (sv_on) {
 #pragma unroll
@@ -257,8 +275,12 @@
             st4(patch + fr * 36 + 8 * gq + 4 * fh, make_float4(acc[nt][4 * gq], acc[nt][4 * gq + 1], acc[nt][4 * gq + 2], acc[nt][4 * gq + 3]));
           float* bq = base + (row0 + (lane >> 3)) * ld + 4 * (lane & 7);
 #pragma unroll
-          for (int q = 0; q < 4; ++q)
-            st4(bq + (int64_t)8 * q * ld, ld4(patch + ((lane >> 3) + 8 * q) * 36 + 4 * (lane & 7)));
+          for (int q = 0; q < 4; ++q) {
+            float4 v = ld4(patch + ((lane >> 3) + 8 * q) * 36 + 4 * (lane & 7));
+            float* dst = bq + (int64_t)8 * q * ld;
+            if constexpr (TL > 0) tail_route(row0 + (lane >> 3) + 8 * q, tu[q], colt + 4 * (lane & 7), v, dst);
+            st4(dst, v);
+          }
         }
       } else {
       const bool vec = full && !g.accumulate && g.vec_out && colt + 32 <= g.N;
@@ -266,18 +288,25 @@
         int64_t ld;
         float* base = out_segment(g.out, colt, ld) + row * ld + 4 * fh;
 #pragma unroll
-        for (int gq = 0; gq < 4; ++gq)
-          st4(base + 8 * gq, make_float4(acc[nt][4 * gq], acc[nt][4 * gq + 1], acc[nt][4 * gq + 2], acc[nt][4 * gq + 3]));
+        for (int gq = 0; gq < 4; ++gq) {
+          float4 v = make_float4(acc[nt][4 * gq], acc[nt][4 * gq + 1], acc[nt][4 * gq + 2], acc[nt][4 * gq + 3]);
+          float* dst = base + 8 * gq;
+          if constexpr (TL > 0) tail_route(row, tu[0], colt + 8 * gq + 4 * fh, v, dst);
+          st4(dst, v);
+        }
       } else if (!(PYGAT_DIAG_K1 & 1)) {
 #pragma unroll
         for (int gq = 0; gq < 4; ++gq) {
           const int col4 = colt + 8 * gq + 4 * fh;
           int64_t ld;
           float* p = out_segment(g.out, col4, ld) + row * ld;
+          float4 v = make_float4(acc[nt][4 * gq], acc[nt][4 * gq + 1], acc[nt][4 * gq + 2], acc[nt][4 * gq + 3]);
+          if constexpr (TL > 0) tail_route(row, tu[0], col4, v, p);
+          const float vv[4] = {v.x, v.y, v.z, v.w};
 #pragma unroll
           for (int j = 0; j < 4; ++j)
             if (row_ok && col4 + j < g.N) {
-              if (g.accumulate) p[j] += acc[nt][4 * gq + j]; else p[j] = acc[nt][4 * gq + j];
+              if (g.accumulate) p[j] += vv[j]; else p[j] = vv[j];
             }
         }
       }
@@ -528,6 +557,26 @@
   return hipGetLastError();
 }
 
+template <int SM, int SPC>
+static hipError_t launch_smallk_x3_tail(const SmallKArgs& g, int NT, int tl, dim3 grid, size_t lds, hipStream_t st) {
+  int dev = -1;
+  (void)hipGetDevice(&dev);
+#define PYGAT_X3_LAUNCH(n, t)                                                                             \
+  {                                                                                                       \
+    static bool attr_set[64] = {};                                                                        \
+    if (dev < 0 || dev >= 64 || !attr_set[dev]) {                                                         \
+      (void)hipFuncSetAttribute(reinterpret_cast<const void*>(&gemm_smallk_x3_kernel<false, n, SM, SPC, t>), \
+                                hipFuncAttributeMaxDynamicSharedMemorySize, 160 * 1024);                  \
+      if (dev >= 0 && dev < 64) attr_set[dev] = true;                                                     \
+    }                                                                                                     \
+    hipLaunchKernelGGL((gemm_smallk_x3_kernel<false, n, SM, SPC, t>), grid, dim3(512), lds, st, g);       \
+  }
+  if (NT == 4) { if (tl == 2) PYGAT_X3_LAUNCH(4, 2) else PYGAT_X3_LAUNCH(4, 1) }
+  else { if (tl == 2) PYGAT_X3_LAUNCH(2, 2) else PYGAT_X3_LAUNCH(2, 1) }
+#undef PYGAT_X3_LAUNCH
+  return hipGetLastError();
+}
+
 template <int SPC>
 static hipError_t launch_smallk_x3_sv(const SmallKArgs& g, int NT, dim3 grid, size_t lds, hipStream_t st) {
   int dev = -1;
@@ -547,7 +596,7 @@
   return hipGetLastError();
 }
 
-int try_gemm_smallk_x3(const SmallKArgs& g_in, int NT, dim3 grid, hipStream_t st) {
+int try_gemm_smallk_x3(const SmallKArgs& g_in, int NT, dim3 grid, hipStream_t st, int tl) {
   SmallKArgs g = g_in;
   const size_t lds = (size_t)3 * (32 * NT) * (g.K + 8) * sizeof(uint16_t) + (g.svec ? (size_t)g.K * 8 * sizeof(float) : 0) +
                      (g.sr_a ? (size_t)32 * NT * sizeof(float) : 0) + 16;
@@ -564,7 +613,13 @@
   constexpr bool generic = false;
   const int spc = (generic || g.accumulate || g.svec || (NT == 5 && g.K == 128)) ? 0 : (g.K == 128 ? 2 : (g.K == 64 ? 1 : 0));
   hipError_t e;
-  if (g.sr_a) {
+  if (tl) {
+    if (!g.sr_a || spc == 0 || g.transB || g.svec || g.accumulate || !g.lds_rows || !g.s_vec || (NT != 2 && NT != 4) ||
+        (g.sr_fp != 8 && g.sr_fp != 16) || (g.N % (32 * NT)) != 0 || !g.tail_out || (g.ld_out % 4) != 0 || !aligned16(g.tail_out))
+      return 0;
+    if (spc == 2) e = g.sr_fp == 16 ? launch_smallk_x3_tail<16, 2>(g, NT, tl, grid, ldsz, st) : launch_smallk_x3_tail<8, 2>(g, NT, tl, grid, ldsz, st);
+    else e = g.sr_fp == 16 ? launch_smallk_x3_tail<16, 1>(g, NT, tl, grid, ldsz, st) : launch_smallk_x3_tail<8, 1>(g, NT, tl, grid, ldsz, st);
+  } else if (g.sr_a) {
     if (spc == 0 || g.transB || g.svec || (g.sr_fp != 8 && g.sr_fp != 16) || (g.N % (32 * NT)) != 0) return 0;
     if (spc == 2) e = g.sr_fp == 16 ? launch_smallk_x3<false, 16, 2>(g, NT, grid, ldsz, st) : launch_smallk_x3<false, 8, 2>(g, NT, grid, ldsz, st);
     else e = g.sr_fp == 16 ? launch_smallk_x3<false, 16, 1>(g, NT, grid, ldsz, st) : launch_smallk_x3<false, 8, 1>(g, NT, grid, ldsz, st);
@@ -588,6 +643,12 @@
 
 int try_project_x3(int n, int Fin, int H, int Fp, const float* X, int64_t ldx, const float* Wcat, int64_t ldw, float* Wh,
                    float* s, const float* a_pad, bool split, hipStream_t st) {
+  return try_project_x3_tail(n, Fin, H, Fp, X, ldx, Wcat, ldw, Wh, s, a_pad, split, st, -1, nullptr, nullptr, 0);
+}
+
+int try_project_x3_tail(int n, int Fin, int H, int Fp, const float* X, int64_t ldx, const float* Wcat, int64_t ldw, float* Wh,
+                        float* s, const float* a_pad, bool split, hipStream_t st, int64_t row_first, const int32_t* urow,
+                        float* out, int elu) {
   const int R = H * Fp;
   if (!split || !a_pad || (Fp != 8 && Fp != 16) || (R % 32) != 0 || (Fin != 64 && Fin != 128) || n < 8192) return 0;
   if (!aligned16(X) || (ldx % 4) != 0) return 0;
@@ -599,11 +660,12 @@
   g.out.nseg = 1; g.out.col_start[0] = 0; g.out.col_start[1] = R; g.out.ptr[0] = Wh; g.out.ld[0] = R;
   g.svec = nullptr; g.sv_ld = 0; g.sv_n = 0; g.s_out = s; g.s_ld = H;
   g.tiles_m = (int)cdiv(n, 256); g.transB = 0; g.sr_a = a_pad; g.sr_fp = Fp;
+  g.row_first = row_first; g.urow = urow; g.tail_out = out; g.ld_out = R; g.tail_elu = elu;
   const int tiles_n = R / (32 * NT);
   int gx = 256 / tiles_n;
   if (gx < 1) gx = 1;
   if (gx > g.tiles_m) gx = g.tiles_m;
-  return try_gemm_smallk_x3(g, NT, dim3((unsigned)gx, (unsigned)tiles_n, 1), st);
+  return try_gemm_smallk_x3(g, NT, dim3((unsigned)gx, (unsigned)tiles_n, 1), st, row_first < 0 ? 0 : (urow ? 2 : 1));
 }
 
 
@@ -1373,7 +1435,8 @@
 int footprint_gemm_x3(int which, int* regs, int* scratch) {
   hipFuncAttributes at;
   const void* fn = which == 0 ? reinterpret_cast<const void*>(&gemm_tn_x3w_kernel)
-                              : reinterpret_cast<const void*>(&gemm_x3gw_kernel<true, false>);
+                 : which == 1 ? reinterpret_cast<const void*>(&gemm_x3gw_kernel<true, false>)
+                              : reinterpret_cast<const void*>(&gemm_smallk_x3_kernel<false, 4, 16, 2, 2>);
   const hipError_t e = hipFuncGetAttributes(&at, fn);
   if (e != hipSuccess) {
     (void)hipGetLastError();
diff --git a/pygat_amd/ops.py b/pygat_amd/ops.py
--- a/pygat_amd/ops.py
+++ b/pygat_amd/ops.py
@@ -60,6 +60,7 @@
 RENUMBER_MIN_BYTES_TAIL = 48 << 20
 TAIL = _config.tail
 TAIL_MIN_SHARE = 0.05
+TAIL_FUSED = _config.tail_fused
 
 
 def head_group(N: int, H: int, Fo: int) -> int:
@@ -354,23 +355,13 @@
             if split_k > 1 else None
         if xs is not None and need[0]:
             xs = None
-        with _span("k1_project"):
-            if xs is not None:
-                check(lib.pygat_project_sparse(L.N, Fin, H, Fo, xs.rowptr.data_ptr(), xs.col.data_ptr(), xs.val.data_ptr(),
-                                               Wcat.data_ptr(), L.ldw, 0.0, None, 0, None, Wh.data_ptr(), _ptr(Sk), s.data_ptr(),
-                                               st), "project_sparse")
-            else:
-                check(lib.pygat_project_blocked(L.N, Fin, H, Fo, x.data_ptr(), L.ldx, L.xb(), Wcat.data_ptr(), L.ldw, a_pad.data_ptr(),
-                                                Wh.data_ptr(), _ptr(Sk), s.data_ptr(), split_k, _ptr(ws), GEMM_MODES[L.mode], st),
-                      "project")
         flags = (_lib.F_ELU if concat else 0) | (_lib.F_SKIP if skip else 0)
-        single = (not concat) and H == 1
-        hattn = torch.empty(L.N, L.R, dtype=f32, device=dev) if (not concat and (need_grad or not single)) else None
-        m = torch.empty(L.N, H, dtype=f32, device=dev) if need_grad else None
-        Z = torch.empty(L.N, H, dtype=f32, device=dev) if need_grad else None
         flavour = backward_flavour(L.R) if need_grad else None
-        aneg = torch.empty(L.N, L.R, dtype=f32, device=dev) if flavour == "rowlocal" else None
-        qneg = torch.empty(L.N, H, dtype=f32, device=dev) if flavour == "rowlocal" else None
+        if (TAIL and graph.degree_sorted and concat and graph.symmetric
+                and (not need_grad or (flavour == "rowlocal" and L.hg >= H and bwd_heads is None))):
+            t = graph.fwd.self_loop_tail(L.ts)
+            if t is not None and L.N - t[0] >= TAIL_MIN_SHARE * L.N:
+                tail = (t[0], t[2], t[1])
         out = pipeline[2] if (pipeline is not None and len(pipeline) > 2 and concat) else None
         if out is not None:
             if tuple(out.shape) != (L.N, H * Fo) or out.dtype != f32 or not out.is_contiguous() or out.device != dev:
@@ -378,13 +369,37 @@
             out = torch.empty(0, dtype=f32, device=dev).set_(out.untyped_storage(), out.storage_offset(), out.shape, out.stride())
         else:
             out = torch.empty(L.N, H * Fo if concat else Fo, dtype=f32, device=dev)
+        fuse_fwd = (TAIL_FUSED and tail is not None and not skip and L.Fo == L.Fp and xs is None and x.dim() == 2
+                    and L.mode == "split-bf16"
+                    and (not need_grad or (DA_IN_K4 and need[2] and L.N * L.R * 4 >= DA_MIN_BYTES
+                                           and lib.pygat_gat_backward_col_da_bytes(tail[1], H, Fo, H) > 0)))
+        with _span("k1_project"):
+            if xs is not None:
+                check(lib.pygat_project_sparse(L.N, Fin, H, Fo, xs.rowptr.data_ptr(), xs.col.data_ptr(), xs.val.data_ptr(),
+                                               Wcat.data_ptr(), L.ldw, 0.0, None, 0, None, Wh.data_ptr(), _ptr(Sk), s.data_ptr(),
+                                               st), "project_sparse")
+            elif fuse_fwd:
+                check(lib.pygat_project_tail_blocked(L.N, Fin, H, Fo, x.data_ptr(), L.ldx, L.xb(), Wcat.data_ptr(), L.ldw,
+                                                     a_pad.data_ptr(), Wh.data_ptr(), s.data_ptr(), split_k, _ptr(ws),
+                                                     GEMM_MODES[L.mode], tail[0], _ptr(user_row), out.data_ptr(), flags, st),
+                      "project_tail")
+            else:
+                check(lib.pygat_project_blocked(L.N, Fin, H, Fo, x.data_ptr(), L.ldx, L.xb(), Wcat.data_ptr(), L.ldw, a_pad.data_ptr(),
+                                                Wh.data_ptr(), _ptr(Sk), s.data_ptr(), split_k, _ptr(ws), GEMM_MODES[L.mode], st),
+                      "project")
+        single = (not concat) and H == 1
+        hattn = torch.empty(L.N, L.R, dtype=f32, device=dev) if (not concat and (need_grad or not single)) else None
+        m = torch.empty(L.N, H, dtype=f32, device=dev) if need_grad else None
+        Z = torch.empty(L.N, H, dtype=f32, device=dev) if need_grad else None
+        aneg = torch.empty(L.N, L.R, dtype=f32, device=dev) if flavour == "rowlocal" else None
+        qneg = torch.empty(L.N, H, dtype=f32, device=dev) if flavour == "rowlocal" else None
         part = torch.empty(lib.pygat_partials_bytes(graph.nnz, L.ts, H, L.Fp) // 4, dtype=f32,
                            device=dev)
-        if (TAIL and graph.degree_sorted and concat and graph.symmetric
-                and (not need_grad or (flavour == "rowlocal" and L.hg >= H and bwd_heads is None))):
-            t = graph.fwd.self_loop_tail(L.ts)
-            if t is not None and L.N - t[0] >= TAIL_MIN_SHARE * L.N:
-                tail = (t[0], t[2], t[1])
+        if fuse_fwd and m is not None:
+            m[tail[0]:].zero_()
+            Z[tail[0]:].fill_(1.0)
+            if qneg is not None:
+                qneg[tail[0]:].zero_()
         chunks = [(graph.fwd.ref(L.ts) if tail is None else tail[1], 0, L.N if tail is None else tail[0])]
         if pipeline is not None and concat and pipeline[0] > 1:
             chunks = (graph.fwd.row_chunks(int(pipeline[0]), L.ts) if tail is None
@@ -408,7 +423,7 @@
                 continue
             with _span("k2_forward"):
                 k2(gref, flags, st)
-                if tail is not None and c == len(chunks) - 1:
+                if tail is not None and c == len(chunks) - 1 and not fuse_fwd:
                     check(lib.pygat_gat_forward_tail(tail[0], L.N - tail[0], H, Fo, flags, Wh.data_ptr(), 0, _ptr(Sk), out.data_ptr(),
                                                      _ptr(user_row), _ptr(m), _ptr(Z), _ptr(qneg), st), "gat_forward_tail")
             if pipeline is not None and concat:
@@ -416,8 +431,9 @@
         if phases:
             main_s.wait_stream(side_s)
             if tail is not None:
-                check(lib.pygat_gat_forward_tail(tail[0], L.N - tail[0], H, Fo, flags, Wh.data_ptr(), 0, _ptr(Sk), out.data_ptr(),
-                                                 _ptr(user_row), _ptr(m), _ptr(Z), _ptr(qneg), st), "gat_forward_tail")
+                if not fuse_fwd:
+                    check(lib.pygat_gat_forward_tail(tail[0], L.N - tail[0], H, Fo, flags, Wh.data_ptr(), 0, _ptr(Sk), out.data_ptr(),
+                                                     _ptr(user_row), _ptr(m), _ptr(Z), _ptr(qneg), st), "gat_forward_tail")
                 pipeline[1](len(chunks), tail[0], L.N, out)
         if not concat and not single:
             check(lib.pygat_head_mean(L.N, H, Fo, hattn.data_ptr(), _ptr(Sk), out.data_ptr(), st), "head_mean")
@@ -426,6 +442,7 @@
         ctx.graph, ctx.L, ctx.alpha, ctx.concat, ctx.flags = graph, L, float(alpha), concat, flags
         ctx.user_row = user_row
         ctx.tail = tail
+        ctx.tail_fwd_fused = fuse_fwd
         ctx.xs = xs
         ctx.flavour = flavour
         ctx.bwd_heads = None
```
